# lachinov/brats2019

Hardware: AMD Instinct MI355X
Metric: volumes_per_sec_fwd_bwd_128cubed_x4ch (higher is better)
Workload: dtype bf16

## Files before the change

brats2019_amd/_lib.py:

```python
from __future__ import annotations

import ctypes as C
import os

import torch

_PKG = os.path.dirname(os.path.abspath(__file__))
LIB_PATH = os.environ.get("RU_LIB_PATH") or os.path.join(_PKG, "lib", "libresunet_hip.so")

_lib = None
PRECISIONS = {"f32": 0, "bf16x3": 1}
GRAD_PRECISIONS = {"bf16x3": 1, "bf16": 2}
FUSE_GN_BWD_STATS, FUSE_GN_BWD_APPLY, FUSE_SIDE_STREAM, FUSE_BATCH_WREDUCE, FUSE_TAIL_FINALIZE, FUSE_PW_DGRAD = 1, 2, 4, 8, 16, 32

_vp, _f, _d, _i, _sz = C.c_void_p, C.c_float, C.c_double, C.c_int, C.c_size_t

SIGNATURES = {
    "ru_last_error": (C.c_char_p, []),
    "ru_version": (_i, []),
    "ru_device_ok": (_i, []),
    "ru_conv3d_workspace_bytes": (_sz, [_i] * 7),
    "ru_conv3d_fwd": (_i, [_vp, _vp, _vp, _vp] + [_i] * 7 + [_vp, _sz, _vp]),
    "ru_conv3d_bwd_data": (_i, [_vp, _vp, _vp] + [_i] * 7 + [_vp, _sz, _vp]),
    "ru_conv3d_fwd_p": (_i, [_vp, _vp, _vp, _vp] + [_i] * 8 + [_vp, _sz, _vp]),
    "ru_conv3d_bwd_data_p": (_i, [_vp, _vp, _vp] + [_i] * 8 + [_vp, _sz, _vp]),
    "ru_conv3d_bwd_weight": (_i, [_vp, _vp, _vp, _vp] + [_i] * 7 + [_vp, _sz, _vp]),
    "ru_conv3d_bwd_weight_p": (_i, [_vp, _vp, _vp, _vp] + [_i] * 8 + [_vp, _sz, _vp]),
    "ru_groupnorm_workspace_bytes": (_sz, [_i, _i, _sz]),
    "ru_groupnorm_fwd": (_i, [_vp] * 7 + [_i, _i, _sz, _i, _f, _f, _vp, _sz, _vp]),
    "ru_groupnorm_bwd": (_i, [_vp] * 9 + [_i, _i, _sz, _i, _f, _vp, _sz, _vp]),
    "ru_leaky_relu_fwd": (_i, [_vp, _vp, _sz, _f, _vp]),
    "ru_leaky_relu_bwd": (_i, [_vp, _vp, _vp, _sz, _f, _vp]),
    "ru_upsample2x_trilinear_fwd": (_i, [_vp, _vp] + [_i] * 5 + [_vp]),
    "ru_upsample2x_trilinear_bwd": (_i, [_vp, _vp] + [_i] * 5 + [_vp]),
    "ru_sigmoid_fwd": (_i, [_vp, _vp, _sz, _vp]),
    "ru_criterion_workspace_bytes": (_sz, [_i, _i, _sz]),
    "ru_criterion_sums": (_i, [_vp, _vp, _vp, _i, _i, _sz, _f, _vp, _sz, _vp]),
    "ru_criterion_grad": (_i, [_vp, _vp, _vp, _d, _f, _f, _f, _f, _vp, _i, _i, _sz, _vp]),
    "ru_criterion_value": (_i, [C.POINTER(_d), _i, _d, _d, C.POINTER(_d), C.POINTER(_d)]),
    "ru_criterion_value_device": (_i, [_vp, _i, _d, _d, _d, _d, _vp, _vp]),
    "ru_crit_moments_workspace_bytes": (_sz, [_i, _i, _sz]),
    "ru_crit_moments": (_i, [_vp, _vp, _i, _i, _sz, C.c_uint, _vp, _vp, _sz, _vp]),
    "ru_crit_reduce": (_i, [_vp, _i, _i, _vp, _vp]),
    "ru_crit_eval": (_i, [_vp, _vp, _i, _i, _d, _d, _vp, _i, _vp, _vp, _vp]),
    "ru_crit_grad": (_i, [_vp, _vp, _vp, _vp, _i, _i, _sz, _i, _vp, _vp]),
    "ru_adam_amsgrad_step": (_i, [_vp] * 5 + [_sz] + [_f] * 5 + [_i, _vp]),
    "ru_adam_step": (_i, [_vp] * 5 + [_sz] + [_f] * 5 + [_i, _vp]),
    "ru_unet_create": (_vp, [_i, C.POINTER(_i), C.POINTER(_i), C.POINTER(_i), _i]),
    "ru_unet_destroy": (None, [_vp]),
    "ru_unet_set_precision": (_i, [_vp, _i]),
    "ru_unet_freeze_params": (_i, [_vp, _i]),
    "ru_unet_get_precision": (_i, [_vp]),
    "ru_unet_set_grad_precision": (_i, [_vp, _i]),
    "ru_unet_get_grad_precision": (_i, [_vp]),
    "ru_unet_set_fusion": (_i, [_vp, C.c_uint]),
    "ru_unet_probe": (_i, [_vp, _i]),
    "ru_unet_probe_read": (_i, [_vp, C.POINTER(C.c_double), C.POINTER(_i)]),
    "ru_unet_probe_read_families": (_i, [_vp, C.POINTER(C.c_double), C.POINTER(_i), _i]),
    "ru_unet_param_count": (_i, [_vp]),
    "ru_unet_param_name": (C.c_char_p, [_vp, _i]),
    "ru_unet_param_ndim": (_i, [_vp, _i]),
    "ru_unet_param_dim": (_i, [_vp, _i, _i]),
    "ru_unet_param_offset": (_sz, [_vp, _i]),
    "ru_unet_param_total": (_sz, [_vp]),
    "ru_unet_param_is_dead": (_i, [_vp, _i]),
    "ru_unet_workspace_bytes": (_sz, [_vp] + [_i] * 5),
    "ru_unet_forward": (_i, [_vp, _vp, _vp, _vp] + [_i] * 5 + [_vp, _sz, _vp]),
    "ru_unet_backward": (_i, [_vp] * 6),
    "ru_unet_backward_criterion": (_i, [_vp, _vp, _vp, _vp, _d, _f, _f, _f, _f, _vp, _vp, _vp]),
    "ru_unet_gn_stats": (_i, [_vp, _i, _vp, _vp, _vp]),
    "ru_comm_unique_id": (_i, [_vp]),
    "ru_comm_init": (_i, [C.POINTER(_vp), _vp, _i, _i]),
    "ru_comm_destroy": (_i, [_vp]),
    "ru_comm_rank": (_i, [_vp]),
    "ru_comm_world": (_i, [_vp]),
    "ru_allreduce": (_i, [_vp, _vp, _sz, _i, _vp]),
    "ru_comm_group_begin": (_i, []),
    "ru_comm_group_end": (_i, []),
    "ru_tta_merge": (_i, [_vp, _i, C.c_uint, _vp, _vp, _vp, _i, _i, _i, _i, _vp]),
    "ru_compose_labels": (_i, [_vp, _vp, C.c_ulonglong, _vp, _sz, _vp]),
    "ru_dice_counts": (_i, [_vp, _vp, _vp, _i, _i, _sz, _vp]),
    "ru_dice_accumulate": (_i, [_vp, _vp, _i, _i, _i, _vp]),
    "ru_hausdorff_workspace_bytes": (_sz, [_i] * 6),
    "ru_hausdorff_sq": (_i, [_vp, _vp] + [_i] * 6 + [_vp, _vp, _sz, _vp]),
    "ru_hausdorff_accumulate": (_i, [_vp, _vp] + [_i] * 4 + [_vp]),
    "ru_label_confusion": (_i, [_vp, _vp, _i, _i, _i, _sz, _vp, _vp, _vp]),
    "ru_overlap_accumulate": (_i, [_vp, _i, _i, _i, _i, _vp, _vp, _vp]),
    "ru_dice1d_accumulate": (_i, [_vp, _vp, _i, _i, _i, _vp]),
    "ru_rmse_accumulate": (_i, [_vp, _vp, _vp]),
    "ru_surface_workspace_bytes": (_sz, [_i] * 6),
    "ru_surface_metrics": (_i, [_vp, _vp] + [_i] * 6 + [_d, _vp, _vp, _vp, _sz, _vp]),
    "ru_surface_accumulate": (_i, [_vp, _vp] + [_i] * 4 + [_vp]),
    "ru_lesion_workspace_bytes": (_sz, [_i] * 7),
    "ru_lesion_metrics": (_i, [_vp, _vp] + [_i] * 7 + [C.c_longlong, _d, _vp, _vp, _vp, _i, _vp, _sz, _vp]),
    "ru_lesion_accumulate": (_i, [_vp, _vp] + [_i] * 4 + [_vp]),
    "ru_tile_gather": (_i, [_vp, _vp] + [_i] * 6 + [C.POINTER(_i), _i, _i, _i, _vp]),
    "ru_tile_scatter": (_i, [_vp, _vp] + [_i] * 6 + [C.POINTER(_i), _i, _i, _i, C.POINTER(_i), C.POINTER(_i), _vp]),
    "ru_blend_accumulate": (_i, [_vp, _vp, _vp] + [_i] * 8 + [C.POINTER(_i), _i, C.POINTER(_i), _i, C.POINTER(_i), _i, _i, _i, _vp]),
    "ru_blend_finalize": (_i, [_vp, _vp, _vp] + [_i] * 8 + [C.POINTER(_i), _i, C.POINTER(_i), _i, C.POINTER(_i), _i, _vp]),
    "ru_case_bbox": (_i, [_vp, _vp, _i, _i, _i, _i, _vp]),
# ... 8 lines not shown
    "ru_postprocess_regions": (_i, [_vp, _vp, _i, _i, _i, _i, C.POINTER(C.c_longlong), C.POINTER(C.c_ulonglong), C.c_uint, C.c_uint, _i, _vp, _vp, _vp, _vp, _sz, _vp]),
    "ru_ens_accumulate": (_i, [_vp, _i, C.c_uint, _vp, _i, _i, _i, _i, _i, C.POINTER(_i), C.POINTER(_i), _vp]),
    "ru_ens_finalize": (_i, [_vp, _i, _vp, _vp, _vp, _i, _sz, _vp]),
    "ru_ens_accumulate_finalize": (_i, [_vp, _i, C.c_uint, _vp, _i, _i, _vp, _vp, _vp, _i, _i, _i, _i, C.POINTER(_i), C.POINTER(_i), _vp]),
    "ru_ens_argmax": (_i, [_vp, _i, _vp, _i, _sz, _vp]),
    "ru_paste_probs": (_i, [_vp, _vp, _i, _i, _i, _i, C.POINTER(_i), C.POINTER(_i), _vp]),
    "ru_unc_accumulate": (_i, [_vp, _i, C.c_uint, _vp, _vp, _i, _i, _i, _i, _i, C.POINTER(_i), C.POINTER(_i), _vp]),
    "ru_unc_accumulate_finalize": (_i, [_vp, _i, C.c_uint, _vp, _vp, _i, _i, _i, _vp, _vp, _vp, _vp, _i, _i, _i, _i, C.POINTER(_i), C.POINTER(_i), _vp]),
    "ru_unc_finalize": (_i, [_vp, _vp, _i, _i, _i, _vp, _vp, _vp, _vp, _i, _sz, _vp]),
    "ru_unc_histogram": (_i, [_vp, _vp, _vp, _i, _i, _i, _vp, _vp, _vp]),
    "ru_unc_score": (_i, [_vp, C.POINTER(_i), _i, _vp, _vp, _vp]),
    "ru_paste_u8c": (_i, [_vp, _vp, _i, _i, _i, _i, C.POINTER(_i), C.POINTER(_i), _vp]),
    "ru_zscore_workspace_bytes": (_sz, [_i, _sz]),
    "ru_zscore_stats": (_i, [_vp, _vp, _i, _sz, _vp, _sz, _vp]),
    "ru_augment_patch": (_i, [_vp, _vp, _vp, _vp, _i, _i, _i, _i, _vp, _vp, _vp, _i, _vp, _vp, _vp, _vp, _vp]),
    "ru_augment_patch_soft": (_i, [_vp, _vp, _vp, _vp, _vp, _i, _i, _i, _i, _vp, _vp, _vp, _i, _vp, _vp, _vp, _vp, _vp]),
    "ru_elastic_workspace_bytes": (_sz, [_i, _i, _i]),
    "ru_elastic_noise": (_i, [C.c_ulonglong, _i, _i, _i, _vp, _vp]),
    "ru_elastic_field": (_i, [_vp, _d, _d, _i, _i, _i, _vp, _vp, _sz, _vp]),
    "ru_elastic_warp": (_i, [_vp, _i, _vp, _i, _vp, _i, _i, _i, _i, _vp, _vp, _vp, _vp, _vp]),
    "ru_layout_convert": (_i, [_vp, _vp, _i, _i, _sz, _i, _vp]),
    "ru_upsample2x_trilinear_fwd_l": (_i, [_vp, _vp] + [_i] * 5 + [_f, _vp]),
    "ru_upsample2x_trilinear_bwd_l": (_i, [_vp, _vp] + [_i] * 5 + [_vp]),
    "ru_conv3d_fwd_l": (_i, [_vp, _vp, _vp, _vp] + [_i] * 7 + [_vp, _sz, _vp]),
    "ru_conv3d_bwd_weight_l": (_i, [_vp, _vp, _vp] + [_i] * 7 + [_vp, _sz, _vp]),
}


CRIT_KINDS = {"Dice_loss_joint": 0, "BCE_Loss": 1, "MSE_Loss": 2, "CE_Loss": 3, "Dice1D": 4, "GDL_joint": 5, "sens_loss_joint": 6,
              "Dice_loss_separate": 7}
CRIT_MOMENTS, CRIT_MAX_TERMS = 7, 8
CRIT_MASK_LOGS, CRIT_MASK_ALL = (1 << 4) | (1 << 5), 0x7F
CRIT_M_D2 = 6

CONF_PROB, CONF_LABEL, OVERLAP_MAX_LABELS = 0, 1, 8
OVERLAP_MODES = {"itk": 0, "wt": 1, "validate": 2}

UNC_MEASURES = {"std": 0, "entropy": 1}
UNC_REGIONS, UNC_LEVELS, UNC_CLASSES = 3, 101, 4

SURFACE_PROB, SURFACE_LABEL, SURFACE_REGIONS, SURFACE_COUNTS = 0, 1, 3, 6
SURFACE_COLUMNS = {"dice": 0, "sensitivity": 1, "specificity": 2, "hd95": 3}

LESION_COUNTS, LESION_TABLE_COLUMNS, LESION_CHUNK = 6, 5, 8
LESION_COLUMNS = {"dice": 0, "hd95": 1}

POSTPROCESS_MASKS, POSTPROCESS_LABELS, POSTPROCESS_REGIONS, POSTPROCESS_STATS = 0, 1, 3, 6


class CritTerm(C.Structure):
    _fields_ = [("kind", _i), ("weight", _d), ("priority", _d), ("bg_weight", _d)]


def load():
    global _lib
    if _lib is not None:
        return _lib
    if not os.path.exists(LIB_PATH):
        raise RuntimeError(
            "libresunet_hip.so not found at %s -- build it with `python -m brats2019_amd.build` "
            "(hipcc, gfx950).  There is no CPU fallback for this path." % LIB_PATH)
    lib = C.CDLL(LIB_PATH)
    for name, (res, args) in SIGNATURES.items():
        if os.environ.get("RU_LIB_PATH") and not hasattr(lib, name):
            continue
        fn = getattr(lib, name)
        fn.restype = res
        fn.argtypes = args
    _lib = lib
    return lib


def last_error():
    return load().ru_last_error().decode("utf-8", "replace")


def check(rc, what=""):
    if rc != 0:
        raise RuntimeError("libresunet_hip: %s failed (%d): %s" % (what, rc, last_error()))


def require_gpu():
    if not torch.cuda.is_available():
        raise RuntimeError("brats2019_amd: no ROCm GPU visible -- the ResUNet hot path is HIP-only (no CPU fallback)")
    load()


def ptr(t, allow_none=False):
    if t is None:
        if allow_none:
            return None
        raise ValueError("null tensor")
    if not t.is_cuda:
        raise RuntimeError("brats2019_amd: expected a ROCm device tensor, got a %s tensor (HIP-only path)" % t.device)
    if not t.is_contiguous():
        raise ValueError("tensor must be contiguous (NCDHW)")
    return C.c_void_p(t.data_ptr())


def f32(t):
    if t.dtype != torch.float32:
        raise TypeError("expected float32, got %s" % t.dtype)
    return ptr(t)


def stream():
# ... 6 lines not shown
```

brats2019_amd/csrc/conv3_sb.hip:

```cpp
#include "conv3_sb_common.hpp"
#include "conv3_wz_pack.hpp"
#include "conv3_mx_pack.hpp"

namespace ru {

constexpr int SB1_W_BYTES = SB_KSTEPS * 2 * 64 * 16;
template <int TZ, int TY, bool IN16, bool OUT16>
__global__ __launch_bounds__(256, 2) void conv3_sb_kernel(const Conv3Args a, const u32x4* __restrict__ wfrag, int ntz, int nty, int ntx, int nchunk) {
    using P = SB<TZ, TY>;
    constexpr int MT = P::MT, HY = P::HY, HX = P::HX, HVOLP = P::HVOLP, NSV = P::NSV, NROW = P::NROW;
    extern __shared__ __attribute__((aligned(16))) float smem[];
    u32x4* lds = reinterpret_cast<u32x4*>(smem);

    const int tid = threadIdx.x, lane = tid & 63, wave = tid >> 6;
    int b = xcd_swizzle(blockIdx.x, gridDim.x);
    const int tiles_per_sample = ntz * nty * ntx;
    const int n = b / tiles_per_sample;
    const int tis = b - n * tiles_per_sample;
    b = tis;
    const int tx = b % ntx; b /= ntx;
    const int ty = b % nty;
    const int tz = b / nty;
    const int z0 = tz * TZ, y0 = ty * TY, x0 = tx * 16;
    const int cog = blockIdx.y;
// ... 526 lines not shown
    float t[8];
#pragma unroll
    for (int e = 0; e < 8; ++e) {
        const int ci = (g & 1) * 8 + e;
        float v = 0.f;
        if (tap >= 0 && ci < cin_conv && co < cout_conv)
            v = mode == 0 ? w[((size_t)co * Cin_f + ci) * 27 + tap] : w[((size_t)ci * Cin_f + co) * 27 + (26 - tap)];
        t[e] = v;
    }
    u32x4 hi, lo;
    split8(t, hi, lo);
    hfrag[((size_t)f * 2 + 0) * 64 + lane] = hi;
    hfrag[((size_t)f * 2 + 1) * 64 + lane] = lo;
}
constexpr int SB_FORMS_ALL = 15;
__device__ __forceinline__ void sb_pack_both(const float* __restrict__ w, u32x4* __restrict__ wfrag, int Cin_f, int Cout_f, int mode, int nchunk, int ncog, int forms, int i) {
    const int direct = ncog * nchunk * SB_KSTEPS * 64;
    if (i < direct) { if (!(forms & 16)) sb_pack_one(w, wfrag, Cin_f, Cout_f, mode, nchunk, ncog, i); return; }
    const int cin_conv = mode == 0 ? Cin_f : Cout_f, cout_conv = mode == 0 ? Cout_f : Cin_f;
    if (sb_head_shape(cin_conv, cout_conv)) { sb_pack_head_one(w, wfrag + (size_t)direct * 2, Cin_f, Cout_f, mode, i - direct); return; }
    if (mx_channels_ok(cin_conv, cout_conv)) { if (forms & 4) mx_pack_one(w, wfrag + (size_t)direct * 2, Cin_f, Cout_f, mode, ncog, i - direct, (forms & 32) != 0); return; }
    if (!wz_channels_ok(cin_conv, cout_conv)) return;
    const int wz = WZ16_FORM ? (cout_conv / 32) * nchunk * 4 * 2 * WZ_KSTEPS * 64 : 0;
    int r = i - direct;
    if (WZ16_FORM && (forms & 1)) {
        if (r < wz) { wz_pack_one(w, reinterpret_cast<wz_u32x4*>(wfrag + (size_t)direct * 2), Cin_f, Cout_f, mode, nchunk, cout_conv / 32, r); return; }
        r -= wz;
    }
    const int wz32 = (cout_conv / 32) * nchunk * 4 * 9 * 64;
    if (forms & 2) {
        if (r < wz32) { wz32_pack_one(w, reinterpret_cast<wz_u32x4*>(wfrag + ((size_t)direct + wz) * 2), Cin_f, Cout_f, mode, nchunk, cout_conv / 32, r); return; }
        r -= wz32;
    }
    if (forms & 8) wz32mx_pack_one(w, reinterpret_cast<wz_u32x4*>(wfrag + ((size_t)direct + wz + wz32) * 2), Cin_f, Cout_f, mode, nchunk, cout_conv / 32, r);
}
static inline int sb_pack_threads(int cin_conv, int cout_conv, int forms) {
    const int nchunk = cdiv(cin_conv, 16), ncog = cdiv(cout_conv, 16);
    return ncog * nchunk * SB_KSTEPS * 64 + (wz_channels_ok(cin_conv, cout_conv) ? (cout_conv / 32) * nchunk * (((WZ16_FORM && (forms & 1)) ? 4 * 2 * WZ_KSTEPS : 0) + ((forms & 2) ? 4 * 9 : 0) + ((forms & 8) ? WZ32MX_UNITS_XI : 0)) * 64 : 0)
         + (sb_head_shape(cin_conv, cout_conv) ? SB_HEAD_KSTEPS * 64 : 0) + (((forms & 4) && mx_channels_ok(cin_conv, cout_conv)) ? ncog * MX_UNITS * 64 : 0);
}
static int sb_pack_forms(int mode) {
    if (mode == 1) return conv3_mxg_enabled() ? (4 | 32) : 0;
    const bool mxon = conv3_mx_enabled();
    const char* e = getenv("RU_WZ");
    if (e && *e == '0') return mxon ? 4 : 0;
    if (mxon && conv3_mx_wz_enabled()) return 4 | 8;
    return (mxon ? 4 : 0) | (conv3_wz32_enabled() ? 2 : 1);
}
__global__ void conv3_sb_pack_kernel(const float* __restrict__ w, u32x4* __restrict__ wfrag, int Cin_f, int Cout_f, int mode, int nchunk, int ncog, int forms) {
    sb_pack_both(w, wfrag, Cin_f, Cout_f, mode, nchunk, ncog, forms, blockIdx.x * blockDim.x + threadIdx.x);
}
__global__ void conv3_sb_pack_batch_kernel(const SbPackBatch b) {
    const SbPackEntry& e = b.e[blockIdx.y];
    sb_pack_both(e.w, reinterpret_cast<u32x4*>(e.wfrag), e.Cin_f, e.Cout_f, e.mode, e.nchunk, e.ncog, e.forms, blockIdx.x * blockDim.x + threadIdx.x);
}
int conv3_sb_pack_batch(SbPackBatch& b, hipStream_t s) {
    if (b.n == 0) return RU_OK;
    int maxtotal = 0;
    for (int i = 0; i < b.n; ++i) {
        const SbPackEntry& e = b.e[i];
        const int t = sb_pack_threads(e.mode == 0 ? e.Cin_f : e.Cout_f, e.mode == 0 ? e.Cout_f : e.Cin_f, e.forms);
        if (t > maxtotal) maxtotal = t;
    }
    hipLaunchKernelGGL(conv3_sb_pack_batch_kernel, dim3(cdiv(maxtotal, 256), b.n), dim3(256), 0, s, b);
    RU_CHECK_LAUNCH("conv3_sb_pack_batch_kernel");
    b.n = 0;
    return RU_OK;
}
int conv3_sb_switch_signature() {
    const char* e = getenv("RU_WZ");
    return ((e && *e == '0') ? 0 : 1) | (conv3_wz32_enabled() ? 2 : 0) | (conv3_mx_enabled() ? 4 : 0) | (conv3_mx_wz_enabled() ? 8 : 0) | (conv3_mxg_enabled() ? 16 : 0);
}
bool conv3_sb_forward_skips_direct(int N, int Cin, int Cout, int D, int H, int W) {
    if (conv3_sb_uses_wz(N, Cin, Cout, D, H, W, 2)) return true;
    return conv3_mx_enabled() && conv3_mx_shape_ok(N, Cin, Cout, D, H, W);
}
int conv3_sb_pack_add(SbPackBatch& b, const float* w, void* wfrag, int Cin_f, int Cout_f, int mode, bool all_forms, hipStream_t s, bool skip_direct) {
    if (b.n == RU_PACK_BATCH) { const int rc = conv3_sb_pack_batch(b, s); if (rc) return rc; }
    const int cin_conv = mode == 0 ? Cin_f : Cout_f, cout_conv = mode == 0 ? Cout_f : Cin_f;
    SbPackEntry& e = b.e[b.n++];
    e.w = w; e.wfrag = wfrag; e.Cin_f = Cin_f; e.Cout_f = Cout_f; e.mode = mode; e.nchunk = cdiv(cin_conv, 16); e.ncog = cdiv(cout_conv, 16);
    e.forms = all_forms ? SB_FORMS_ALL : (sb_pack_forms(mode) | ((skip_direct && mode == 0) ? 16 : 0));
    return RU_OK;
}

size_t conv3_sb_frag_bytes_direct(int Cin_conv, int Cout_conv) {
    return (size_t)cdiv(Cout_conv, 16) * cdiv(Cin_conv, 16) * SB_KSTEPS * 2 * 64 * 16;
}
size_t conv3_sb_frag_bytes(int Cin_conv, int Cout_conv) {
    return conv3_sb_frag_bytes_direct(Cin_conv, Cout_conv) + wz_frag_bytes(Cin_conv, Cout_conv) + wz32_frag_bytes(Cin_conv, Cout_conv) + wz32mx_frag_bytes(Cin_conv, Cout_conv)
         + (sb_head_shape(Cin_conv, Cout_conv) ? (size_t)SB_HEAD_KSTEPS * 2 * 64 * 16 : 0) + mx_frag_bytes(Cin_conv, Cout_conv);
}
bool conv3_sb_head_takes_residual(int N, int Cin, int Cout, int D, int H, int W) {
    const char* e = getenv("RU_HEAD_RES");
    if (e && *e == '0') return false;
    if (!conv3_sb_head_form_enabled() || !sb_head_shape(Cin, Cout) || Cin % 16 != 0 || (W & 3) != 0) return false;
    if ((size_t)D * H * W * 64 >= ((size_t)1 << 31)) return false;
    return sb_use_v2(sb_choose(N, Cout, D, H, W));
}
bool conv3_sb_head_form_enabled() {
    const char* e = getenv("RU_HEAD_FORM");
    return !(e && e[0] == '0');
}

int conv3_sb_pack_weights(const float* w, void* wfrag, int Cin_f, int Cout_f, int mode, hipStream_t s, bool grad_operand) {
    const int cin_conv = mode == 0 ? Cin_f : Cout_f, cout_conv = mode == 0 ? Cout_f : Cin_f;
    const int nchunk = cdiv(cin_conv, 16), ncog = cdiv(cout_conv, 16);
    const int forms = SB_FORMS_ALL | (grad_operand ? 32 : 0);
    const int total = sb_pack_threads(cin_conv, cout_conv, forms);
    hipLaunchKernelGGL(conv3_sb_pack_kernel, dim3(cdiv(total, 256)), dim3(256), 0, s, w, (u32x4*)wfrag, Cin_f, Cout_f, mode, nchunk, ncog, forms);
    RU_CHECK_LAUNCH("conv3_sb_pack_kernel");
    return RU_OK;
}

bool conv3_sb_uses_wz(int N, int Cin, int Cout, int D, int H, int W, int products) {
    const char* e = getenv("RU_WZ");
    const bool off = e && *e == '0';
    return !off && products != 1 && conv3_wz_shape_ok(N, Cin, Cout, D, H, W);
}
int conv3_sb_tiles_per_sample(int N, int Cin, int Cout, int D, int H, int W, int products) {
    if (conv3_sb_uses_wz(N, Cin, Cout, D, H, W, products)) return (int)wz_grid_x(N, Cout, D, H, W);
    const SBChoice c = sb_choose(N, Cout, D, H, W);
    if (sb_use_v2(c)) return (int)sb2_grid_x(N, Cout, D, H, W);
    return cdiv(D, c.tz) * cdiv(H, c.ty) * cdiv(W, 16);
}

bool conv3_sb_bst_usable(int N, int Cout, int D, int H, int W) { return sb_use_v2(sb_choose(N, Cout, D, H, W)); }

template <int TZ, int TY, bool IN16, bool OUT16>
static int sb_cfg(const Conv3Args& a, hipStream_t s) {
    using P = SB<TZ, TY>;
    static PerDevice attr_done;
    if (!attr_done.get()) {
        hipError_t e = hipFuncSetAttribute(reinterpret_cast<const void*>(conv3_sb_kernel<TZ, TY, IN16, OUT16>), hipFuncAttributeMaxDynamicSharedMemorySize, P::LDS_BYTES + SB1_W_BYTES);
        if (e != hipSuccess) return hip_fail(e, "hipFuncSetAttribute(conv3_sb)");
        attr_done.set();
    }
// ... 86 lines not shown
```

brats2019_amd/csrc/engine.hip:

```cpp
#include "ru_common.h"

#include <vector>
#include <math.h>
#include <stdlib.h>
#include <string.h>

#include <string>
#include <vector>

namespace ru {

static thread_local char g_err[512] = "";
void set_error(const char* fmt, ...) {
    va_list ap;
    va_start(ap, fmt);
    vsnprintf(g_err, sizeof(g_err), fmt, ap);
    va_end(ap);
}
int hip_fail(hipError_t e, const char* what) {
    set_error("%s: %s", what, hipGetErrorString(e));
    return RU_EHIP;
}

constexpr float kSlope = 1e-2f;
// ... 30 lines not shown
    return on;
}
static int trace_sync(const char* what, hipStream_t s) {
    fprintf(stderr, "[ru] %s\n", what);
    const hipError_t e = hipStreamSynchronize(s);
    if (e != hipSuccess) { fprintf(stderr, "[ru]   -> %s\n", hipGetErrorString(e)); return hip_fail(e, what); }
    return RU_OK;
}

enum { FAM_CONV_L0 = 0, FAM_CONV_DEEP, FAM_WGRAD_L0, FAM_WGRAD_DEEP, FAM_GN, FAM_PW, FAM_OTHER, FAM_COUNT };
enum { INST_CONV16_FWD = 0, INST_CONV16_DGRAD, INST_CONV_DEEP_FWD, INST_CONV_DEEP_DGRAD, INST_WGRAD16_FUSED, INST_WGRAD16_PLAIN, INST_WGRAD_DEEP, INST_COUNT };
struct FamilySink {
    std::vector<hipEvent_t> ev;
    std::vector<int> fam;
    std::vector<int> inst;
    size_t used = 0;
    ~FamilySink() { for (hipEvent_t e : ev) (void)hipEventDestroy(e); }
};
static thread_local FamilySink* t_sink = nullptr;
static thread_local int t_hint_c = 16;
static thread_local int t_hint_inst = -1;
struct RedQueues { WgradRedList main, side; hipStream_t side_stream = nullptr; };
static thread_local RedQueues* t_red = nullptr;
static WgradRedList* red_for(hipStream_t s) { return t_red ? ((t_red->side_stream && s == t_red->side_stream) ? &t_red->side : &t_red->main) : nullptr; }
static int family_of(const char* call) {
    auto has = [&](const char* k) { return strstr(call, k) != nullptr; };
    if (has("wgrad3_launch")) return t_hint_c <= 16 ? FAM_WGRAD_L0 : FAM_WGRAD_DEEP;
    if (has("wgrad_reduce_flush")) return FAM_WGRAD_DEEP;
    if (has("conv3_launch") || has("conv3_sb_launch")) return t_hint_c <= 16 ? FAM_CONV_L0 : FAM_CONV_DEEP;
    if (has("gn_")) return FAM_GN;
    if (has("conv1_") || has("wgrad1_launch") || has("up2_") || has("s2d_launch") || has("d2s_launch") || has("lrelu_bwd_launch")) return FAM_PW;
    return FAM_OTHER;
}
static void sink_begin(const char* call, hipStream_t s) {
    FamilySink& k = *t_sink;
    while (k.ev.size() < k.used + 2) {
        hipEvent_t e;
        if (hipEventCreate(&e) != hipSuccess) return;
        k.ev.push_back(e);
    }
    if (k.fam.size() < k.ev.size() / 2) { k.fam.resize(k.ev.size() / 2); k.inst.resize(k.ev.size() / 2); }
    k.fam[k.used / 2] = family_of(call);
    k.inst[k.used / 2] = t_hint_inst;
    t_hint_inst = -1;
    (void)hipEventRecord(k.ev[k.used], s);
}
static void sink_end(hipStream_t s) {
    FamilySink& k = *t_sink;
    if (k.ev.size() < k.used + 2) return;
    (void)hipEventRecord(k.ev[k.used + 1], s);
    k.used += 2;
}

#define RU_RUN(call)                      \
    do {                                  \
        if (!A.dry) {                     \
            if (A.failed) { set_error("workspace too small"); return RU_ENOMEM; } \
            if (t_sink) sink_begin(#call, s); \
            const int rc__ = (call);      \
            if (t_sink) sink_end(s);      \
            if (rc__ != RU_OK) return rc__; \
            if (trace_on()) { const int rt__ = trace_sync(#call, s); if (rt__ != RU_OK) return rt__; } \
        }                                 \
    } while (0)

__global__ void gn_scale_shift_kernel(const float* __restrict__ gamma, const float* __restrict__ beta, const float* __restrict__ mean,
                                      const float* __restrict__ rstd, float* __restrict__ scale, float* __restrict__ shift, int N, int C, int G) {
    const int i = blockIdx.x * blockDim.x + threadIdx.x;
    if (i >= N * C) return;
    const int n = i / C, c = i % C, g = c / (C / G);
    const float a = gamma[c] * rstd[n * G + g];
    scale[i] = a;
    shift[i] = beta[c] - mean[n * G + g] * a;
}

}

using namespace ru;

struct ParamInfo {
    std::string name;
    int ndim;
    int dims[5];
    size_t offset, numel;
    bool dead;
};

struct BlockP {
    int down = -1, conv1 = -1, conv2 = -1, n1w = -1, n1b = -1, n2w = -1, n2b = -1;
    int cin_down = 0, c = 0;
    size_t pk_f1 = 0, pk_f2 = 0, pk_d1 = 0, pk_d2 = 0, pk_downT = 0, pk_down16 = 0;
    size_t fk_f1 = 0, fk_f2 = 0, fk_d1 = 0, fk_d2 = 0;
};

struct GNSave {
    float *mean = nullptr, *rstd = nullptr, *scale = nullptr, *shift = nullptr;
    float act_slope = 0.01f;
    float* k = nullptr;
};

struct BlockSave {
    const BlockP* bp = nullptr;
    const float* xprev = nullptr;
    float* xs2d = nullptr;
    const float* x = nullptr;
    const GNSave* xg = nullptr;
    float *y1 = nullptr, *y2 = nullptr, *out = nullptr;
    GNSave g1, g2;
    int N = 0, C = 0, D = 0, H = 0, W = 0;
};

struct DecSave {
    const float* z = nullptr;
    float *u = nullptr, *v = nullptr, *c = nullptr;
    const float* skip = nullptr;
    int level = 0;
};

constexpr int kOneProduct = 0x100;
struct ru_unet {
    int depth = 0, nout = 0;
    std::vector<int> enc, dec, ch;
    std::vector<ParamInfo> params;
    size_t total = 0;
    std::vector<std::vector<BlockP>> enc_blocks, dec_blocks;
    std::vector<BlockP> first_blocks;
    std::vector<int> up_w, dec1_w;
    std::vector<size_t> pk_upT, pk_decT;
    int conv_in = -1, nin_w = -1, nin_b = -1, conv_out_w = -1, conv_out_b = -1;
    size_t pk_in = 0, pk_out = 0, pk_out_d = 0, pk_total = 0;
    size_t fk_in = 0, fk_out = 0, fk_out_d = 0, fk_total = 0;
    int precision = RU_PREC_F32;
    unsigned fusion = RU_FUSE_GN_BWD_STATS | RU_FUSE_GN_BWD_APPLY | RU_FUSE_SIDE_STREAM | RU_FUSE_BATCH_WREDUCE | RU_FUSE_PW_DGRAD;
    int grad_precision = RU_PREC_BF16X3;
    int grad_products() const { return (precision == RU_PREC_BF16X3 && grad_precision == RU_PREC_BF16) ? 1 : 3; }
    int wgrad_mode() const { return precision | (grad_products() == 1 ? kOneProduct : 0); }
    bool c16 = false;
    char* fpack = nullptr;

    bool have_fwd = false, training = false;
    int N = 0, D = 0, H = 0, W = 0;
    char* ws = nullptr;
    size_t ws_bytes = 0, fwd_end = 0, fwd_keep = 0;
    float* pack = nullptr;
    const float* x_in = nullptr;
    const float* x_in4 = nullptr;
    bool x_in4_planned = false;
    bool params_frozen = false;
    const float* packed_params = nullptr;
    const void* packed_base = nullptr;
    int packed_prec = -1;
    bool packed_c16 = false;
    int pack_sig = -1;
    float *y0 = nullptr, *t0 = nullptr, *probs = nullptr;
    GNSave g0;
    const float* head_in = nullptr;
    std::vector<BlockSave> first_s;
    std::vector<std::vector<BlockSave>> enc_s, dec_s;
    std::vector<DecSave> dstage;
    std::vector<const float*> skips;
    std::vector<GNSave> gn_order;
    bool probe_on = false;
    bool probe_families = false;
    ru::FamilySink* sink = nullptr;
    std::vector<hipEvent_t> probe_ev;
    size_t probe_used = 0;
    hipStream_t side = nullptr;
    std::vector<hipEvent_t> fork_ev;
    ru::RedQueues red;
    unsigned* tickets = nullptr;
    int ticket_next = 0;
    unsigned* next_ticket() { return tickets ? tickets + (ticket_next++ & 255) : nullptr; }
    bool tails() const { return c16 && (fusion & RU_FUSE_TAIL_FINALIZE) && tickets != nullptr; }
    size_t fork_used = 0;
    ~ru_unet() {
        for (hipEvent_t e : probe_ev) (void)hipEventDestroy(e);
        for (hipEvent_t e : fork_ev) (void)hipEventDestroy(e);
        if (side) (void)hipStreamDestroy(side);
        if (tickets) (void)hipFree(tickets);
        delete sink;
    }
};

static int add_param(ru_unet* h, const std::string& name, std::initializer_list<int> dims, bool dead = false) {
    ParamInfo p;
    p.name = name;
    p.ndim = (int)dims.size();
    size_t n = 1;
    int i = 0;
    for (int d : dims) { p.dims[i++] = d; n *= (size_t)d; }
    for (; i < 5; ++i) p.dims[i] = 1;
    p.offset = h->total;
    p.numel = n;
    p.dead = dead;
    h->total += n;
    h->params.push_back(p);
    return (int)h->params.size() - 1;
}

static BlockP add_block(ru_unet* h, const std::string& prefix, int cin_down, int c, bool dead = false) {
    BlockP b;
    b.c = c;
    b.cin_down = cin_down;
    if (cin_down > 0) b.down = add_param(h, prefix + "downsample.0.weight", {c, cin_down, 2, 2, 2}, dead);
    b.conv1 = add_param(h, prefix + "conv1.conv1.weight", {c, c, 3, 3, 3}, dead);
    b.conv2 = add_param(h, prefix + "conv2.conv1.weight", {c, c, 3, 3, 3}, dead);
    b.n1w = add_param(h, prefix + "norm1.weight", {c}, dead);
    b.n1b = add_param(h, prefix + "norm1.bias", {c}, dead);
    b.n2w = add_param(h, prefix + "norm2.weight", {c}, dead);
    b.n2b = add_param(h, prefix + "norm2.bias", {c}, dead);
    return b;
}

static std::string fmt(const char* f, int a, int b = 0) {
    char buf[128];
    snprintf(buf, sizeof(buf), f, a, b);
    return buf;
}

static void assign_block_packs(ru_unet* h, BlockP& b) {
    const size_t n = conv3_packed_floats(b.c, b.c);
    b.pk_f1 = h->pk_total; h->pk_total += n;
    b.pk_f2 = h->pk_total; h->pk_total += n;
    b.pk_d1 = h->pk_total; h->pk_total += n;
    b.pk_d2 = h->pk_total; h->pk_total += n;
    if (b.down >= 0) {
        b.pk_downT = h->pk_total; h->pk_total += (size_t)8 * b.cin_down * b.c;
        b.pk_down16 = h->pk_total; h->pk_total += (size_t)2 * 8 * b.cin_down * b.c;
    }
    const size_t f = conv3_sb_frag_bytes(b.c, b.c);
    b.fk_f1 = h->fk_total; h->fk_total += f;
    b.fk_f2 = h->fk_total; h->fk_total += f;
    b.fk_d1 = h->fk_total; h->fk_total += f;
    b.fk_d2 = h->fk_total; h->fk_total += f;
}

extern "C" ru_unet_t ru_unet_create(int depth, const int* encoder_layers, const int* decoder_layers,
                                    const int* number_of_channels, int number_of_outputs) {
    if (depth < 2 || depth > 8 || !encoder_layers || !decoder_layers || !number_of_channels || number_of_outputs < 1) {
        set_error("ru_unet_create: bad configuration");
        return nullptr;
    }
    for (int i = 0; i < depth; ++i) {
        if (number_of_channels[i] % kGroups != 0 || number_of_channels[i] <= 0 || encoder_layers[i] < 1 || decoder_layers[i] < 1) {
            set_error("ru_unet_create: channels must be positive multiples of 8 (GroupNorm(8, C)) and layer counts >= 1");
            return nullptr;
        }
    }
    ru_unet* h = new ru_unet();
    if (const char* e = getenv("RU_SIDE_STREAM")) { if (*e == '0') h->fusion &= ~(unsigned)RU_FUSE_SIDE_STREAM; }
    if (const char* e = getenv("RU_FUSION_OFF")) h->fusion &= ~(unsigned)strtoul(e, nullptr, 0);
    if (const char* e = getenv("RU_FUSION_ON")) h->fusion |= (unsigned)strtoul(e, nullptr, 0) & 63u;
    h->depth = depth;
    h->nout = number_of_outputs;
    h->enc.assign(encoder_layers, encoder_layers + depth);
    h->dec.assign(decoder_layers, decoder_layers + depth);
    h->ch.assign(number_of_channels, number_of_channels + depth);
    const std::vector<int>& ch = h->ch;
    h->enc_blocks.resize(depth - 1);
    for (int i = 0; i < depth - 1; ++i)
        for (int j = 0; j < h->enc[i + 1]; ++j)
            h->enc_blocks[i].push_back(add_block(h, fmt("encoder_convs.%d.%d.", i, j), j == 0 ? ch[i] : 0, ch[i + 1]));
    for (int i = 0; i < depth - 1; ++i) h->up_w.push_back(add_param(h, fmt("upsampling.%d.1.weight", i), {ch[i], ch[i + 1], 1, 1, 1}));
    h->dec_blocks.resize(depth);
    for (int i = 0; i < depth; ++i)
        for (int j = 0; j < h->dec[i]; ++j)
            h->dec_blocks[i].push_back(add_block(h, fmt("decoder_convs.%d.%d.", i, j), 0, ch[i], i == depth - 1));
    for (int i = 0; i < depth; ++i)
        h->dec1_w.push_back(add_param(h, fmt("decoder_convs1x1.%d.weight", i), {ch[i], 2 * ch[i], 1, 1, 1}, i == depth - 1));
    h->conv_in = add_param(h, "conv_input.weight", {ch[0], kInCh, 3, 3, 3});
    h->nin_w = add_param(h, "norm_input.weight", {ch[0]});
    h->nin_b = add_param(h, "norm_input.bias", {ch[0]});
    for (int j = 0; j < h->enc[0]; ++j) h->first_blocks.push_back(add_block(h, fmt("conv_first.%d.", j), 0, ch[0]));
    h->conv_out_w = add_param(h, "conv_output.weight", {number_of_outputs, ch[0], 3, 3, 3});
    h->conv_out_b = add_param(h, "conv_output.bias", {number_of_outputs});
    h->pk_total = 0;
    h->pk_in = h->pk_total; h->pk_total += conv3_packed_floats(kInCh, ch[0]);
    h->pk_out = h->pk_total; h->pk_total += conv3_packed_floats(ch[0], number_of_outputs);
    h->pk_out_d = h->pk_total; h->pk_total += conv3_packed_floats(number_of_outputs, ch[0]);
    h->fk_total = 0;
    h->fk_in = h->fk_total; h->fk_total += conv3_sb_frag_bytes(kInCh, ch[0]);
    h->fk_out = h->fk_total; h->fk_total += conv3_sb_frag_bytes(ch[0], number_of_outputs);
    h->fk_out_d = h->fk_total; h->fk_total += conv3_sb_frag_bytes(number_of_outputs, ch[0]);
    for (auto& b : h->first_blocks) assign_block_packs(h, b);
    for (auto& lv : h->enc_blocks) for (auto& b : lv) assign_block_packs(h, b);
    for (int i = 0; i < depth - 1; ++i) for (auto& b : h->dec_blocks[i]) assign_block_packs(h, b);
    for (int i = 0; i < depth - 1; ++i) {
        h->pk_upT.push_back(h->pk_total); h->pk_total += (size_t)ch[i + 1] * ch[i];
        h->pk_decT.push_back(h->pk_total); h->pk_total += (size_t)2 * ch[i] * ch[i];
    }
    return h;
}

extern "C" void ru_unet_destroy(ru_unet_t h) { delete h; }
extern "C" int ru_unet_set_precision(ru_unet_t h, int precision) {
    RU_REQUIRE(h && (precision == RU_PREC_F32 || precision == RU_PREC_BF16X3), "ru_unet_set_precision: bad argument");
    h->precision = precision;
    h->have_fwd = false;
    return RU_OK;
}
extern "C" int ru_unet_get_precision(ru_unet_t h) { return h ? h->precision : -1; }
extern "C" int ru_unet_set_fusion(ru_unet_t h, unsigned mask) {
    RU_REQUIRE(h && (mask & ~(unsigned)(RU_FUSE_GN_BWD_STATS | RU_FUSE_GN_BWD_APPLY | RU_FUSE_SIDE_STREAM | RU_FUSE_BATCH_WREDUCE | RU_FUSE_TAIL_FINALIZE | RU_FUSE_PW_DGRAD)) == 0, "ru_unet_set_fusion: bad argument");
// ... 23 lines not shown
    for (size_t i = 0; i + 1 < k.used; i += 2) {
        hipError_t e = hipEventSynchronize(k.ev[i + 1]);
        if (e != hipSuccess) return hip_fail(e, "hipEventSynchronize(family probe)");
        float t = 0.f;
        e = hipEventElapsedTime(&t, k.ev[i], k.ev[i + 1]);
        if (e != hipSuccess) return hip_fail(e, "hipEventElapsedTime(family probe)");
        ms[k.fam[i / 2]] += t;
        launches[k.fam[i / 2]] += 1;
        const int in = k.inst[i / 2];
        if (in >= 0 && ru::FAM_COUNT + in < nfam) { ms[ru::FAM_COUNT + in] += t; launches[ru::FAM_COUNT + in] += 1; }
    }
    k.used = 0;
    return RU_OK;
}
extern "C" int ru_unet_probe_read(ru_unet_t h, double* total_ms, int* launches) {
    RU_REQUIRE(h && total_ms && launches, "ru_unet_probe_read: null argument");
    double sum = 0.0;
    for (size_t i = 0; i + 1 < h->probe_used; i += 2) {
        hipError_t e = hipEventSynchronize(h->probe_ev[i + 1]);
        if (e != hipSuccess) return hip_fail(e, "hipEventSynchronize(probe)");
        float ms = 0.f;
        e = hipEventElapsedTime(&ms, h->probe_ev[i], h->probe_ev[i + 1]);
        if (e != hipSuccess) return hip_fail(e, "hipEventElapsedTime(probe)");
        sum += ms;
    }
    *total_ms = sum;
    *launches = (int)(h->probe_used / 2);
    h->probe_used = 0;
    return RU_OK;
}
extern "C" int ru_unet_set_grad_precision(ru_unet_t h, int precision) {
    RU_REQUIRE(h && (precision == RU_PREC_BF16X3 || precision == RU_PREC_BF16), "ru_unet_set_grad_precision: RU_PREC_BF16X3 or RU_PREC_BF16");
    h->grad_precision = precision;
    return RU_OK;
}
extern "C" int ru_unet_get_grad_precision(ru_unet_t h) { return h ? h->grad_precision : -1; }
extern "C" int ru_unet_freeze_params(ru_unet_t h, int frozen) {
    RU_REQUIRE(h, "ru_unet_freeze_params: null handle");
    h->params_frozen = frozen != 0;
    h->packed_params = nullptr;
    return RU_OK;
}
extern "C" int ru_unet_param_count(ru_unet_t h) { return h ? (int)h->params.size() : 0; }
extern "C" const char* ru_unet_param_name(ru_unet_t h, int i) { return (h && i >= 0 && i < (int)h->params.size()) ? h->params[i].name.c_str() : nullptr; }
extern "C" int ru_unet_param_ndim(ru_unet_t h, int i) { return (h && i >= 0 && i < (int)h->params.size()) ? h->params[i].ndim : 0; }
extern "C" int ru_unet_param_dim(ru_unet_t h, int i, int d) { return (h && i >= 0 && i < (int)h->params.size() && d >= 0 && d < 5) ? h->params[i].dims[d] : 0; }
extern "C" size_t ru_unet_param_offset(ru_unet_t h, int i) { return (h && i >= 0 && i < (int)h->params.size()) ? h->params[i].offset : 0; }
extern "C" size_t ru_unet_param_total(ru_unet_t h) { return h ? h->total : 0; }
extern "C" int ru_unet_param_is_dead(ru_unet_t h, int i) { return (h && i >= 0 && i < (int)h->params.size()) ? (int)h->params[i].dead : 0; }

static inline const float* P(const ru_unet* h, const float* params, int idx) { return params ? params + h->params[idx].offset : nullptr; }
static inline float* G(const ru_unet* h, float* grads, int idx) { return grads ? grads + h->params[idx].offset : nullptr; }

static int pack_all(ru_unet* h, const float* params, Arena& A, hipStream_t s) {
    float* pk = h->pack;
    SbPackBatch batch;
    batch.n = 0;
    auto pack3 = [&](int pidx, size_t pk_off, size_t fk_off, int cin_f, int cout_f, int mode, int lvl = -1) -> int {
        const bool skipd = h->training && h->c16 && mode == 0 && lvl >= 0 &&
                           conv3_sb_forward_skips_direct(h->N, cin_f, cout_f, h->D >> lvl, h->H >> lvl, h->W >> lvl);
        if (h->precision == RU_PREC_BF16X3) RU_RUN(conv3_sb_pack_add(batch, P(h, params, pidx), h->fpack + fk_off, cin_f, cout_f, mode, !h->training, s, skipd));
        if (h->precision == RU_PREC_F32 && h->c16) RU_RUN(conv3_f32c_pack_weights(P(h, params, pidx), h->fpack + fk_off, cin_f, cout_f, mode, s));
        if (!h->c16) RU_RUN(conv3_pack_weights(P(h, params, pidx), pk + pk_off, cin_f, cout_f, mode, s));
        return RU_OK;
    };
    auto blk = [&](const BlockP& b, int lvl) -> int {
        int rc = pack3(b.conv1, b.pk_f1, b.fk_f1, b.c, b.c, 0, lvl); if (rc) return rc;
        rc = pack3(b.conv2, b.pk_f2, b.fk_f2, b.c, b.c, 0, lvl); if (rc) return rc;
        if (h->training) {
            rc = pack3(b.conv1, b.pk_d1, b.fk_d1, b.c, b.c, 1); if (rc) return rc;
            rc = pack3(b.conv2, b.pk_d2, b.fk_d2, b.c, b.c, 1); if (rc) return rc;
        }
        if (b.down >= 0) {
            if (h->c16) RU_RUN(pack_down16_launch(P(h, params, b.down), pk + b.pk_down16, pk + b.pk_down16 + (size_t)8 * b.cin_down * b.c, b.c, b.cin_down, s));
            else RU_RUN(transpose_launch(P(h, params, b.down), pk + b.pk_downT, b.c, 8 * b.cin_down, s));
        }
        return RU_OK;
    };
    { int rc = pack3(h->conv_in, h->pk_in, h->fk_in, kInCh, h->ch[0], 0); if (rc) return rc; }
    { int rc = pack3(h->conv_out_w, h->pk_out, h->fk_out, h->ch[0], h->nout, 0); if (rc) return rc; }
    if (h->training) { int rc = pack3(h->conv_out_w, h->pk_out_d, h->fk_out_d, h->ch[0], h->nout, 1); if (rc) return rc; }
    for (auto& b : h->first_blocks) { int rc = blk(b, 0); if (rc) return rc; }
    for (size_t lv = 0; lv < h->enc_blocks.size(); ++lv) for (auto& b : h->enc_blocks[lv]) { int rc = blk(b, (int)lv + 1); if (rc) return rc; }
    for (int i = 0; i < h->depth - 1; ++i) for (auto& b : h->dec_blocks[i]) { int rc = blk(b, i); if (rc) return rc; }
    for (int i = 0; i < h->depth - 1; ++i) {
        if (h->c16 && !h->training) continue;
        RU_RUN(transpose_launch(P(h, params, h->up_w[i]), pk + h->pk_upT[i], h->ch[i], h->ch[i + 1], s));
        RU_RUN(transpose_launch(P(h, params, h->dec1_w[i]), pk + h->pk_decT[i], h->ch[i], 2 * h->ch[i], s));
    }
    RU_RUN(conv3_sb_pack_batch(batch, s));
    return RU_OK;
}

static int conv3_gn(ru_unet* h, Arena& A, hipStream_t s, const float* x, const float* wp, const char* wf, float* y, const GNSave* in_gn,
                    const float* gamma, const float* beta, GNSave& out_gn, int N, int Cin, int Cout, int D, int H, int W, bool x_c16 = true,
                    bool x_c4 = false) {
    const int nblk = !h->c16 ? conv3_tiles_per_sample(N, Cin, Cout, D, H, W, h->precision)
                     : (h->precision == RU_PREC_F32 ? conv3_f32c_tiles_per_sample(N, Cin, Cout, D, H, W) : conv3_sb_tiles_per_sample(N, Cin, Cout, D, H, W));
    t_hint_c = Cout;
    float* partials = A.alloc((size_t)N * Cout * nblk * 2);
    out_gn.mean = A.alloc_keep((size_t)N * kGroups);
    out_gn.rstd = A.alloc_keep((size_t)N * kGroups);
    out_gn.scale = A.alloc_keep((size_t)N * Cout);
    out_gn.shift = A.alloc_keep((size_t)N * Cout);
    Conv3Args a{};
    a.x = x; a.wp = wp; a.y = y; a.mode = h->precision; a.wfrag = wf;
    a.in_scale = in_gn ? in_gn->scale : nullptr;
    a.in_shift = in_gn ? in_gn->shift : nullptr;
    a.in_slope = in_gn ? in_gn->act_slope : kSlope;
    a.stat_partials = partials;
    a.N = N; a.Cin = Cin; a.Cout = Cout; a.D = D; a.H = H; a.W = W;
    a.in_c16 = h->c16 && x_c16; a.out_c16 = h->c16; a.in_c4 = x_c4;
    a.products = 2;
    const bool probed = h->probe_on && !A.dry && h->c16 && x_c16 && !x_c4 && Cin == 16 && Cout == 16 && D == h->D && H == h->H && W == h->W;
    if (probed) {
        while (h->probe_ev.size() < h->probe_used + 2) {
            hipEvent_t e;
            const hipError_t er = hipEventCreate(&e);
            if (er != hipSuccess) return hip_fail(er, "hipEventCreate(probe)");
            h->probe_ev.push_back(e);
        }
        (void)hipEventRecord(h->probe_ev[h->probe_used], s);
    }
    const int ksplit = (!h->c16 && conv3_effective_mode(h->precision, W) == RU_PREC_F32) ? conv3_f32_ksplit(N, Cin, Cout, D, H, W) : 1;
    out_gn.k = (h->training && h->c16) ? A.alloc_keep((size_t)N * 3 * Cout) : nullptr;
    const bool tail = !A.dry && h->tails() && ksplit == 1 && h->precision == RU_PREC_BF16X3;
    if (tail) {
        FinTail& f = a.fin;
        f.ticket = h->next_ticket(); f.kind = 1; f.nblk = nblk; f.N = N; f.C = Cout; f.G = kGroups; f.V = (size_t)D * H * W; f.eps = kEps;
        f.gamma = gamma; f.beta = beta; f.mean = out_gn.mean; f.rstd = out_gn.rstd; f.scale = out_gn.scale; f.shift = out_gn.shift; f.bst_k = out_gn.k;
    }
    if (ksplit > 1) {
        const size_t nel = (size_t)N * Cout * D * H * W;
        float* part = A.alloc((size_t)ksplit * nel);
        a.y = part; a.stat_partials = nullptr; a.ksplit = ksplit;
        RU_RUN(conv3_launch(a, s));
        RU_RUN(sum_partials_launch(part, ksplit, nel, y, s));
        RU_RUN(gn_stats_launch(y, partials, N, Cout, (size_t)D * H * W, s));
    } else {
        t_hint_inst = (a.in_c16 && a.out_c16) ? (Cin == 16 && Cout == 16 ? INST_CONV16_FWD : (Cin >= 32 ? INST_CONV_DEEP_FWD : -1)) : -1;
        RU_RUN(conv3_launch(a, s));
// ... 31 lines not shown
        Conv1Args c1{};
        c1.x0 = sv.xs2d; c1.C0 = 8 * bp.cin_down; c1.y = xd; c1.out_slope = 1.f;
        c1.N = N; c1.Cout = C; c1.V = Vo;
        if (h->c16) {
            c1.x0 = xprev; c1.s2d = 1; c1.Dc = Do; c1.Hc = Ho; c1.Wc = Wo;
            c1.wT = h->pack + bp.pk_down16; c1.ldw = 8 * bp.cin_down;
            RU_RUN(conv1_16_launch(c1, s));
        } else {
            RU_RUN(s2d_launch(xprev, sv.xs2d, N, bp.cin_down, D, H, W, s));
            c1.wT = h->pack + bp.pk_downT; c1.ldw = C;
            RU_RUN(conv1_launch(c1, s));
        }
        x = xd; D = Do; H = Ho; W = Wo;
    }
    const size_t V = (size_t)D * H * W;
    sv.x = x; sv.N = N; sv.C = C; sv.D = D; sv.H = H; sv.W = W;
    sv.y1 = A.alloc((size_t)N * C * V);
    int rc = conv3_gn(h, A, s, x, h->pack + bp.pk_f1, h->fpack + bp.fk_f1, sv.y1, xin_gn, P(h, params, bp.n1w), P(h, params, bp.n1b), sv.g1, N, C, C, D, H, W);
    if (rc) return rc;
    sv.y2 = A.alloc((size_t)N * C * V);
    rc = conv3_gn(h, A, s, sv.y1, h->pack + bp.pk_f2, h->fpack + bp.fk_f2, sv.y2, &sv.g1, P(h, params, bp.n2w), P(h, params, bp.n2b), sv.g2, N, C, C, D, H, W);
    if (rc) return rc;
    if (defer_out) {
        RU_REQUIRE(h->c16 && !xin_gn, "block_fwd: the deferred residual pass exists in the voxel-major flow only");
        sv.out = h->training ? A.alloc((size_t)N * C * V) : nullptr;
        *out = sv.out;
        return RU_OK;
    }
    sv.out = recycle ? out_early : A.alloc((size_t)N * C * V);
    if (h->c16) RU_RUN(gn_apply16_launch(sv.y2, sv.g2.scale, sv.g2.shift, x, sv.out, N, C, V, kSlope, s,
                                         xin_gn ? xin_gn->scale : nullptr, xin_gn ? xin_gn->shift : nullptr, xin_gn ? xin_gn->act_slope : 1.f));
    else RU_RUN(gn_apply_launch(sv.y2, sv.g2.scale, sv.g2.shift, x, sv.out, N, C, V, kSlope, s));
    *out = sv.out;
    if (recycle) A.rewind(mark);
    return RU_OK;
}

static int unet_forward_impl(ru_unet* h, const float* params, const float* x, float* probs_out, Arena& A, hipStream_t s) {
    const int N = h->N, depth = h->depth;
    std::vector<int> Dl(depth), Hl(depth), Wl(depth);
    for (int i = 0; i < depth; ++i) { Dl[i] = h->D >> i; Hl[i] = h->H >> i; Wl[i] = h->W >> i; }
    auto Vl = [&](int i) { return (size_t)Dl[i] * Hl[i] * Wl[i]; };
    h->gn_order.clear();
    static const bool f32c_off = [] { const char* e = getenv("RU_F32C"); return e && *e == '0'; }();
    const bool f32c_fits = (size_t)h->D * h->H * h->W * 64 < ((size_t)1 << 31);
    h->c16 = (h->precision == RU_PREC_BF16X3 || (h->precision == RU_PREC_F32 && !h->training && !f32c_off && f32c_fits)) && (h->W & 3) == 0;
    for (int c : h->ch) h->c16 = h->c16 && (c % 16 == 0);
    h->pack = A.alloc(h->pk_total);
    h->fpack = reinterpret_cast<char*>(A.alloc(h->fk_total / sizeof(float) + 64));
    float* wf4_in = A.alloc(conv3_sb4_frag_bytes(h->ch[0]) / sizeof(float) + 64);
    const bool reuse_packs = h->params_frozen && !h->training && !A.dry && h->packed_params == params && h->packed_base == (const void*)h->pack &&
                             h->packed_prec == h->precision && h->packed_c16 == h->c16;
    int rc = RU_OK;
    if (!reuse_packs) {
        rc = pack_all(h, params, A, s);
        if (rc) return rc;
    }

    const int C0 = h->ch[0];
    const BlockSave* head_block = nullptr;
    h->x_in = x;
    h->x_in4 = nullptr;
    h->x_in4_planned = false;
    h->y0 = A.alloc((size_t)N * C0 * Vl(0));
    const size_t stem_mark = A.off;
    if (h->c16 && h->precision == RU_PREC_BF16X3 && conv3_sb4_usable(N, kInCh, C0, Dl[0], Hl[0], Wl[0])) {
        float* x4 = A.alloc((size_t)N * 4 * Vl(0));
        float* wf4 = wf4_in;
        h->x_in4 = x4;
        h->x_in4_planned = true;
        RU_RUN(pad_to_c4_launch(x, x4, N, kInCh, Vl(0), s));
        if (!reuse_packs) RU_RUN(conv3_sb4_pack_weights(P(h, params, h->conv_in), wf4, kInCh, C0, 0, s));
        rc = conv3_gn(h, A, s, x4, nullptr, reinterpret_cast<const char*>(wf4), h->y0, nullptr, P(h, params, h->nin_w), P(h, params, h->nin_b), h->g0,
                      N, kInCh, C0, Dl[0], Hl[0], Wl[0], false, true);
    } else {
        rc = conv3_gn(h, A, s, x, h->pack + h->pk_in, h->fpack + h->fk_in, h->y0, nullptr, P(h, params, h->nin_w), P(h, params, h->nin_b), h->g0, N, kInCh, C0, Dl[0], Hl[0], Wl[0], false);
    }
    if (rc) return rc;
    if (!h->training) A.rewind(stem_mark);
    h->g0.act_slope = 1.0f;
    const bool stem_fused = h->c16 && !h->first_blocks.empty() && h->first_blocks[0].down < 0;
    h->t0 = nullptr;
    if (!stem_fused) {
        h->t0 = A.alloc((size_t)N * C0 * Vl(0));
        if (h->c16) RU_RUN(gn_apply16_launch(h->y0, h->g0.scale, h->g0.shift, nullptr, h->t0, N, C0, Vl(0), 1.0f, s));
        else RU_RUN(gn_apply_launch(h->y0, h->g0.scale, h->g0.shift, nullptr, h->t0, N, C0, Vl(0), 1.0f, s));
    }
    const float* cur = stem_fused ? h->y0 : h->t0;
    h->first_s.assign(h->first_blocks.size(), BlockSave());
    for (size_t j = 0; j < h->first_blocks.size(); ++j) {
        rc = block_fwd(h, params, A, s, h->first_blocks[j], cur, N, Dl[0], Hl[0], Wl[0], h->first_s[j], &cur, (stem_fused && j == 0) ? &h->g0 : nullptr);
        if (rc) return rc;
    }
    h->skips.assign(depth - 1, nullptr);
    h->enc_s.assign(depth - 1, {});
    for (int i = 0; i < depth - 1; ++i) {
        h->skips[i] = cur;
        h->enc_s[i].assign(h->enc_blocks[i].size(), BlockSave());
        for (size_t j = 0; j < h->enc_blocks[i].size(); ++j) {
            const int lv = j == 0 ? i : i + 1;
            rc = block_fwd(h, params, A, s, h->enc_blocks[i][j], cur, N, Dl[lv], Hl[lv], Wl[lv], h->enc_s[i][j], &cur);
            if (rc) return rc;
        }
    }
    h->dstage.assign(depth - 1, DecSave());
    h->dec_s.assign(depth - 1, {});
    for (int i = depth - 2; i >= 0; --i) {
        DecSave& ds = h->dstage[i];
        ds.level = i;
        ds.z = cur;
        ds.skip = h->skips[i];
        const int Ci = h->ch[i], Cc = h->ch[i + 1];
        const bool recycle = !h->training;
        float* c_early = recycle ? A.alloc((size_t)N * Ci * Vl(i)) : nullptr;
        const size_t dmark = A.off;
        if (!h->c16) {
            ds.u = A.alloc((size_t)N * Cc * Vl(i));
            RU_RUN(up2_fwd_launch(cur, ds.u, N, Cc, Dl[i + 1], Hl[i + 1], Wl[i + 1], s));
        }
        ds.v = A.alloc((size_t)N * Ci * Vl(i));
        Conv1Args c1{};
        c1.x0 = ds.u; c1.C0 = Cc; c1.y = ds.v; c1.out_slope = kSlope;
        c1.N = N; c1.Cout = Ci; c1.V = Vl(i);
        ds.c = recycle ? c_early : A.alloc((size_t)N * Ci * Vl(i));
        Conv1Args c2{};
        c2.x0 = ds.skip; c2.C0 = Ci; c2.x1 = ds.v; c2.C1 = Ci;
        c2.y = ds.c; c2.out_slope = 1.f; c2.N = N; c2.Cout = Ci; c2.V = Vl(i);
        if (h->c16) {
            float* zc = A.alloc((size_t)N * Ci * Vl(i + 1));
            c1.x0 = cur; c1.y = zc; c1.out_slope = 1.f; c1.V = Vl(i + 1);
            c1.wT = P(h, params, h->up_w[i]); c1.ldw = Cc;
// ... 104 lines not shown
    }
    Wgrad3Args w{};
    w.x = x; w.dy = dy; w.dw = dw; w.mode = mode; w.x_c16 = x_c16; w.dy_c16 = dy_c16; w.dy_s16 = dy_s16 ? 1 : 0;
    w.products = products; w.defer = red_for(s);
    w.in_scale = xg ? xg->scale : nullptr; w.in_shift = xg ? xg->shift : nullptr; w.in_slope = xg ? xg->act_slope : kSlope;
    w.ws_bytes = wgrad3_workspace_bytes(N, Cin, Cout, D, H, W);
    w.ws = A.alloc(w.ws_bytes / sizeof(float));
    w.N = N; w.Cin = Cin; w.Cout = Cout; w.D = D; w.H = H; w.W = W;
    if (gb) {
        w.gb_y = gb->y; w.gb_d = gb->d; w.gb_scale = gb->g->scale; w.gb_shift = gb->g->shift; w.gb_coef = gb->coef; w.gb_slope = kSlope;
        w.gb_out = const_cast<float*>(dy); w.dy_s16 = 0; w.gb_g16 = gb->g16 ? 1 : 0;
    }
    t_hint_inst = (x_c16 && dy_c16) ? (Cin == 16 && Cout == 16 ? (gb ? INST_WGRAD16_FUSED : INST_WGRAD16_PLAIN) : (Cin >= 32 ? INST_WGRAD_DEEP : -1)) : -1;
    RU_RUN(wgrad3_launch(w, s));
    return RU_OK;
}

static int wgrad1_run(Arena& A, hipStream_t s, const float* x, const float* dy, float* dw, int ldw, int N, int Cin, int Cout, size_t V,
                      bool c16 = false, int tap_split = 0) {
    Wgrad1Args w{};
    w.x = x; w.dy = dy; w.dw = dw; w.ldw = ldw; w.c16 = c16; w.tap_split = tap_split; w.defer = red_for(s);
    w.ws_bytes = wgrad1_workspace_bytes(N, Cin, Cout, V);
    w.ws = A.alloc(w.ws_bytes / sizeof(float));
    w.N = N; w.Cin = Cin; w.Cout = Cout; w.V = V;
    RU_RUN(wgrad1_launch(w, s));
    return RU_OK;
}

static int side_event(ru_unet* h, hipEvent_t* out) {
    if (h->fork_used == h->fork_ev.size()) {
        hipEvent_t e;
        const hipError_t er = hipEventCreateWithFlags(&e, hipEventDisableTiming);
        if (er != hipSuccess) return hip_fail(er, "hipEventCreateWithFlags(side)");
        h->fork_ev.push_back(e);
    }
    *out = h->fork_ev[h->fork_used++];
    return RU_OK;
}
static int side_fork(ru_unet* h, hipStream_t main) {
    if (!h->side) {
        int lo = 0, hi = 0;
        (void)hipDeviceGetStreamPriorityRange(&lo, &hi);
        const hipError_t er = hipStreamCreateWithPriority(&h->side, hipStreamNonBlocking, lo);
        if (er != hipSuccess) return hip_fail(er, "hipStreamCreateWithPriority(side)");
    }
    h->red.side_stream = h->side;
    hipEvent_t e;
    int rc = side_event(h, &e);
    if (rc) return rc;
    hipError_t er = hipEventRecord(e, main);
    if (er == hipSuccess) er = hipStreamWaitEvent(h->side, e, 0);
    return er == hipSuccess ? RU_OK : hip_fail(er, "side_fork");
}
static int side_join(ru_unet* h, hipStream_t main) {
    if (!h->side || h->fork_used == 0) return RU_OK;
    hipEvent_t e;
    int rc = side_event(h, &e);
    if (rc) return rc;
    hipError_t er = hipEventRecord(e, h->side);
    if (er == hipSuccess) er = hipStreamWaitEvent(main, e, 0);
    h->fork_used = 0;
    return er == hipSuccess ? RU_OK : hip_fail(er, "side_join");
}

struct GNNext {
    const float* y; const float* k; float slope;
    const GNSave* g; const float* gamma; float* dgamma; float* dbeta;
    FusedSums out;
};
static int block_bwd(ru_unet* h, const float* params, float* grads, Arena& A, hipStream_t s, const BlockSave& sv, const float* dout,
                     const float** dxprev_out, const float* join = nullptr, bool* joined = nullptr, const FusedSums* sums2 = nullptr,
                     GNNext* nx = nullptr) {
    if (joined) *joined = false;
    const BlockP& bp = *sv.bp;
    const int N = sv.N, C = sv.C, D = sv.D, H = sv.H, W = sv.W;
    t_hint_c = C;
    const size_t V = (size_t)D * H * W;
    float* dy2 = A.alloc((size_t)N * C * V);
    const bool c16 = h->c16;
    const bool fa = c16 && h->precision == RU_PREC_BF16X3 && C == 16 && (h->fusion & RU_FUSE_GN_BWD_APPLY);
    const bool ds16 = c16;
    const int dgrad_products = c16 ? 1 : h->grad_products();
    float *coef2 = nullptr, *coef1 = nullptr;
    int rc = gn_bwd(h, A, s, sv.y2, dout, sv.g2, P(h, params, bp.n2w), kSlope, dy2, G(h, grads, bp.n2w), G(h, grads, bp.n2b), N, C, V, sums2,
                    fa ? &coef2 : nullptr, ds16);
    if (rc) return rc;
    const bool g16 = fa && h->grad_products() == 3 && conv3_mxg_usable(N, C, C, D, H, W);
    const GbApply gb2{sv.y2, dout, &sv.g2, coef2, g16};
    const bool aside = !A.dry && (h->fusion & RU_FUSE_SIDE_STREAM) && c16 && h->precision == RU_PREC_BF16X3 && !fa && !trace_on();
    hipStream_t sw = s;
    if (aside) { rc = side_fork(h, s); if (rc) return rc; sw = h->side; }
    rc = wgrad3_run(A, sw, h->wgrad_mode(), sv.y1, &sv.g1, dy2, G(h, grads, bp.conv2), N, C, C, D, H, W, c16, c16, nullptr, ds16, fa ? &gb2 : nullptr);
    if (rc) return rc;
    float* da1 = A.alloc((size_t)N * C * V);
    Conv3Args d2{};
    d2.x = dy2; d2.wp = h->pack + bp.pk_d2; d2.y = da1; d2.mode = h->precision; d2.products = h->grad_products(); d2.wfrag = h->fpack + bp.fk_d2; d2.in_c16 = c16; d2.out_c16 = c16; d2.in_s16 = ds16; d2.in_g16 = g16; d2.N = N; d2.Cin = C; d2.Cout = C; d2.D = D; d2.H = H; d2.W = W;
    const bool fuse1 = c16 && h->precision == RU_PREC_BF16X3 && conv3_sb_bst_usable(N, C, D, H, W) && (h->fusion & RU_FUSE_GN_BWD_STATS);
    FusedSums sums1;
    if (fuse1) {
        sums1.nblk = conv3_sb_tiles_per_sample(N, C, C, D, H, W, dgrad_products);
        sums1.part = A.alloc((size_t)N * C * sums1.nblk * 2);
        sums1.coef = A.alloc((size_t)N * C * 3);
        d2.bst_y = sv.y1; d2.bst_k = sv.g1.k; d2.bst_slope = kSlope; d2.stat_partials = sums1.part;
        if (!A.dry && h->tails()) {
            fill_bwd_tail(h, d2.fin, sums1, sv.g1, P(h, params, bp.n1w), G(h, grads, bp.n1w), G(h, grads, bp.n1b), N, C, V, 1);
            sums1.done = true;
        }
    }
    t_hint_inst = c16 ? (C == 16 ? INST_CONV16_DGRAD : INST_CONV_DEEP_DGRAD) : -1;
    RU_RUN(conv3_launch(d2, s));
    float* dy1 = A.alloc((size_t)N * C * V);
    rc = gn_bwd(h, A, s, sv.y1, da1, sv.g1, P(h, params, bp.n1w), kSlope, dy1, G(h, grads, bp.n1w), G(h, grads, bp.n1b), N, C, V, fuse1 ? &sums1 : nullptr,
                fa ? &coef1 : nullptr, ds16);
    if (rc) return rc;
// ... 13 lines not shown
        nx->out.coef = A.alloc((size_t)N * C * 3);
        d1.bst_y = nx->y; d1.bst_k = nx->k; d1.bst_slope = nx->slope; d1.stat_partials = nx->out.part;
        if (!A.dry && h->tails() && nx->g) {
            fill_bwd_tail(h, d1.fin, nx->out, *nx->g, nx->gamma, nx->dgamma, nx->dbeta, N, C, V, 1);
            nx->out.done = true;
        }
    }
    t_hint_inst = c16 ? (C == 16 ? INST_CONV16_DGRAD : INST_CONV_DEEP_DGRAD) : -1;
    RU_RUN(conv3_launch(d1, s));
    if (bp.down < 0) { *dxprev_out = dx; return RU_OK; }
    const int Cp = bp.cin_down;
    {
        Wgrad1Args w{};
        w.x = c16 ? sv.xprev : sv.xs2d; w.dy = dx; w.dw = G(h, grads, bp.down); w.ldw = 8 * Cp; w.c16 = c16; w.tap_split = c16 ? Cp : 0; w.defer = red_for(s);
        if (c16) { w.s2d = 1; w.Dc = D; w.Hc = H; w.Wc = W; }
        w.ws_bytes = wgrad1_workspace_bytes(N, 8 * Cp, C, V);
        w.ws = A.alloc(w.ws_bytes / sizeof(float));
        w.N = N; w.Cin = 8 * Cp; w.Cout = C; w.V = V;
        RU_RUN(wgrad1_launch(w, s));
    }
    float* t = c16 ? nullptr : A.alloc((size_t)N * 8 * Cp * V);
    Conv1Args c1{};
    c1.x0 = dx; c1.C0 = C; c1.y = t; c1.out_slope = 1.f; c1.N = N; c1.Cout = 8 * Cp; c1.V = V;
    float* dxp = A.alloc((size_t)N * Cp * V * 8);
    if (c16) {
        c1.wT = h->pack + bp.pk_down16 + (size_t)8 * Cp * C; c1.ldw = C;
        c1.y = dxp; c1.s2d = 2; c1.Dc = D; c1.Hc = H; c1.Wc = W;
        c1.add = join;
        if (joined) *joined = true;
        if (nx && (h->fusion & RU_FUSE_GN_BWD_STATS) && conv1_16_bst_nblk(c1) > 0) {
            nx->out.nblk = conv1_16_bst_nblk(c1);
            nx->out.part = A.alloc((size_t)N * Cp * nx->out.nblk * 2);
            nx->out.coef = A.alloc((size_t)N * Cp * 3);
            c1.bst_y = nx->y; c1.bst_k = nx->k; c1.bst_slope = nx->slope; c1.stat_partials = nx->out.part;
        }
        RU_RUN(conv1_16_launch(c1, s));
    } else {
        c1.wT = P(h, params, bp.down); c1.ldw = 8 * Cp;
        RU_RUN(conv1_launch(c1, s));
        RU_RUN(d2s_launch(t, dxp, N, Cp, 2 * D, 2 * H, 2 * W, s));
    }
    *dxprev_out = dxp;
    return RU_OK;
}

static int unet_backward_impl(ru_unet* h, const float* params, const float* dprobs, float* grads, float* dx_in, Arena& A, hipStream_t s,
                              const CritGradArgs* crit = nullptr) {
    const int N = h->N, depth = h->depth;
    std::vector<int> Dl(depth), Hl(depth), Wl(depth);
    for (int i = 0; i < depth; ++i) { Dl[i] = h->D >> i; Hl[i] = h->H >> i; Wl[i] = h->W >> i; }
    auto Vl = [&](int i) { return (size_t)Dl[i] * Hl[i] * Wl[i]; };
    const int C0 = h->ch[0];
    t_hint_c = C0;
    RU_RUN(fill_launch(grads, 0.f, h->total, s));
    const bool c16 = h->c16;
    const bool head4 = c16 && conv3_sb4_usable(N, h->nout, C0, Dl[0], Hl[0], Wl[0]);
    float* d4 = head4 ? A.alloc((size_t)N * 4 * Vl(0)) : nullptr;
    const bool need_dlog = !head4 || C0 > 16;
    float* dlog = need_dlog ? A.alloc((size_t)N * h->nout * Vl(0)) : nullptr;
    const size_t wsb = bias_grad_workspace_bytes(N, h->nout, Vl(0));
    float* wsp = A.alloc(wsb / sizeof(float) + 1);
    const bool crit_fused = crit && head4 && !need_dlog;
    float* dpb = (!(head4 && !need_dlog) && (crit || A.dry)) ? A.alloc((size_t)N * h->nout * Vl(0)) : nullptr;
    if (crit && !crit_fused) {
        RU_RUN(crit_grad_launch(h->probs, crit->target, crit->sums, crit->count, crit->w_dice, crit->w_bce, crit->bgw, crit->priority, dpb, N, h->nout, Vl(0), s));
        dprobs = dpb;
    }
    if (crit_fused) {
        RU_RUN(head_grad_c4_crit_launch(h->probs, *crit, d4, G(h, grads, h->conv_out_b), N, h->nout, Vl(0), wsp, wsb, s));
    } else if (head4) {
        RU_RUN(head_grad_c4_launch(h->probs, dprobs, d4, G(h, grads, h->conv_out_b), N, h->nout, Vl(0), wsp, wsb, s));
        if (need_dlog) RU_RUN(sigmoid_bwd_launch(h->probs, dprobs, dlog, (size_t)N * h->nout * Vl(0), s));
    } else {
        RU_RUN(sigmoid_bwd_launch(h->probs, dprobs, dlog, (size_t)N * h->nout * Vl(0), s));
        RU_RUN(bias_grad_launch(dlog, G(h, grads, h->conv_out_b), N, h->nout, Vl(0), wsp, wsb, s));
    }
    int rc = wgrad3_run(A, s, h->wgrad_mode(), h->head_in, nullptr, dlog, G(h, grads, h->conv_out_w), N, C0, h->nout, Dl[0], Hl[0], Wl[0], c16, false,
                        C0 <= 16 ? d4 : nullptr);
    if (rc) return rc;
    float* dcur_buf = A.alloc((size_t)N * C0 * Vl(0));
    Conv3Args dh{};
    dh.x = dlog; dh.wp = h->pack + h->pk_out_d; dh.y = dcur_buf; dh.mode = h->precision; dh.wfrag = h->fpack + h->fk_out_d; dh.out_c16 = c16; dh.N = N; dh.Cin = h->nout; dh.Cout = C0; dh.D = Dl[0]; dh.H = Hl[0]; dh.W = Wl[0];
    if (head4) {
        float* wf4 = A.alloc(conv3_sb4_frag_bytes(C0) / sizeof(float) + 64);
        RU_RUN(conv3_sb4_pack_weights(P(h, params, h->conv_out_w), wf4, C0, h->nout, 1, s));
        dh.x = d4; dh.wfrag = wf4; dh.in_c4 = 1;
    }
    const bool no_bst = !(h->fusion & RU_FUSE_GN_BWD_STATS);
    const BlockSave* hb = (depth >= 2 && !h->dec_s[0].empty()) ? &h->dec_s[0].back() : nullptr;
    FusedSums hsums;
    if (head4 && hb && !no_bst && conv3_sb_bst_usable(N, C0, Dl[0], Hl[0], Wl[0])) {
        hsums.nblk = conv3_sb_tiles_per_sample(N, h->nout, C0, Dl[0], Hl[0], Wl[0]);
        hsums.part = A.alloc((size_t)N * C0 * hsums.nblk * 2);
        hsums.coef = A.alloc((size_t)N * C0 * 3);
        dh.bst_y = hb->y2; dh.bst_k = hb->g2.k; dh.bst_slope = kSlope; dh.stat_partials = hsums.part;
        if (!A.dry && h->tails()) {
            const BlockP& lb = *hb->bp;
            fill_bwd_tail(h, dh.fin, hsums, hb->g2, P(h, params, lb.n2w), G(h, grads, lb.n2w), G(h, grads, lb.n2b), N, C0, Vl(0), 1);
            hsums.done = true;
        }
    }
    RU_RUN(conv3_launch(dh, s));
    const float* dcur = dcur_buf;
    std::vector<const float*> dskip(depth - 1, nullptr);
    FusedSums carry = hsums;
    for (int i = 0; i <= depth - 2; ++i) {
        for (int j = (int)h->dec_s[i].size() - 1; j >= 0; --j) {
            const bool fused2 = carry.nblk > 0 && j == (int)h->dec_s[i].size() - 1;
            const FusedSums sin = carry;
            rc = block_bwd(h, params, grads, A, s, h->dec_s[i][j], dcur, &dcur, nullptr, nullptr, fused2 ? &sin : nullptr);
            if (rc) return rc;
        }
        carry = FusedSums();
        const DecSave& ds = h->dstage[i];
        const int Ci = h->ch[i], Cc = h->ch[i + 1];
        const size_t V = Vl(i);
        const float* wdec = P(h, params, h->dec1_w[i]);
        float* gdec = G(h, grads, h->dec1_w[i]);
        float* dsk = A.alloc((size_t)N * Ci * V);
        float* dv = A.alloc((size_t)N * Ci * V);
        float* dpre = A.alloc((size_t)N * Ci * V);
        const bool dg_fused = c16 && Ci <= 32 && (h->fusion & RU_FUSE_PW_DGRAD);
        if (c16) {
            Wgrad1Args w{};
            w.x = ds.skip; w.x1 = ds.v; w.C0 = Ci; w.dy = dcur; w.dw = gdec; w.ldw = 2 * Ci; w.c16 = 1; w.defer = red_for(s);
            w.ws_bytes = wgrad1_workspace_bytes(N, 2 * Ci, Ci, V);
            w.ws = A.alloc(w.ws_bytes / sizeof(float));
            w.N = N; w.Cin = 2 * Ci; w.Cout = Ci; w.V = V;
            if (dg_fused) { w.dg_w = wdec; w.dg_ldw = 2 * Ci; w.dg_y0 = dsk; w.dg_y1 = dpre; w.dg_mask_slope = kSlope; }
            RU_RUN(wgrad1_launch(w, s));
        } else {
            rc = wgrad1_run(A, s, ds.skip, dcur, gdec, 2 * Ci, N, Ci, Ci, V, c16);
            if (rc) return rc;
            rc = wgrad1_run(A, s, ds.v, dcur, A.dry ? nullptr : gdec + Ci, 2 * Ci, N, Ci, Ci, V, c16);
            if (rc) return rc;
        }
        Conv1Args a1{};
        a1.x0 = dcur; a1.C0 = Ci; a1.y = dsk; a1.out_slope = 1.f; a1.N = N; a1.Cout = Ci; a1.V = V;
// ... 117 lines not shown
        RU_RUN(conv3_launch(di, s));
    }
    if (t_red && !t_red->side.e.empty()) RU_RUN(wgrad_reduce_flush(t_red->side, h->side));
    if (!A.dry) { rc = side_join(h, s); if (rc) return rc; }
    if (t_red && !t_red->main.e.empty()) RU_RUN(wgrad_reduce_flush(t_red->main, s));
    return RU_OK;
}

static int check_dims(ru_unet* h, int N, int D, int H, int W) {
    const int m = 1 << (h->depth - 1);
    RU_REQUIRE(N > 0 && D > 0 && H > 0 && W > 0, "ru_unet: bad extents");
    RU_REQUIRE(D % m == 0 && H % m == 0 && W % m == 0, "ru_unet: D,H,W must be divisible by %d (model.py:361 stride-2 convs)", m);
    return RU_OK;
}

extern "C" size_t ru_unet_workspace_bytes(ru_unet_t h, int N, int D, int H, int W, int training) {
    if (!h || check_dims(h, N, D, H, W) != RU_OK) return 0;
    ru_unet tmp = *h;
    tmp.probe_ev.clear();
    tmp.probe_on = false;
    tmp.sink = nullptr;
    tmp.side = nullptr;
    tmp.tickets = nullptr;
    tmp.fork_ev.clear();
    tmp.N = N; tmp.D = D; tmp.H = H; tmp.W = W; tmp.training = training != 0;
    Arena A;
    A.dry = true;
    if (unet_forward_impl(&tmp, nullptr, nullptr, nullptr, A, nullptr) != RU_OK) return 0;
    if (training) {
        if (unet_backward_impl(&tmp, nullptr, nullptr, nullptr, (float*)1, A, nullptr) != RU_OK) return 0;
    }
    return A.need() + 4096;
}

extern "C" int ru_unet_forward(ru_unet_t h, const float* params, const float* x, float* probs, int N, int D, int H, int W, int training,
                               void* ws, size_t ws_bytes, ru_stream_t stream) {
    RU_REQUIRE(h && params && x && probs && ws, "ru_unet_forward: null argument");
    int rc = check_dims(h, N, D, H, W);
    if (rc) return rc;
    h->have_fwd = false;
    h->N = N; h->D = D; h->H = H; h->W = W; h->training = training != 0;
    h->ws = (char*)ws; h->ws_bytes = ws_bytes;
    Arena A;
    A.dry = false; A.base = (char*)ws; A.cap = ws_bytes;
    if (!h->tickets && (h->fusion & RU_FUSE_TAIL_FINALIZE)) {
        hipError_t e = hipMalloc((void**)&h->tickets, 256 * sizeof(unsigned));
        if (e != hipSuccess) { h->tickets = nullptr; return hip_fail(e, "ru_unet_forward: ticket words"); }
    }
    if (h->tickets && (h->fusion & RU_FUSE_TAIL_FINALIZE)) {
        hipError_t e = hipMemsetAsync(h->tickets, 0, 256 * sizeof(unsigned), (hipStream_t)stream);
        if (e != hipSuccess) return hip_fail(e, "ru_unet_forward: ticket words");
    }
    h->ticket_next = 0;
    ru::t_sink = h->probe_families ? h->sink : nullptr;
    rc = unet_forward_impl(h, params, x, probs, A, (hipStream_t)stream);
    ru::t_sink = nullptr;
    if (rc) return rc;
    if (A.failed) { set_error("ru_unet_forward: workspace too small (%zu bytes given)", ws_bytes); return RU_ENOMEM; }
    h->fwd_end = A.off;
    h->fwd_keep = A.keep;
    h->have_fwd = true;
    return RU_OK;
}

static int backward_entry(ru_unet_t h, const float* params, const float* dprobs, const CritGradArgs* crit, float* grads, float* dx, ru_stream_t stream) {
    if (!h->have_fwd || !h->training) { set_error("ru_unet_backward: needs a preceding training-mode ru_unet_forward"); return RU_ESTATE; }
    Arena A;
    A.dry = false; A.base = h->ws; A.cap = h->ws_bytes; A.off = h->fwd_end; A.keep = h->fwd_keep;
    ru::t_sink = h->probe_families ? h->sink : nullptr;
    h->red.main.e.clear();
    h->red.side.e.clear();
    ru::t_red = (h->fusion & RU_FUSE_BATCH_WREDUCE) && !trace_on() ? &h->red : nullptr;
    RU_REQUIRE(h->precision != RU_PREC_BF16X3 || h->pack_sig == conv3_sb_switch_signature(),
               "ru_unet_backward: RU_WZ / RU_MX / RU_MXG changed since the forward whose packs this backward reads (signature %d then, %d now)", h->pack_sig, conv3_sb_switch_signature());
    int rc = unet_backward_impl(h, params, dprobs, grads, dx, A, (hipStream_t)stream, crit);
    ru::t_red = nullptr;
    ru::t_sink = nullptr;
    if (rc && h->side) {
        (void)side_join(h, (hipStream_t)stream);
        h->fork_used = 0;
    }
    if (rc) return rc;
    if (A.failed) { set_error("ru_unet_backward: workspace too small"); return RU_ENOMEM; }
    return RU_OK;
}
extern "C" int ru_unet_backward_criterion(ru_unet_t h, const float* params, const float* target, const double* sums, double count,
                                          float w_dice, float w_bce, float bg_weight, float priority, float* grads, float* dx, ru_stream_t stream) {
    RU_REQUIRE(h && params && target && sums && grads && count > 0.0, "ru_unet_backward_criterion: null argument");
    const CritGradArgs cg{target, sums, count, w_dice, w_bce, bg_weight, priority};
    return backward_entry(h, params, nullptr, &cg, grads, dx, stream);
}

extern "C" int ru_unet_backward(ru_unet_t h, const float* params, const float* dprobs, float* grads, float* dx, ru_stream_t stream) {
    RU_REQUIRE(h && params && dprobs && grads, "ru_unet_backward: null argument");
    return backward_entry(h, params, dprobs, nullptr, grads, dx, stream);
}

extern "C" int ru_unet_gn_stats(ru_unet_t h, int idx, float* mean, float* rstd, ru_stream_t stream) {
    RU_REQUIRE(h && h->have_fwd, "ru_unet_gn_stats: no forward state");
    if (idx < 0) return (int)h->gn_order.size();
    RU_REQUIRE(idx < (int)h->gn_order.size() && mean && rstd, "ru_unet_gn_stats: bad index");
    const size_t bytes = (size_t)h->N * kGroups * sizeof(float);
    hipError_t e = hipMemcpyAsync(mean, h->gn_order[idx].mean, bytes, hipMemcpyDeviceToDevice, (hipStream_t)stream);
    if (e == hipSuccess) e = hipMemcpyAsync(rstd, h->gn_order[idx].rstd, bytes, hipMemcpyDeviceToDevice, (hipStream_t)stream);
    if (e != hipSuccess) return hip_fail(e, "ru_unet_gn_stats");
    return RU_OK;
}

extern "C" const char* ru_last_error(void) { return g_err; }
// ... 206 lines not shown
}

extern "C" int ru_groupnorm_bwd(const float* x, const float* gamma, const float* beta, const float* mean, const float* rstd, const float* dy,
                                float* dx, float* dgamma, float* dbeta, int N, int C, size_t V, int G, float slope,
                                void* ws, size_t ws_bytes, ru_stream_t stream) {
    RU_REQUIRE(x && gamma && beta && mean && rstd && dy && dx, "ru_groupnorm_bwd: null argument");
    RU_REQUIRE(C % G == 0, "ru_groupnorm_bwd: C %% G != 0");
    hipStream_t s = (hipStream_t)stream;
    WsCarver Cw(ws, ws_bytes);
    const int nblk = gn_bwd_tiles(V);
    float* part = Cw.take((size_t)N * C * nblk * 2);
    float* scale = Cw.take((size_t)N * C);
    float* shift = Cw.take((size_t)N * C);
    float* coef = Cw.take((size_t)N * C * 3);
    RU_WS_OK(Cw);
    hipLaunchKernelGGL(gn_scale_shift_kernel, dim3(cdiv(N * C, 256)), dim3(256), 0, s, gamma, beta, mean, rstd, scale, shift, N, C, G);
    RU_CHECK_LAUNCH("gn_scale_shift_kernel");
    int rc = gn_bwd_reduce_launch(x, dy, scale, shift, mean, rstd, slope, part, N, C, V, G, s);
    if (rc) return rc;
    rc = gn_bwd_finalize_launch(part, nblk, gamma, mean, rstd, coef, dgamma, dbeta, N, C, V, G, s);
    if (rc) return rc;
    return gn_bwd_apply_launch(x, dy, scale, shift, coef, slope, dx, N, C, V, s);
}

extern "C" int ru_leaky_relu_fwd(const float* x, float* y, size_t n, float slope, ru_stream_t stream) { return lrelu_fwd_launch(x, y, n, slope, (hipStream_t)stream); }
extern "C" int ru_leaky_relu_bwd(const float* y, const float* dy, float* dx, size_t n, float slope, ru_stream_t stream) { return lrelu_bwd_launch(y, dy, dx, n, slope, (hipStream_t)stream); }
extern "C" int ru_upsample2x_trilinear_fwd(const float* x, float* y, int N, int C, int D, int H, int W, ru_stream_t stream) { return up2_fwd_launch(x, y, N, C, D, H, W, (hipStream_t)stream); }
extern "C" int ru_upsample2x_trilinear_bwd(const float* dy, float* dx, int N, int C, int D, int H, int W, ru_stream_t stream) { return up2_bwd_launch(dy, dx, N, C, D, H, W, (hipStream_t)stream); }
extern "C" int ru_sigmoid_fwd(const float* x, float* y, size_t n, ru_stream_t stream) { return sigmoid_launch(x, y, n, (hipStream_t)stream); }

extern "C" size_t ru_criterion_workspace_bytes(int N, int C, size_t V) { return 4096 + (size_t)N * C * crit_tiles(V) * 3 * sizeof(float); }
extern "C" int ru_criterion_sums(const float* p, const float* g, double* sums, int N, int C, size_t V, float bg_weight, void* ws, size_t ws_bytes, ru_stream_t stream) {
    RU_REQUIRE(p && g && sums, "ru_criterion_sums: null argument");
    return crit_sums_launch(p, g, sums, N, C, V, bg_weight, ws, ws_bytes, (hipStream_t)stream);
}
extern "C" int ru_criterion_grad(const float* p, const float* g, const double* sums, double count, float w_dice, float w_bce, float bg_weight,
                                 float priority, float* dp, int N, int C, size_t V, ru_stream_t stream) {
    RU_REQUIRE(p && g && sums && dp && count > 0, "ru_criterion_grad: bad argument");
    return crit_grad_launch(p, g, sums, count, w_dice, w_bce, bg_weight, priority, dp, N, C, V, (hipStream_t)stream);
}
extern "C" int ru_criterion_value(const double* sums_host, int C, double count, double priority, double* dice, double* bce) {
    RU_REQUIRE(sums_host && C > 0 && count > 0, "ru_criterion_value: bad argument");
    double acc = 0.0;
    for (int c = 0; c < C; ++c) acc += 2.0 * (sums_host[c] + 1e-6) / (sums_host[C + c] + 2e-6);
    if (dice) *dice = priority * (1.0 - acc / C);
    if (bce) *bce = -sums_host[2 * C] / count;
    return RU_OK;
}
extern "C" int ru_criterion_value_device(const double* sums, int C, double count, double priority, double w_dice, double w_bce, double* out3,
                                         ru_stream_t stream) {
    RU_REQUIRE(sums && out3 && C > 0 && C <= 64 && count > 0, "ru_criterion_value_device: bad argument");
    return crit_value_launch(sums, C, count, priority, w_dice, w_bce, out3, (hipStream_t)stream);
}
extern "C" int ru_adam_amsgrad_step(float* w, const float* g, float* m, float* v, float* vmax, size_t n, float lr, float beta1, float beta2,
                                    float eps, float weight_decay, int step, ru_stream_t stream) {
    RU_REQUIRE(w && g && m && v && vmax, "ru_adam_amsgrad_step: null argument");
    return adam_launch(w, g, m, v, vmax, n, lr, beta1, beta2, eps, weight_decay, step, (hipStream_t)stream);
}

extern "C" int ru_adam_step(float* w, const float* g, float* m, float* v, float* vmax_or_null, size_t n, float lr, float beta1, float beta2,
                            float eps, float weight_decay, int step, ru_stream_t stream) {
    RU_REQUIRE(w && g && m && v, "ru_adam_step: null argument");
    return adam_launch(w, g, m, v, vmax_or_null, n, lr, beta1, beta2, eps, weight_decay, step, (hipStream_t)stream);
}

extern "C" int ru_tta_merge(const float* probs, int K, unsigned flips, float* mean_out, unsigned char* mask, unsigned long long* counts,
                            int C, int D, int H, int W, ru_stream_t stream) {
    RU_REQUIRE(probs && mask && counts, "ru_tta_merge: null argument");
    return tta_merge_launch(probs, K, flips, mean_out, mask, counts, C, D, H, W, (hipStream_t)stream);
}
extern "C" int ru_compose_labels(const unsigned char* mask, const unsigned long long* counts, unsigned long long et_min, unsigned char* labels,
                                 size_t V, ru_stream_t stream) {
    RU_REQUIRE(mask && counts && labels, "ru_compose_labels: null argument");
    return compose_labels_launch(mask, counts, et_min, labels, V, (hipStream_t)stream);
}

extern "C" int ru_dice_accumulate(const unsigned long long* counts, double* acc, int N, int C, int nacc, ru_stream_t stream) {
    return dice_accumulate_launch(counts, acc, N, C, nacc, (hipStream_t)stream);
}
extern "C" int ru_dice_counts(const float* p, const float* g, unsigned long long* counts, int N, int C, size_t V, ru_stream_t stream) {
    RU_REQUIRE(p && g && counts && N > 0 && C > 0, "ru_dice_counts: bad argument");
    return dice_counts_launch(p, g, counts, N * C, V, (hipStream_t)stream);
}

extern "C" int ru_layout_convert(const float* src, float* dst, int N, int C, size_t V, int to_c16, ru_stream_t stream) {
    RU_REQUIRE(src && dst && N > 0, "ru_layout_convert: bad argument");
    return layout_convert_launch(src, dst, N, C, V, to_c16, (hipStream_t)stream);
}

extern "C" int ru_upsample2x_trilinear_fwd_l(const float* x, float* y, int N, int C, int D, int H, int W, float out_slope, ru_stream_t stream) {
    RU_REQUIRE(x && y && N > 0 && C > 0 && D > 0 && H > 0 && W > 0, "ru_upsample2x_trilinear_fwd_l: bad argument");
    return up2_fwd16_launch(x, y, N, C, D, H, W, out_slope, (hipStream_t)stream);
}
extern "C" int ru_upsample2x_trilinear_bwd_l(const float* dy, float* dx, int N, int C, int D, int H, int W, ru_stream_t stream) {
    RU_REQUIRE(dy && dx && N > 0 && C > 0 && D > 0 && H > 0 && W > 0, "ru_upsample2x_trilinear_bwd_l: bad argument");
    return up2_bwd16_launch(dy, dx, N, C, D, H, W, (hipStream_t)stream);
}
extern "C" int ru_conv3d_fwd_l(const float* x, const float* w, const float* bias, float* y, int N, int Cin, int Cout, int D, int H, int W,
                               int flags, void* ws, size_t ws_bytes, ru_stream_t stream) {
    RU_REQUIRE(x && w && y, "ru_conv3d_fwd_l: null argument");
    hipStream_t s = (hipStream_t)stream;
    WsCarver C(ws, ws_bytes);
    Conv3Args a{};
    void* wf = C.take(conv3_sb_frag_bytes(Cin, Cout) / 4 + 64);
    RU_WS_OK(C);
    const bool f32 = (flags & 16) != 0;
// ... 79 lines not shown
```

brats2019_amd/csrc/pointwise.hip:

```cpp
#include "pw_helpers.hpp"

namespace ru {

template <int VEC, int COT>
__global__ __launch_bounds__(256) void conv1_kernel(const Conv1Args a) {
    const int n = blockIdx.z;
    const int co0 = blockIdx.y * COT;
    const size_t V = a.V;
    const size_t v = ((size_t)blockIdx.x * 256 + threadIdx.x) * VEC;
    if (v >= V) return;
    float acc[COT][VEC];
#pragma unroll
    for (int o = 0; o < COT; ++o)
#pragma unroll
        for (int k = 0; k < VEC; ++k) acc[o][k] = 0.f;
    int widx[COT];
#pragma unroll
    for (int o = 0; o < COT; ++o) widx[o] = (co0 + o < a.Cout) ? co0 + o : a.Cout - 1;

    const float* xp = a.x0 + (size_t)n * a.C0 * V + v;
    const float* wr = a.wT;
#pragma unroll 4
    for (int c = 0; c < a.C0; ++c) {
        float xv[VEC];
// ... 67 lines not shown
    const float* x0 = a.x0 + (size_t)n * a.C0 * V;
    const float* x1 = a.x1 ? a.x1 + (size_t)n * a.C1 * V : a.x0;
    auto cstep = [&](int c0) __attribute__((always_inline)) {
        const int c = c0 + k;
        const bool cok = c < Ct;
        const int cc = cok ? c : Ct - 1;
        const float av = cok ? a.wT[(size_t)cc * a.ldw + oa] : 0.f;
        const float* xp = cc < a.C0 ? x0 + (size_t)cc * V : x1 + (size_t)(cc - a.C0) * V;
        float bv[4];
#pragma unroll
        for (int t = 0; t < 4; ++t) bv[t] = xp[vb[t]];
#pragma unroll
        for (int t = 0; t < 4; ++t) acc[t] = __builtin_amdgcn_mfma_f32_16x16x4f32(av, bv[t], acc[t], 0, 0, 0);
    };
    int c0 = 0;
    for (; c0 + 12 < Ct; c0 += 16) { cstep(c0); cstep(c0 + 4); cstep(c0 + 8); cstep(c0 + 12); }
    for (; c0 < Ct; c0 += 4) cstep(c0);
#pragma unroll
    for (int t = 0; t < 4; ++t) {
        const size_t v = v0 + 16 * t + r;
        if (v >= V) continue;
#pragma unroll
        for (int q = 0; q < 4; ++q) {
            const int o = o0 + k * 4 + q;
            if (o >= a.Cout) continue;
            const size_t idx = ((size_t)n * a.Cout + o) * V + v;
            float y = lrelu(acc[t][q], a.out_slope);
            if (a.add) y += a.add[idx];
            a.y[idx] = y;
        }
    }
}

int conv1_launch(const Conv1Args& a, hipStream_t s) {
    RU_REQUIRE(a.N > 0 && a.C0 > 0 && a.Cout > 0 && a.V > 0 && a.ldw >= a.Cout, "conv1: bad shape");
    const bool vec = (a.V % 4) == 0;
    const long wg_big = (long)((a.V / 4 + 255) / 256) * cdiv(a.Cout, 16) * a.N;
    if (wg_big < 256 && a.C0 + a.C1 >= 32) {
        const int nvt = (int)((a.V + 63) / 64);
        dim3 grid((unsigned)cdiv(nvt, 4), (unsigned)cdiv(a.Cout, 16), (unsigned)a.N);
        hipLaunchKernelGGL(conv1_mfma_kernel, grid, dim3(256), 0, s, a, nvt);
    } else if (!vec || wg_big < 256) {
        dim3 grid((unsigned)((a.V + 255) / 256), (unsigned)cdiv(a.Cout, 4), (unsigned)a.N);
        hipLaunchKernelGGL((conv1_kernel<1, 4>), grid, dim3(256), 0, s, a);
    } else {
        dim3 grid((unsigned)((a.V / 4 + 255) / 256), (unsigned)cdiv(a.Cout, 16), (unsigned)a.N);
        hipLaunchKernelGGL((conv1_kernel<4, 16>), grid, dim3(256), 0, s, a);
    }
    RU_CHECK_LAUNCH("conv1_kernel");
    return RU_OK;
}

__global__ void transpose_kernel(const float* __restrict__ src, float* __restrict__ dst, int rows, int cols) {
    const int i = blockIdx.x * blockDim.x + threadIdx.x;
    if (i >= rows * cols) return;
    const int c = i / rows, r = i % rows;
    dst[i] = src[(size_t)r * cols + c];
}
int transpose_launch(const float* src, float* dst, int rows, int cols, hipStream_t s) {
    hipLaunchKernelGGL(transpose_kernel, dim3(cdiv(rows * cols, 256)), dim3(256), 0, s, src, dst, rows, cols);
    RU_CHECK_LAUNCH("transpose_kernel");
    return RU_OK;
}

__global__ __launch_bounds__(256) void s2d_kernel(const float* __restrict__ x, float* __restrict__ y, int NC, int D, int H, int W) {
    const int Do = D / 2, Ho = H / 2, Wo = W / 2;
    const size_t total = (size_t)NC * Do * Ho * Wo;
    const size_t Vo = (size_t)Do * Ho * Wo;
    for (size_t i = (size_t)blockIdx.x * blockDim.x + threadIdx.x; i < total; i += (size_t)gridDim.x * blockDim.x) {
        const int xo = (int)(i % Wo);
        size_t r = i / Wo;
        const int yo = (int)(r % Ho); r /= Ho;
        const int zo = (int)(r % Do);
        const size_t nc = r / Do;
        const float* xp = x + ((nc * D + 2 * zo) * H + 2 * yo) * (size_t)W + 2 * xo;
        float* yp = y + nc * 8 * Vo + ((size_t)zo * Ho + yo) * Wo + xo;
#pragma unroll
        for (int ij = 0; ij < 4; ++ij) {
            const float2 t = *reinterpret_cast<const float2*>(xp + ((size_t)(ij >> 1) * H + (ij & 1)) * W);
            yp[(size_t)(ij * 2) * Vo] = t.x;
            yp[(size_t)(ij * 2 + 1) * Vo] = t.y;
        }
    }
}
__global__ __launch_bounds__(256) void d2s_kernel(const float* __restrict__ y, float* __restrict__ x, int NC, int D, int H, int W) {
    const int Do = D / 2, Ho = H / 2, Wo = W / 2;
    const size_t total = (size_t)NC * Do * Ho * Wo;
    const size_t Vo = (size_t)Do * Ho * Wo;
    for (size_t i = (size_t)blockIdx.x * blockDim.x + threadIdx.x; i < total; i += (size_t)gridDim.x * blockDim.x) {
        const int xo = (int)(i % Wo);
        size_t r = i / Wo;
        const int yo = (int)(r % Ho); r /= Ho;
        const int zo = (int)(r % Do);
        const size_t nc = r / Do;
        float* xp = x + ((nc * D + 2 * zo) * H + 2 * yo) * (size_t)W + 2 * xo;
        const float* yp = y + nc * 8 * Vo + ((size_t)zo * Ho + yo) * Wo + xo;
#pragma unroll
        for (int ij = 0; ij < 4; ++ij) {
            float2 t;
            t.x = yp[(size_t)(ij * 2) * Vo];
            t.y = yp[(size_t)(ij * 2 + 1) * Vo];
            *reinterpret_cast<float2*>(xp + ((size_t)(ij >> 1) * H + (ij & 1)) * W) = t;
        }
    }
}
int s2d_launch(const float* x, float* y, int N, int C, int D, int H, int W, hipStream_t s) {
    RU_REQUIRE(D % 2 == 0 && H % 2 == 0 && W % 2 == 0, "s2d: extents must be even");
    const size_t total = (size_t)N * C * (D / 2) * (H / 2) * (W / 2);
    hipLaunchKernelGGL(s2d_kernel, dim3(grid1d(total, 256)), dim3(256), 0, s, x, y, N * C, D, H, W);
    RU_CHECK_LAUNCH("s2d_kernel");
// ... 609 lines not shown
int head_grad_c4_crit_launch(const float* p, const CritGradArgs& cg, float* d4, float* db, int N, int C, size_t V, void* ws, size_t ws_bytes, hipStream_t s) {
    RU_REQUIRE(C > 0 && C <= 4 && V % 4 == 0 && cg.target && cg.sums, "head_grad_c4_crit: 1..4 channels, V % 4 == 0, target and sums");
    if (!ws || ws_bytes < bias_grad_workspace_bytes(N, C, V)) { set_error("head_grad_c4_crit: workspace too small"); return RU_ENOMEM; }
    const int nblk = (int)((V + BG_CHUNK - 1) / BG_CHUNK);
    hipLaunchKernelGGL(head_grad_c4_kernel<true>, dim3(nblk, N), dim3(256), 0, s, p, cg.target, d4, (float*)ws, C, V, nblk, cg);
    RU_CHECK_LAUNCH("head_grad_c4_kernel<crit>");
    hipLaunchKernelGGL(bias_final_kernel, dim3(C), dim3(256), 0, s, (const float*)ws, db, N, C, nblk);
    RU_CHECK_LAUNCH("bias_final_kernel");
    return RU_OK;
}

constexpr int CR_CHUNK = 8192;
int crit_tiles(size_t V) { return (int)((V + CR_CHUNK - 1) / CR_CHUNK); }
__global__ __launch_bounds__(256) void crit_partial_kernel(const float* __restrict__ p, const float* __restrict__ g, float* __restrict__ part,
                                                           size_t V, int nblk, float bgw) {
    __shared__ float buf[4];
    const size_t row = blockIdx.y;
    const size_t v0 = (size_t)blockIdx.x * CR_CHUNK;
    const size_t v1 = v0 + CR_CHUNK < V ? v0 + CR_CHUNK : V;
    const float one_eps = (float)(1.0 + 1e-6);
    float si = 0.f, su = 0.f, sb = 0.f;
    for (size_t v = v0 + threadIdx.x; v < v1; v += 256) {
        const float pv = p[row * V + v], gv = g[row * V + v];
        si += pv * gv;
        su += pv * pv + gv;
        sb += gv * logf(pv + 1e-6f) + bgw * (1.f - gv) * logf(one_eps - pv);
    }
    si = block_sum(si, buf);
    su = block_sum(su, buf);
    sb = block_sum(sb, buf);
    if (threadIdx.x == 0) {
        float* q = part + (row * nblk + blockIdx.x) * 3;
        q[0] = si; q[1] = su; q[2] = sb;
    }
}
__global__ __launch_bounds__(256) void crit_final_kernel(const float* __restrict__ part, double* __restrict__ sums, int N, int C, int nblk) {
    __shared__ double buf[4];
    double bce = 0.0;
    for (int c = 0; c < C; ++c) {
        double si = 0.0, su = 0.0, sb = 0.0;
        for (int i = threadIdx.x; i < N * nblk; i += 256) {
            const int n = i / nblk, b = i % nblk;
            const float* q = part + (((size_t)n * C + c) * nblk + b) * 3;
            si += (double)q[0]; su += (double)q[1]; sb += (double)q[2];
        }
        si = block_sum_d(si, buf);
        su = block_sum_d(su, buf);
        sb = block_sum_d(sb, buf);
        if (threadIdx.x == 0) { sums[c] = si; sums[C + c] = su; }
        bce += sb;
    }
    if (threadIdx.x == 0) sums[2 * C] = bce;
}
int crit_sums_launch(const float* p, const float* g, double* sums, int N, int C, size_t V, float bgw, void* ws, size_t ws_bytes, hipStream_t s) {
    const int nblk = crit_tiles(V);
    if (!ws || ws_bytes < (size_t)N * C * nblk * 3 * sizeof(float)) { set_error("criterion: workspace too small"); return RU_ENOMEM; }
    hipLaunchKernelGGL(crit_partial_kernel, dim3(nblk, N * C), dim3(256), 0, s, p, g, (float*)ws, V, nblk, bgw);
    RU_CHECK_LAUNCH("crit_partial_kernel");
    hipLaunchKernelGGL(crit_final_kernel, dim3(1), dim3(256), 0, s, (const float*)ws, sums, N, C, nblk);
    RU_CHECK_LAUNCH("crit_final_kernel");
    return RU_OK;
}
__global__ void crit_value_kernel(const double* __restrict__ sums, int C, double count, double priority, double w_dice, double w_bce,
                                  double* __restrict__ out) {
    double q = threadIdx.x < (unsigned)C ? 2.0 * (sums[threadIdx.x] + 1e-6) / (sums[C + threadIdx.x] + 2e-6) : 0.0;
    for (int o = 32; o > 0; o >>= 1) q += __shfl_xor(q, o);
    if (threadIdx.x == 0) {
        const double dice = priority * (1.0 - q / C), bce = -sums[2 * C] / count;
        out[0] = w_dice * dice + w_bce * bce; out[1] = dice; out[2] = bce;
    }
}
int crit_value_launch(const double* sums, int C, double count, double priority, double w_dice, double w_bce, double* out3, hipStream_t s) {
    hipLaunchKernelGGL(crit_value_kernel, dim3(1), dim3(64), 0, s, sums, C, count, priority, w_dice, w_bce, out3);
    RU_CHECK_LAUNCH("crit_value_kernel");
    return RU_OK;
}
__global__ __launch_bounds__(256) void crit_grad_kernel(const float* __restrict__ p, const float* __restrict__ g, const double* __restrict__ sums,
                                                        double count, float w_dice, float w_bce, float bgw, float priority,
                                                        float* __restrict__ dp, int C, size_t V) {
    const size_t row = blockIdx.y;
    const int c = (int)(row % C);
    const double I = sums[c] + 1e-6, U = sums[C + c] + 2e-6;
    const double k = (double)priority * (2.0 / (double)C) * (double)w_dice;
    const float cg = (float)(-k / U), cp = (float)(2.0 * k * I / (U * U));
    const float cb = (float)((double)w_bce / count);
    const float one_eps = (float)(1.0 + 1e-6);
    for (size_t v = (size_t)blockIdx.x * 256 + threadIdx.x; v < V; v += (size_t)gridDim.x * 256) {
        const float pv = p[row * V + v], gv = g[row * V + v];
        const float bce = -(gv / (pv + 1e-6f) - bgw * (1.f - gv) / (one_eps - pv));
        dp[row * V + v] = (cg * gv + cp * pv) + cb * bce;
    }
}
int crit_grad_launch(const float* p, const float* g, const double* sums, double count, float w_dice, float w_bce,
                     float bgw, float priority, float* dp, int N, int C, size_t V, hipStream_t s) {
    hipLaunchKernelGGL(crit_grad_kernel, rows_grid(V, 1, N * C), dim3(256), 0, s, p, g, sums, count, w_dice, w_bce, bgw, priority, dp, C, V);
    RU_CHECK_LAUNCH("crit_grad_kernel");
    return RU_OK;
}

__global__ __launch_bounds__(256) void tta_merge_kernel(const float* __restrict__ p, int K, unsigned flips, float* __restrict__ mean_out,
                                                        unsigned char* __restrict__ mask_out, unsigned long long* __restrict__ counts,
                                                        int C, int D, int H, int W) {
    __shared__ unsigned int cnt[4];
    const size_t V = (size_t)D * H * W;
    const int c = blockIdx.y;
    if (threadIdx.x < 4) cnt[threadIdx.x] = 0;
    __syncthreads();
    unsigned int local = 0;
    for (size_t v = (size_t)blockIdx.x * 256 + threadIdx.x; v < V; v += (size_t)gridDim.x * 256) {
        const int x = (int)(v % W);
        const int y = (int)((v / W) % H);
        const int z = (int)(v / ((size_t)W * H));
        float acc = 0.f;
        for (int k = 0; k < K; ++k) {
            const unsigned f = (flips >> (3 * k)) & 7u;
            const int zz = (f & 1u) ? D - 1 - z : z, yy = (f & 2u) ? H - 1 - y : y, xx = (f & 4u) ? W - 1 - x : x;
            const float t = p[(((size_t)k * C + c) * D + zz) * H * W + (size_t)yy * W + xx];
            acc = k == 0 ? t : acc + t;
        }
        const float m = acc / (float)K;
        if (mean_out) mean_out[(size_t)c * V + v] = m;
        const bool on = m > 0.5f;
        mask_out[(size_t)c * V + v] = on ? 1 : 0;
// ... 233 lines not shown
            const float t = (float)(x - f);
            const size_t stride = ax == 0 ? HW : (ax == 1 ? (size_t)a.W : 1);
            off[ax][0] = (size_t)(reflect_idx(i0, a.P[ax]) + a.lo[ax]) * stride;
            off[ax][1] = (size_t)(reflect_idx(i0 + 1, a.P[ax]) + a.lo[ax]) * stride;
            wgt[ax][0] = 1.f - t;
            wgt[ax][1] = t;
        }
        float acc[RU_AUG_MAXC];
#pragma unroll
        for (int c = 0; c < RU_AUG_MAXC; ++c) acc[c] = 0.f;
        float cw1 = 0.f, cw2 = 0.f, cw3 = 0.f;
#pragma unroll
        for (int q = 0; q < 8; ++q) {
            const int qa = q >> 2, qb = (q >> 1) & 1, qc = q & 1;
            const float w = wgt[0][qa] * wgt[1][qb] * wgt[2][qc];
            const size_t v = off[0][qa] + off[1][qb] + off[2][qc];
#pragma unroll
            for (int c = 0; c < RU_AUG_MAXC; ++c)
                if (c < a.C) acc[c] += w * a.image[(size_t)c * DHW + v];
            if (SOFT) {
                cw1 += w * a.soft[v];
                cw2 += w * a.soft[DHW + v];
                cw3 += w * a.soft[2 * DHW + v];
            } else {
                const int l = a.label[v];
                cw1 += l == 1 ? w : 0.f;
                cw2 += l == 2 ? w : 0.f;
                cw3 += l == 3 ? w : 0.f;
            }
        }
#pragma unroll
        for (int c = 0; c < RU_AUG_MAXC; ++c)
            if (c < a.C) a.data[(size_t)c * total + o] = ((acc[c] - a.mean[c]) * a.istd[c]) * a.gain[c] + a.bias[c];
        if (SOFT) {
            a.target[o] = cw1;
            a.target[total + o] = cw2;
            a.target[2 * total + o] = cw3;
        } else {
            a.target[o] = (cw1 + cw2) + cw3;
            a.target[total + o] = cw1 + cw3;
            a.target[2 * total + o] = cw3;
        }
    }
}
int augment_patch_launch(const AugmentArgs& a, hipStream_t s) {
    const size_t total = (size_t)a.P[0] * a.P[1] * a.P[2];
    if (a.soft) hipLaunchKernelGGL(augment_patch_kernel<true>, dim3(grid1d(total, 256, 4096)), dim3(256), 0, s, a);
    else hipLaunchKernelGGL(augment_patch_kernel<false>, dim3(grid1d(total, 256, 4096)), dim3(256), 0, s, a);
    RU_CHECK_LAUNCH("augment_patch_kernel");
    return RU_OK;
}

template <bool AMS>
__global__ __launch_bounds__(256) void adam_kernel(float* __restrict__ w, const float* __restrict__ g, float* __restrict__ m, float* __restrict__ v,
                                                   float* __restrict__ vmax, size_t n, float step_size, float b1, float b2, float eps, float wd,
                                                   float bc2_sqrt) {
    for (size_t i = (size_t)blockIdx.x * 256 + threadIdx.x; i < n; i += (size_t)gridDim.x * 256) {
        const float wi = w[i];
        const float gi = g[i] + wd * wi;
        const float mi = m[i] + (gi - m[i]) * (1.f - b1);
        const float vi = v[i] * b2 + (1.f - b2) * gi * gi;
        float vm = vi;
        if (AMS) { vm = fmaxf(vmax[i], vi); vmax[i] = vm; }
        const float denom = sqrtf(vm) / bc2_sqrt + eps;
        m[i] = mi; v[i] = vi;
        w[i] = wi - step_size * (mi / denom);
    }
}
int adam_launch(float* w, const float* g, float* m, float* v, float* vmax, size_t n, float lr, float b1, float b2,
                float eps, float wd, int step, hipStream_t s) {
    if (n == 0) return RU_OK;
    RU_REQUIRE(step >= 1, "adam: step is 1-based");
    const double bc1 = 1.0 - pow((double)b1, (double)step), bc2 = 1.0 - pow((double)b2, (double)step);
    if (vmax) hipLaunchKernelGGL(adam_kernel<true>, dim3(grid1d(n, 256 * 4, 4096)), dim3(256), 0, s, w, g, m, v, vmax, n, (float)((double)lr / bc1), b1, b2, eps, wd,
                                 (float)sqrt(bc2));
    else hipLaunchKernelGGL(adam_kernel<false>, dim3(grid1d(n, 256 * 4, 4096)), dim3(256), 0, s, w, g, m, v, vmax, n, (float)((double)lr / bc1), b1, b2, eps, wd,
                            (float)sqrt(bc2));
    RU_CHECK_LAUNCH("adam_kernel");
    return RU_OK;
}

}
```

brats2019_amd/csrc/pointwise_c16.hip:

```cpp
#include "pw_helpers.hpp"
#include "fin_tail.hpp"
#include <type_traits>
#include <stdlib.h>

namespace ru {

typedef float f32x4_c16 __attribute__((ext_vector_type(4)));
template <int I, int N, class F> __device__ __forceinline__ void static_for_c1_impl(F&& f) {
    if constexpr (I < N) { f(std::integral_constant<int, I>{}); static_for_c1_impl<I + 1, N>(f); }
}
template <int N, class F> __device__ __forceinline__ void static_for_c1(F&& f) { static_for_c1_impl<0, N>(f); }

static inline dim3 c16_grid(size_t V, int blocks_nc, unsigned cap = 2048) {
    size_t bx = (V * 4 + 255) / 256;
    if (bx > cap) bx = cap;
    if (bx < 1) bx = 1;
    return dim3((unsigned)bx, (unsigned)blocks_nc);
}

template <int RES, bool NT = false>
__global__ __launch_bounds__(256) void gn_apply16_kernel(const float* __restrict__ x, const float* __restrict__ scale, const float* __restrict__ shift,
                                                         const float* __restrict__ res, float* __restrict__ y, int C, size_t V, float slope,
                                                         const float* __restrict__ rscale, const float* __restrict__ rshift, float rslope) {
    const int nb = blockIdx.y, CB = C >> 4;
// ... 257 lines not shown
        const int kx = (int)(r % W); r /= W;
        const int ky = (int)(r % H);
        const int k0 = (int)(r / H) * UP2B_ZC;
        const int k1 = k0 + UP2B_ZC < D ? k0 + UP2B_ZC : D;
        float wy[4], wx[4];
        size_t oy[4], ox[4];
#pragma unroll
        for (int t = 0; t < 4; ++t) {
            const int y = 2 * ky - 1 + t, xx = 2 * kx - 1 + t;
            wy[t] = (y >= 0 && y < Ho) ? up2_coef(y, H, ky) : 0.f;
            wx[t] = (xx >= 0 && xx < Wo) ? up2_coef(xx, W, kx) : 0.f;
            oy[t] = (size_t)(y < 0 ? 0 : (y >= Ho ? Ho - 1 : y)) * Wo;
            ox[t] = (size_t)(xx < 0 ? 0 : (xx >= Wo ? Wo - 1 : xx)) * 4 + q;
        }
        float4 accP = make_float4(0.f, 0.f, 0.f, 0.f), accC = accP;
        for (int m = k0; m <= k1; ++m) {
#pragma unroll
            for (int h = 0; h < 2; ++h) {
                const int z = 2 * m - 1 + h;
                const bool in = z >= 0 && z < Do;
                const size_t zrow = (size_t)(z < 0 ? 0 : (z >= Do ? Do - 1 : z)) * Ho * Wo;
                float4 pz = make_float4(0.f, 0.f, 0.f, 0.f);
#pragma unroll
                for (int b = 0; b < 4; ++b) {
                    const float4* row = dp + (zrow + oy[b]) * 4;
                    const float4 p0 = row[ox[0]], p1 = row[ox[1]], p2 = row[ox[2]], p3 = row[ox[3]];
                    pz.x += wy[b] * (wx[0] * p0.x + wx[1] * p1.x + wx[2] * p2.x + wx[3] * p3.x);
                    pz.y += wy[b] * (wx[0] * p0.y + wx[1] * p1.y + wx[2] * p2.y + wx[3] * p3.y);
                    pz.z += wy[b] * (wx[0] * p0.z + wx[1] * p1.z + wx[2] * p2.z + wx[3] * p3.z);
                    pz.w += wy[b] * (wx[0] * p0.w + wx[1] * p1.w + wx[2] * p2.w + wx[3] * p3.w);
                }
                const float cP = (in && m - 1 >= k0) ? up2_coef(z, D, m - 1) : 0.f;
                const float cC = (in && m < k1) ? up2_coef(z, D, m) : 0.f;
                accP.x += cP * pz.x; accP.y += cP * pz.y; accP.z += cP * pz.z; accP.w += cP * pz.w;
                accC.x += cC * pz.x; accC.y += cC * pz.y; accC.z += cC * pz.z; accC.w += cC * pz.w;
            }
            if (m - 1 >= k0) op[(((size_t)(m - 1) * H + ky) * W + kx) * 4 + q] = accP;
            accP = accC;
            accC = make_float4(0.f, 0.f, 0.f, 0.f);
        }
    }
}
int up2_bwd16_launch(const float* dy, float* dx, int N, int C, int D, int H, int W, hipStream_t s) {
    RU_REQUIRE(C % 16 == 0, "up2_bwd16: C must be a multiple of 16");
    const size_t total = (size_t)((D + UP2B_ZC - 1) / UP2B_ZC) * H * W * 4;
    size_t bx = (total + 255) / 256;
    if (bx > 16384) bx = 16384;
    hipLaunchKernelGGL(up2_bwd16_kernel, dim3((unsigned)bx, (unsigned)(N * (C / 16))), dim3(256), 0, s, dy, dx, D, H, W);
    RU_CHECK_LAUNCH("up2_bwd16_kernel");
    return RU_OK;
}

__global__ void pack_down16_kernel(const float* __restrict__ w, float* __restrict__ wd, float* __restrict__ wdT, int Cout, int Cin) {
    const int i = blockIdx.x * blockDim.x + threadIdx.x;
    if (i >= Cout * Cin * 8) return;
    const int tap = i & 7, c = (i >> 3) % Cin, o = i / (8 * Cin);
    const float v = w[i];
    wd[(size_t)o * 8 * Cin + tap * Cin + c] = v;
    wdT[(size_t)(tap * Cin + c) * Cout + o] = v;
}
int pack_down16_launch(const float* w, float* wd, float* wdT, int Cout, int Cin, hipStream_t s) {
    const int total = Cout * Cin * 8;
    hipLaunchKernelGGL(pack_down16_kernel, dim3(cdiv(total, 256)), dim3(256), 0, s, w, wd, wdT, Cout, Cin);
    RU_CHECK_LAUNCH("pack_down16_kernel");
    return RU_OK;
}

template <int COB, int S2D, int NSLOT, bool PAIR = false>
__global__ __launch_bounds__(256, (PAIR || NSLOT > 0) ? 2 : 1) void conv1_16_kernel(const Conv1Args a, int nvt) {
    static_assert(!PAIR || (S2D == 2 && COB == 4 && (NSLOT == 1 || NSLOT == 2)), "paired stores: the scatter mode with statistics, four blocks per workgroup");
    constexpr bool BST = NSLOT > 0;
    constexpr int NSL = BST ? NSLOT : 1;
    __shared__ float red[BST ? 4 * NSL * 16 * 2 : 1];
    const int lane = threadIdx.x & 63, wave = threadIdx.x >> 6;
    const int n = blockIdx.z, cog = blockIdx.y;
    const size_t V = a.V;
    const int r = lane & 15, g = lane >> 4;
    const int nkb0 = a.C0 >> 4, nkb1 = a.C1 >> 4, nkb = nkb0 + nkb1, CBo = a.Cout >> 4;
    const int Hf = 2 * a.Hc, Wf = 2 * a.Wc;
    const size_t Vf = V * 8;
    const int CBf_out = CBo >> 3;
    const int Cstat = S2D == 2 ? (a.Cout >> 3) : a.Cout;
    f32x4_c16 bs1[NSL], bs2[NSL], bk[NSL][3];
    if constexpr (BST) {
#pragma unroll
        for (int sl = 0; sl < NSL; ++sl) {
            bs1[sl] = f32x4_c16{0.f, 0.f, 0.f, 0.f}; bs2[sl] = f32x4_c16{0.f, 0.f, 0.f, 0.f};
            const int cob = cog * COB + sl, chb = S2D == 2 ? cob % CBf_out : cob;
            const float* kp = a.bst_k + (size_t)n * 3 * Cstat + (cob < CBo ? chb : 0) * 16 + 4 * g;
#pragma unroll
            for (int t3 = 0; t3 < 3; ++t3) { const float4 q = *reinterpret_cast<const float4*>(kp + (size_t)t3 * Cstat); bk[sl][t3] = f32x4_c16{q.x, q.y, q.z, q.w}; }
        }
    }
    const bool nt_out = (size_t)a.N * a.Cout * V * sizeof(float) >= ((size_t)128 << 20);
    const int vt = blockIdx.x * 4 + wave;
    const bool live = vt < nvt;
    if (!live) { if constexpr (!BST) return; }
    if (live) {
    const size_t v0 = (size_t)vt * 64;
    size_t vb[4], fv[4];
#pragma unroll
    for (int t = 0; t < 4; ++t) {
        size_t v = v0 + 16 * t + r;
        if (v >= V) v = V - 1;
        vb[t] = v * 16 + 4 * g;
        fv[t] = 0;
        if constexpr (S2D != 0) {
            const int xc = (int)(v % a.Wc);
            const size_t rr = v / a.Wc;
            const int yc = (int)(rr % a.Hc), zc = (int)(rr / a.Hc);
            fv[t] = ((size_t)(2 * zc) * Hf + 2 * yc) * Wf + 2 * xc;
        }
// ... 329 lines not shown
```

brats2019_amd/csrc/ru_common.h:

```cpp
#pragma once
#include <hip/hip_runtime.h>
#include <stddef.h>
#include <stdint.h>
#include <stdio.h>
#include <stdarg.h>

#include <vector>

#include "../../include/resunet_hip.h"

namespace ru {

typedef __bf16 ru_bf16x2 __attribute__((ext_vector_type(2)));
__device__ __forceinline__ void split_pair(float a, float b, unsigned& hb, unsigned& lb) {
    ru_bf16x2 h;
    h[0] = (__bf16)a;
    h[1] = (__bf16)b;
    hb = __builtin_bit_cast(unsigned, h);
    const float h0 = __builtin_bit_cast(float, __builtin_amdgcn_perm(hb, hb, 0x01000c0cu));
    const float h1 = __builtin_bit_cast(float, hb & 0xffff0000u);
    ru_bf16x2 l;
    l[0] = (__bf16)(a - h0);
    l[1] = (__bf16)(b - h1);
    lb = __builtin_bit_cast(unsigned, l);
}
__device__ __forceinline__ unsigned mxg_exponent_byte(unsigned biased_exponent_of_amax) {
    const int b = (int)biased_exponent_of_amax - 7;
    return (unsigned)(b < 9 ? 9 : b);
}
typedef short ru_s16x2 __attribute__((ext_vector_type(2)));
template <class V>
__device__ __forceinline__ float mxg_hi8(const float (&t)[8], V& hi, float (&lo)[8]) {
    float m = 0.f;
#pragma unroll
    for (int c = 0; c < 4; ++c) {
        ru_bf16x2 h;
        h[0] = (__bf16)t[2 * c];
        h[1] = (__bf16)t[2 * c + 1];
        const unsigned hb = __builtin_bit_cast(unsigned, h);
        hi[c] = hb;
        const float h0 = __builtin_bit_cast(float, __builtin_amdgcn_perm(hb, hb, 0x01000c0cu)), h1 = __builtin_bit_cast(float, hb & 0xffff0000u);
        lo[2 * c] = t[2 * c] - h0;
        lo[2 * c + 1] = t[2 * c + 1] - h1;
        m = fmaxf(m, fmaxf(fabsf(h0), fabsf(h1)));
    }
    return m;
}
__device__ __forceinline__ void mxg_cvt8(const float (&t)[8], const float (&lo)[8], float amax16, unsigned (&l8)[2], unsigned (&x8)[2]) {
    const unsigned b = mxg_exponent_byte((__builtin_bit_cast(unsigned, amax16) >> 23) & 0xffu);
    const float sc = __builtin_bit_cast(float, b << 23), sc8 = __builtin_bit_cast(float, (b - 8u) << 23);
#pragma unroll
    for (int d = 0; d < 2; ++d) {
        ru_s16x2 w = __builtin_amdgcn_cvt_scalef32_pk_fp8_f32(__builtin_bit_cast(ru_s16x2, lo[4 * d]), lo[4 * d], lo[4 * d + 1], sc8, false);
        w = __builtin_amdgcn_cvt_scalef32_pk_fp8_f32(w, lo[4 * d + 2], lo[4 * d + 3], sc8, true);
        l8[d] = __builtin_bit_cast(unsigned, w);
        ru_s16x2 v = __builtin_amdgcn_cvt_scalef32_pk_fp8_f32(__builtin_bit_cast(ru_s16x2, t[4 * d]), t[4 * d], t[4 * d + 1], sc, false);
        v = __builtin_amdgcn_cvt_scalef32_pk_fp8_f32(v, t[4 * d + 2], t[4 * d + 3], sc, true);
        x8[d] = __builtin_bit_cast(unsigned, v);
    }
}
template <int NP, class V>
__device__ __forceinline__ void split_n(const float (&t)[2 * NP], V& hi, V& lo) {
#pragma unroll
    for (int i = 0; i < NP; ++i) {
        unsigned hb, lb;
        split_pair(t[2 * i], t[2 * i + 1], hb, lb);
        hi[i] = hb;
        lo[i] = lb;
    }
}

void set_error(const char* fmt, ...);
int hip_fail(hipError_t e, const char* what);

#define RU_CHECK_LAUNCH(what)                                  \
    do {                                                       \
        hipError_t e__ = hipGetLastError();                    \
        if (e__ != hipSuccess) return ru::hip_fail(e__, what); \
    } while (0)

#define RU_REQUIRE(cond, ...)            \
    do {                                 \
        if (!(cond)) {                   \
            ru::set_error(__VA_ARGS__);  \
            return RU_EINVAL;            \
        }                                \
    } while (0)

struct PerDevice {
    bool done[64] = {};
    static int cur() { int d = 0; return (hipGetDevice(&d) == hipSuccess && d >= 0 && d < 64) ? d : -1; }
    bool get() const { const int d = cur(); return d >= 0 && done[d]; }
    void set() { const int d = cur(); if (d >= 0) done[d] = true; }
};

static inline size_t align_up(size_t v, size_t a) { return (v + a - 1) / a * a; }
static inline int cdiv(int a, int b) { return (a + b - 1) / b; }
static inline int round_up(int a, int b) { return cdiv(a, b) * b; }

struct Box3 { int lo[3], size[3]; };
static inline int make_box(Box3& b, const int* lo, const int* size, int D, int H, int W, const char* who) {
    const int dims[3] = {D, H, W};
    for (int a = 0; a < 3; ++a) {
        if (!(lo[a] >= 0 && size[a] > 0 && lo[a] + size[a] <= dims[a])) { set_error("%s: the box must lie inside the volume", who); return RU_EINVAL; }
        b.lo[a] = lo[a]; b.size[a] = size[a];
    }
    return RU_OK;
}

struct FinTail {
    unsigned* ticket;
    int kind;
    int nblk, N, C, G;
    size_t V;
    float eps;
    int s2_sign;
    const float* gamma;
    const float* beta;
    float* mean;
    float* rstd;
    float* scale;
    float* shift;
// ... 15 lines not shown
    float in_slope;
    const float* in_res;
    float* in_sum_out;
    float* stat_partials;
    int sigmoid;
    int N, Cin, Cout, D, H, W;
    int CinP, CoutP;
    int mode;
    const void* wfrag;
    int in_c16, out_c16;
    int in_s16;
    int in_g16;
    int in_c4;
    const float* bst_y;
    const float* bst_k;
    float bst_slope;
    int products;
    int ksplit;
    FinTail fin;
};
int conv3_f32_ksplit(int N, int Cin, int Cout, int D, int H, int W);
int sum_partials_launch(const float* part, int ksplit, size_t n, float* y, hipStream_t s);
int conv3_cin_pad(int Cin);
static inline int conv3_cout_pad(int Cout) { return round_up(Cout, 16); }
static inline int conv3_effective_mode(int mode, int W) { return (mode == RU_PREC_BF16X3 && (W & 3) == 0) ? RU_PREC_BF16X3 : RU_PREC_F32; }
int conv3_tiles_per_sample(int N, int Cin, int Cout, int D, int H, int W, int mode);
int conv3_launch(const Conv3Args& a, hipStream_t s);
size_t conv3_f32c_frag_bytes(int Cin_conv, int Cout_conv);
int conv3_f32c_pack_weights(const float* w, void* wfr, int Cin_f, int Cout_f, int mode, hipStream_t s);
int conv3_f32c_tiles_per_sample(int N, int Cin, int Cout, int D, int H, int W);
int conv3_f32c_launch(const Conv3Args& a, const void* wfr, hipStream_t s);
bool conv3_f32c_head_takes_residual(int Cin, int Cout, int W);
int conv3_sb_tiles_per_sample(int N, int Cin, int Cout, int D, int H, int W, int products = 3);
bool conv3_sb_head_form_enabled();
bool conv3_sb_uses_wz(int N, int Cin, int Cout, int D, int H, int W, int products);
bool conv3_sb_head_takes_residual(int N, int Cin, int Cout, int D, int H, int W);
int conv3_sb_launch(const Conv3Args& a, hipStream_t s);
size_t conv3_sb_frag_bytes(int Cin_conv, int Cout_conv);
size_t conv3_sb_frag_bytes_direct(int Cin_conv, int Cout_conv);
size_t conv3_sb4_frag_bytes(int Cout_conv);
int conv3_sb4_pack_weights(const float* w, void* wfrag, int Cin_f, int Cout_f, int mode, hipStream_t s);
bool conv3_sb4_usable(int N, int Cin, int Cout, int D, int H, int W);
int conv3_sb_pack_weights(const float* w, void* wfrag, int Cin_f, int Cout_f, int mode, hipStream_t s, bool grad_operand = false);
constexpr int RU_PACK_BATCH = 64;
struct SbPackEntry { const float* w; void* wfrag; int Cin_f, Cout_f, mode, nchunk, ncog, forms; };
struct SbPackBatch { SbPackEntry e[RU_PACK_BATCH]; int n; };
int conv3_sb_pack_add(SbPackBatch& b, const float* w, void* wfrag, int Cin_f, int Cout_f, int mode, bool all_forms, hipStream_t s, bool skip_direct = false);
int conv3_sb_switch_signature();
bool conv3_mxg_enabled();
bool conv3_mxg_usable(int N, int Cin, int Cout, int D, int H, int W);
int conv3_mxg_split_launch(const float* x, void* g16, size_t nvox, hipStream_t s);
bool conv3_sb_forward_skips_direct(int N, int Cin, int Cout, int D, int H, int W);
int conv3_sb_pack_batch(SbPackBatch& b, hipStream_t s);
int conv3_pack_weights(const float* w, float* wp, int Cin_f, int Cout_f, int mode, hipStream_t s);
size_t conv3_packed_floats(int Cin_conv, int Cout_conv);

struct Wgrad3Args {
    const float* x;
    const float* dy;
    const float* in_scale;
    const float* in_shift;
    float in_slope;
    float* dw;
    float* db;
    void* ws;
    size_t ws_bytes;
    int N, Cin, Cout, D, H, W;
    int mode;
    int x_c16, dy_c16;
    int dw_cin, dw_cout;
    int dy_s16;
    int x_c4, dy_c4;
    const float* gb_y;
    const float* gb_d;
    const float* gb_scale;
    const float* gb_shift;
    const float* gb_coef;
    float gb_slope;
    float* gb_out;
    int gb_g16;
    int products;
    int swapped;
    struct WgradRedList* defer;
};
size_t wgrad3_workspace_bytes(int N, int Cin, int Cout, int D, int H, int W);
int wgrad3_launch(const Wgrad3Args& a, hipStream_t s);
struct WgradRedEntry { const float* partials; float* dw; int nparts, taps, CoP, CiP, Cout, Cin, so, sc, split, flip, lo, blk0; };
struct WgradRedList { std::vector<WgradRedEntry> e; };
int wgrad_reduce_launch(const float* partials, int nparts, int taps, int CoP, int CiP, int Cout, int Cin, float* dw, int so, int sc, int split, hipStream_t s,
                        int flip_taps = 0, WgradRedList* defer = nullptr);
int wgrad_reduce_flush(WgradRedList& l, hipStream_t s);
size_t wgrad3_sb_workspace_bytes(int N, int Cin, int Cout, int D, int H, int W);
int wgrad3_sb_launch(const Wgrad3Args& a, hipStream_t s);
size_t wgrad3_tr_workspace_bytes(int N, int Cin, int Cout, int D, int H, int W);
int wgrad3_tr_launch(const Wgrad3Args& a, hipStream_t s);

struct Wgrad1Args {
    const float* x;
    const float* dy;
    float* dw;
    int ldw;
    void* ws;
    size_t ws_bytes;
    int N, Cin, Cout;
    size_t V;
    int c16;
// ... 37 lines not shown
int layout_convert_launch(const float* src, float* dst, int N, int C, size_t V, int to_c16, hipStream_t s);
int pad_to_c16_launch(const float* src, float* dst, int N, int C, size_t V, hipStream_t s);
int pad_to_c4_launch(const float* src, float* dst, int N, int C, size_t V, hipStream_t s);

int s2d_launch(const float* x, float* y, int N, int C, int D, int H, int W, hipStream_t s);
int d2s_launch(const float* y, float* x, int N, int C, int D, int H, int W, hipStream_t s);

int gn_stats_tiles(size_t V);
int gn_stats_launch(const float* x, float* partials, int N, int C, size_t V, hipStream_t s);
int gn_finalize_launch(const float* partials, int nblk, const float* gamma, const float* beta, float* mean, float* rstd,
                       float* scale, float* shift, int N, int C, size_t V, int G, float eps, hipStream_t s, float* bst_k = nullptr);
int gn_apply_launch(const float* x, const float* scale, const float* shift, const float* res, float* y,
                    int N, int C, size_t V, float slope, hipStream_t s);
int gn_bwd_tiles(size_t V);
int gn_bwd_reduce_launch(const float* x, const float* dy, const float* scale, const float* shift, const float* mean,
                         const float* rstd, float slope, float* partials, int N, int C, size_t V, int G, hipStream_t s);
int gn_bwd_finalize_launch(const float* partials, int nblk, const float* gamma, const float* mean, const float* rstd,
                           float* coef, float* dgamma, float* dbeta, int N, int C, size_t V, int G, hipStream_t s, int s2_sign = 0);
bool conv3_sb_bst_usable(int N, int Cout, int D, int H, int W);
int gn_bwd_apply_launch(const float* x, const float* dy, const float* scale, const float* shift, const float* coef,
                        float slope, float* dx, int N, int C, size_t V, hipStream_t s);

int lrelu_fwd_launch(const float* x, float* y, size_t n, float slope, hipStream_t s);
int lrelu_bwd_launch(const float* y, const float* dy, float* dx, size_t n, float slope, hipStream_t s);
int sigmoid_launch(const float* x, float* y, size_t n, hipStream_t s);
int sigmoid_bwd_launch(const float* p, const float* dp, float* dz, size_t n, hipStream_t s);
int add_launch(const float* a, const float* b, float* y, size_t n, hipStream_t s);
int fill_launch(float* p, float v, size_t n, hipStream_t s);
int up2_fwd_launch(const float* x, float* y, int N, int C, int D, int H, int W, hipStream_t s);
int up2_bwd_launch(const float* dy, float* dx, int N, int C, int D, int H, int W, hipStream_t s);
int bias_grad_launch(const float* dy, float* db, int N, int C, size_t V, void* ws, size_t ws_bytes, hipStream_t s);
size_t bias_grad_workspace_bytes(int N, int C, size_t V);
int head_grad_c4_launch(const float* p, const float* dp, float* d4, float* db, int N, int C, size_t V, void* ws, size_t ws_bytes, hipStream_t s);
struct CritGradArgs { const float* target; const double* sums; double count; float w_dice, w_bce, bgw, priority; };
int head_grad_c4_crit_launch(const float* p, const CritGradArgs& cg, float* d4, float* db, int N, int C, size_t V, void* ws, size_t ws_bytes, hipStream_t s);

int gn_apply16_launch(const float* x, const float* scale, const float* shift, const float* res, float* y, int N, int C, size_t V, float slope, hipStream_t s,
                      const float* rscale = nullptr, const float* rshift = nullptr, float rslope = 1.f);
int gn_bwd_tiles16(size_t V);
int gn_bwd_reduce16_launch(const float* x, const float* dy, const float* scale, const float* shift, const float* mean, const float* rstd,
                           float slope, float* partials, int N, int C, size_t V, int G, hipStream_t s, const FinTail* fin = nullptr);
int gn_bwd_apply16_launch(const float* x, const float* dy, const float* scale, const float* shift, const float* coef, float slope, float* dx,
                          int N, int C, size_t V, int split, hipStream_t s);
int up2_fwd16_launch(const float* x, float* y, int N, int C, int D, int H, int W, float slope, hipStream_t s);
int up2_bwd16_launch(const float* dy, float* dx, int N, int C, int D, int H, int W, hipStream_t s);
int pack_down16_launch(const float* w, float* wd, float* wdT, int Cout, int Cin, hipStream_t s);
int conv1_16_launch(const Conv1Args& a, hipStream_t s);

int crit_tiles(size_t total);
int crit_sums_launch(const float* p, const float* g, double* sums, int N, int C, size_t V, float bgw, void* ws, size_t ws_bytes, hipStream_t s);
int crit_grad_launch(const float* p, const float* g, const double* sums, double count, float w_dice, float w_bce,
                     float bgw, float priority, float* dp, int N, int C, size_t V, hipStream_t s);
int crit_value_launch(const double* sums, int C, double count, double priority, double w_dice, double w_bce, double* out3, hipStream_t s);
int tta_merge_launch(const float* p, int K, unsigned flips, float* mean_out, unsigned char* mask, unsigned long long* counts, int C, int D, int H, int W, hipStream_t s);
int compose_labels_launch(const unsigned char* mask, const unsigned long long* counts, unsigned long long et_min, unsigned char* labels, size_t V, hipStream_t s);
int dice_counts_launch(const float* p, const float* g, unsigned long long* counts, int rows, size_t V, hipStream_t s);
int dice_accumulate_launch(const unsigned long long* counts, double* acc, int N, int C, int nacc, hipStream_t s);
constexpr int RU_AUG_MAXC = 8;
struct AugmentArgs {
    const float* image;
    const unsigned char* label;
    const float* soft;
    float* data;
    float* target;
    int C, D, H, W;
    int lo[3], P[3];
    double scale[3];
    int flags;
    float mean[RU_AUG_MAXC], istd[RU_AUG_MAXC], gain[RU_AUG_MAXC], bias[RU_AUG_MAXC];
};
size_t zscore_workspace_bytes(int C, size_t V);
int zscore_stats_launch(const float* x, double* stats, int C, size_t V, void* ws, size_t ws_bytes, hipStream_t s);
int augment_patch_launch(const AugmentArgs& a, hipStream_t s);
int adam_launch(float* w, const float* g, float* m, float* v, float* vmax, size_t n, float lr, float b1, float b2,
                float eps, float wd, int step, hipStream_t s);

}
```

brats2019_amd/loss.py:

```python
from __future__ import annotations

import torch
import torch.nn as nn

from . import _lib, ops


def _all_reduce_sums(sums, group):
    import torch.distributed as dist
    if group is not False and dist.is_available() and dist.is_initialized():
        dist.all_reduce(sums, op=dist.ReduceOp.SUM, group=None if group in (None, True) else group)
        return dist.get_world_size(None if group in (None, True) else group)
    return 1


_HAND_OVER_DEPTH = 0


class hand_over_to_network:

    def __enter__(self):
        global _HAND_OVER_DEPTH
        _HAND_OVER_DEPTH += 1
        return self

    def __exit__(self, *exc):
        global _HAND_OVER_DEPTH
        _HAND_OVER_DEPTH -= 1
        return False


def _observed(pred):
    return bool(getattr(pred, "retains_grad", False)) or bool(getattr(pred, "_backward_hooks", None))


def _hand_over(pred, gt, sums, count, w_dice, w_bce, bg_weight, priority, gout):
    node = pred.grad_fn
    if node is None or not getattr(node, "accepts_criterion", False) or type(node).__name__ != "_UNetFnBackward":
        return None
    if getattr(node, "pending_criterion", None) is not None:
        pc, node.pending_criterion = node.pending_criterion, None
        first = ops.criterion_grad(pred, pc["target"], pc["sums"], pc["count"], pc["w_dice"], pc["w_bce"], pc["bg_weight"], pc["priority"]).mul_(pc["gout"].to(torch.float32))
        return first.add_(ops.criterion_grad(pred, gt, sums, count, w_dice, w_bce, bg_weight, priority).mul_(gout.to(torch.float32)))
    if _HAND_OVER_DEPTH <= 0 or _observed(pred):
        return None
    dummy = torch.zeros((), dtype=pred.dtype, device=pred.device).expand(pred.shape)
    node.pending_criterion = dict(target=gt, sums=sums, count=count, w_dice=w_dice, w_bce=w_bce, bg_weight=bg_weight, priority=priority, gout=gout, dummy=dummy)

    def _clear():
        node.pending_criterion = None
    torch.autograd.Variable._execution_engine.queue_callback(_clear)
    return dummy


class _CriterionFn(torch.autograd.Function):
    @staticmethod
    def forward(ctx, pred, gt, w_dice, w_bce, bg_weight, priority, group):
        sums = ops.criterion_sums(pred, gt, bg_weight)
        world = _all_reduce_sums(sums, group)
        count = float(pred.numel()) * world
        out = ops.criterion_losses(sums, count, priority, w_dice, w_bce)
        ctx.save_for_backward(pred, gt, sums)
        ctx.cfg = (count, w_dice, w_bce, bg_weight, priority)
        return out[0].to(torch.float32)

    @staticmethod
    def backward(ctx, gout):
        pred, gt, sums = ctx.saved_tensors
        count, w_dice, w_bce, bg_weight, priority = ctx.cfg
        dp = _hand_over(pred, gt, sums, count, w_dice, w_bce, bg_weight, priority, gout)
        if dp is None:
            dp = ops.criterion_grad(pred, gt, sums, count, w_dice, w_bce, bg_weight, priority)
            dp.mul_(gout.to(dp.dtype))
        return dp, None, None, None, None, None, None


class _PairFn(torch.autograd.Function):

    @staticmethod
    def forward(ctx, pred, gt, bg_weight, priority, group):
        sums = ops.criterion_sums(pred, gt, bg_weight)
        world = _all_reduce_sums(sums, group)
        count = float(pred.numel()) * world
        out = ops.criterion_losses(sums, count, priority, 0.5, 0.5).to(torch.float32)
        ctx.save_for_backward(pred, gt, sums)
        ctx.cfg = (count, bg_weight, priority)
        loss, dice, bce = out[0], out[1], out[2]
        ctx.mark_non_differentiable(dice, bce)
        return loss, dice, bce

    @staticmethod
    def backward(ctx, gout, _gd, _gb):
        pred, gt, sums = ctx.saved_tensors
        count, bg_weight, priority = ctx.cfg
        dp = _hand_over(pred, gt, sums, count, 0.5, 0.5, bg_weight, priority, gout)
        if dp is None:
            dp = ops.criterion_grad(pred, gt, sums, count, 0.5, 0.5, bg_weight, priority)
            dp.mul_(gout.to(dp.dtype))
        return dp, None, None, None, None


def fuse_criterion_list(criterion):
    if not isinstance(criterion, (tuple, list)) or len(criterion) != 2:
        return _fuse_terms(criterion)
    kinds = [type(c) for c in criterion]
    if sorted(k.__name__ for k in kinds) != ["BCE_Loss", "Dice_loss_joint"] or not all(k in (Dice_loss_joint, BCE_Loss) for k in kinds):
        return _fuse_terms(criterion)
    dice = criterion[0] if kinds[0] is Dice_loss_joint else criterion[1]
    bce = criterion[0] if kinds[0] is BCE_Loss else criterion[1]
    if dice.index != bce.label_index or dice.data_parallel != bce.data_parallel:
        return None
    dice_first = kinds[0] is Dice_loss_joint

    def run(x, y):
        assert x[dice.index].shape == y[dice.index].shape
        loss, d, b = _PairFn.apply(x[dice.index], y[dice.index], float(bce.bg_weight), float(dice.priority), dice.data_parallel)
        return loss, ([d, b] if dice_first else [b, d])
    return run


class _LossBase(nn.Module):

    def __init__(self):
        super().__init__()
        self.data_parallel = False

    def _run(self, x, y, index, w_dice, w_bce, bg_weight, priority):
        assert x[index].shape == y[index].shape
        return _CriterionFn.apply(x[index], y[index], w_dice, w_bce, bg_weight, priority, self.data_parallel)


class Dice_loss_joint(_LossBase):

    def __init__(self, index=0, priority=1):
        super().__init__()
        self.index = index
        self.priority = priority
# ... 135 lines not shown
```

brats2019_amd/ops.py:

```python
from __future__ import annotations

import ctypes as C

import torch

from . import _lib as L

LEAKY_SLOPE = 1e-2


def _dims5(x):
    if x.dim() != 5:
        raise ValueError("expected an NCDHW tensor, got shape %s" % (tuple(x.shape),))
    return [int(v) for v in x.shape]


def _prep(t):
    L.require_gpu()
    if t is None:
        return None
    return t.contiguous().float() if (not t.is_contiguous() or t.dtype != torch.float32) else t


def conv3d(x, w, bias=None, precision="f32"):
# ... 83 lines not shown
    x = _prep(x)
    n, c, d, h, w = _dims5(x)
    y = torch.empty((n, c, 2 * d, 2 * h, 2 * w), dtype=torch.float32, device=x.device)
    L.check(L.load().ru_upsample2x_trilinear_fwd(L.f32(x), L.f32(y), n, c, d, h, w, L.stream()), "ru_upsample2x_trilinear_fwd")
    return y


def upsample2x_bwd(dy):
    dy = _prep(dy)
    n, c, d2, h2, w2 = _dims5(dy)
    dx = torch.empty((n, c, d2 // 2, h2 // 2, w2 // 2), dtype=torch.float32, device=dy.device)
    L.check(L.load().ru_upsample2x_trilinear_bwd(L.f32(dy), L.f32(dx), n, c, d2 // 2, h2 // 2, w2 // 2, L.stream()),
            "ru_upsample2x_trilinear_bwd")
    return dx


def sigmoid(x):
    x = _prep(x)
    y = torch.empty_like(x)
    L.check(L.load().ru_sigmoid_fwd(L.f32(x), L.f32(y), x.numel(), L.stream()), "ru_sigmoid_fwd")
    return y


def criterion_sums(p, g, bg_weight=1e-2):
    p, g = _prep(p), _prep(g)
    if p.shape != g.shape:
        raise AssertionError("prediction/target shape mismatch")
    lib = L.load()
    n, c = int(p.shape[0]), int(p.shape[1])
    v = p.numel() // (n * c)
    sums = torch.empty(2 * c + 1, dtype=torch.float64, device=p.device)
    ws = L.workspace(lib.ru_criterion_workspace_bytes(n, c, v), p.device)
    L.check(lib.ru_criterion_sums(L.f32(p), L.f32(g), L.ptr(sums), n, c, v, bg_weight, L.ptr(ws), ws.numel(), L.stream()),
            "ru_criterion_sums")
    return sums


def criterion_grad(p, g, sums, count, w_dice=0.5, w_bce=0.5, bg_weight=1e-2, priority=1.0):
    p, g = _prep(p), _prep(g)
    n, c = int(p.shape[0]), int(p.shape[1])
    v = p.numel() // (n * c)
    dp = torch.empty_like(p)
    L.check(L.load().ru_criterion_grad(L.f32(p), L.f32(g), L.ptr(sums), float(count), w_dice, w_bce, bg_weight, priority,
                                       L.f32(dp), n, c, v, L.stream()), "ru_criterion_grad")
    return dp


def criterion_losses(sums, count, priority=1.0, w_dice=0.5, w_bce=0.5):
    c = (sums.numel() - 1) // 2
    out = torch.empty(3, dtype=torch.float64, device=sums.device)
    L.check(L.load().ru_criterion_value_device(L.ptr(sums), c, float(count), float(priority), float(w_dice), float(w_bce), L.ptr(out), L.stream()),
            "ru_criterion_value_device")
    return out


def criterion_value(sums, count, priority=1.0):
    out = criterion_losses(sums, count, priority)
    return out[1], out[2]


def _rows(p):
    n, c = int(p.shape[0]), int(p.shape[1])
    return n, c, p.numel() // max(n * c, 1)


def crit_moments(p, g, mask=L.CRIT_MASK_ALL):
    p, g = _prep(p), _prep(g)
    if p.shape != g.shape:
        raise AssertionError("prediction/target shape mismatch")
    lib = L.load()
    n, c, v = _rows(p)
    m = torch.empty((n, c, L.CRIT_MOMENTS), dtype=torch.float64, device=p.device)
    ws = L.workspace(lib.ru_crit_moments_workspace_bytes(n, c, v), p.device)
    L.check(lib.ru_crit_moments(L.f32(p), L.f32(g), n, c, v, int(mask), L.ptr(m), L.ptr(ws), ws.numel(), L.stream()), "ru_crit_moments")
    return m


def crit_reduce(moments):
    n, c = int(moments.shape[0]), int(moments.shape[1])
    out = torch.empty(c * L.CRIT_MOMENTS + 1, dtype=torch.float64, device=moments.device)
    L.check(L.load().ru_crit_reduce(L.ptr(moments), n, c, L.ptr(out), L.stream()), "ru_crit_reduce")
    return out


def crit_eval(totals, moments, terms, count, n_global):
    n, c = int(moments.shape[0]), int(moments.shape[1])
    arr = (L.CritTerm * max(len(terms), 1))(*[L.CritTerm(L.CRIT_KINDS[k], float(w), float(pr), float(bg)) for k, w, pr, bg in terms])
    values = torch.empty(1 + len(terms), dtype=torch.float64, device=moments.device)
    coef = torch.empty((n, c, 5), dtype=torch.float32, device=moments.device)
    L.check(L.load().ru_crit_eval(L.ptr(totals), L.ptr(moments), n, c, float(count), float(n_global), C.cast(arr, C.c_void_p), len(terms),
                                  L.ptr(values), L.ptr(coef), L.stream()), "ru_crit_eval")
    return values, coef


def crit_grad(p, g, coef, scale=None, with_logs=True):
    p, g = _prep(p), _prep(g)
    n, c, v = _rows(p)
    dp = torch.empty_like(p)
    sc = None if scale is None else scale.detach().to(torch.float32).contiguous()
    L.check(L.load().ru_crit_grad(L.f32(p), L.f32(g), L.ptr(coef), L.ptr(sc, True), n, c, v, int(bool(with_logs)), L.f32(dp), L.stream()),
            "ru_crit_grad")
    return dp


def adam_amsgrad_step(w, g, m, v, vmax, step, lr, betas=(0.9, 0.999), eps=1e-8, weight_decay=0.0):
    L.check(L.load().ru_adam_amsgrad_step(L.f32(w), L.f32(g), L.f32(m), L.f32(v), L.f32(vmax), w.numel(), lr, betas[0], betas[1],
# ... 629 lines not shown
```

brats2019_amd/optim.py:

```python
from __future__ import annotations

import torch

from . import _lib as L


class Adam(torch.optim.Optimizer):
    def __init__(self, params, lr=1e-3, betas=(0.9, 0.999), eps=1e-8, weight_decay=0, amsgrad=False, **unsupported):
        for k, v in unsupported.items():
            if k in ("foreach", "fused", "capturable", "differentiable", "maximize", "decoupled_weight_decay") and not v:
                continue
            raise NotImplementedError("brats2019_amd.optim.Adam: option %s=%r is not implemented by the HIP kernel" % (k, v))
        if not 0.0 <= lr:
            raise ValueError("Invalid learning rate: %r" % (lr,))
        if not 0.0 <= eps:
            raise ValueError("Invalid epsilon value: %r" % (eps,))
        if not (0.0 <= betas[0] < 1.0 and 0.0 <= betas[1] < 1.0):
            raise ValueError("Invalid beta parameters: %r" % (betas,))
        if not 0.0 <= weight_decay:
            raise ValueError("Invalid weight_decay value: %r" % (weight_decay,))
        super().__init__(params, dict(lr=lr, betas=betas, eps=eps, weight_decay=weight_decay, amsgrad=amsgrad))
        self._flat = {}

    def __setstate__(self, state):
        super().__setstate__(state)
        for group in self.param_groups:
            group.setdefault("amsgrad", False)
        self._flat = {}

    def load_state_dict(self, state_dict):
        super().load_state_dict(state_dict)
        self._flat = {}

    _KEYS = ("exp_avg", "exp_avg_sq", "max_exp_avg_sq")

    def _plan(self, gi, group):
        plan = self._flat.get(gi)
        params = [p for p in group["params"]]
        sig = (bool(group["amsgrad"]),) + tuple((p.data_ptr(), p.dtype, p.device) for p in params)
        if plan is not None and plan["sig"] == sig:
            return plan
        for p in params:
            if not p.is_cuda:
                raise RuntimeError("brats2019_amd.optim.Adam: parameters must live on a ROCm GPU (HIP-only path; no CPU fallback)")
            if p.dtype != torch.float32 or not p.is_contiguous():
                raise TypeError("brats2019_amd.optim.Adam: contiguous float32 parameters only")
        keys = self._KEYS if group["amsgrad"] else self._KEYS[:2]
        lo = min(p.data_ptr() for p in params)
        hi = max(p.data_ptr() + 4 * p.numel() for p in params)
        span = (hi - lo) // 4
        dev = params[0].device
        total = sum(p.numel() for p in params)
        flat_ok = span <= 2 * total + 1024 and all(p.device == dev for p in params)
        bufs = {k: torch.zeros(span if flat_ok else 0, dtype=torch.float32, device=dev) for k in keys}
        order = sorted(range(len(params)), key=lambda i: params[i].data_ptr())
        plan = dict(sig=sig, lo=lo, span=span, flat=flat_ok, bufs=bufs, order=order, keys=keys)
        for p in params:
            if p in self.state and self.state[p]:
                self._init_state(plan, p)
        self._flat[gi] = plan
        return plan

    def _init_state(self, plan, p):
        st = self.state[p]
        off = (p.data_ptr() - plan["lo"]) // 4
        for k in plan["keys"]:
            old = st.get(k)
            if plan["flat"]:
                view = plan["bufs"][k][off:off + p.numel()].view_as(p)
                if old is not None and old.data_ptr() != view.data_ptr():
                    view.copy_(old.to(device=p.device, dtype=torch.float32))
                st[k] = view
            elif old is None or not (old.is_cuda and old.dtype == torch.float32 and old.is_contiguous()):
                st[k] = torch.zeros_like(p, memory_format=torch.contiguous_format) if old is None else old.to(device=p.device, dtype=torch.float32).contiguous()
        if "step" not in st:
            st["step"] = torch.tensor(0.0, dtype=torch.float32)
        return st

    @torch.no_grad()
    def step(self, closure=None):
        loss = None
        if closure is not None:
            with torch.enable_grad():
                loss = closure()
        lib = L.load()
        stream = L.stream()
        for gi, group in enumerate(self.param_groups):
            params = group["params"]
            if not params:
                continue
            plan = self._plan(gi, group)
            ams = bool(group["amsgrad"])
            b1, b2 = group["betas"]
            lr = group["lr"]
            lr = float(lr.item()) if isinstance(lr, torch.Tensor) else float(lr)
            runs = []
            for i in plan["order"]:
                p = params[i]
                g = p.grad
                if g is None:
                    continue
                if g.is_sparse:
                    raise RuntimeError("Adam does not support sparse gradients")
                if not g.is_cuda or g.dtype != torch.float32 or not g.is_contiguous():
                    g = g.to(device=p.device, dtype=torch.float32).contiguous()
                    p.grad = g
                st = self.state[p]
                if "step" not in st or any(k not in st for k in plan["keys"]):
                    st = self._init_state(plan, p)
                stp = st["step"]
                k = int(stp.item() if isinstance(stp, torch.Tensor) else stp) + 1
                if isinstance(stp, torch.Tensor):
                    stp += 1
                else:
                    st["step"] = k
                n = p.numel()
                ptrs = (p.data_ptr(), g.data_ptr(), st["exp_avg"].data_ptr(), st["exp_avg_sq"].data_ptr(),
                        st["max_exp_avg_sq"].data_ptr() if ams else 0)
                if runs:
                    r = runs[-1]
                    if r[6] == k and all(r[j] + 4 * r[5] == ptrs[j] for j in range(4 + int(ams))):
                        r[5] += n
                        continue
                runs.append([ptrs[0], ptrs[1], ptrs[2], ptrs[3], ptrs[4], n, k])
            for w, g, m, v, vm, n, k in runs:
                L.check(lib.ru_adam_step(w, g, m, v, vm if ams else None, n, lr, float(b1), float(b2), float(group["eps"]),
                                         float(group["weight_decay"]), k, stream), "ru_adam_step")
            self.__dict__["last_launches"] = len(runs)
        return loss
```

brats2019_amd/parallel.py:

```python
from __future__ import annotations

import math

import torch
import torch.distributed as dist


class HipBackend:

    def __init__(self, cfg=None, device=None, precision=None, grad_precision=None):
        from . import _lib as L
        from .engine import UNetEngine, DEFAULT_CFG
        from .model import default_precision
        L.require_gpu()
        self.cfg = dict(cfg or DEFAULT_CFG)
        self.engine = UNetEngine(precision=precision or default_precision(self.cfg["number_of_channels"]), **self.cfg)
        if grad_precision:
            self.engine.set_grad_precision(grad_precision)
        self.device = torch.device(device if device is not None else "cuda:%d" % torch.cuda.current_device())
        self.total = self.engine.layout.total
        self.live_segments = []
        for _name, (shape, off, dead) in self.engine.layout.entries.items():
            n = 1
            for d in shape:
                n *= d
            if dead:
                continue
            if self.live_segments and self.live_segments[-1][1] == off:
                self.live_segments[-1][1] = off + n
            else:
                self.live_segments.append([off, off + n])

        self.reduce_runs = merge_runs(self.live_segments)

    def new_flat(self, fill=0.0):
        return torch.full((self.total,), float(fill), dtype=torch.float32, device=self.device)

    def forward(self, flat, x, training=True):
        return self.engine.forward(flat, x, training=training)

    def criterion_sums(self, probs, target, bg_weight):
        from . import ops
        return ops.criterion_sums(probs, target, bg_weight)

    def criterion_losses(self, sums, count, priority):
        from . import ops
        out = ops.criterion_losses(sums, count, priority, 0.5, 0.5)
        return out[0], out[1], out[2]

    def criterion_grad(self, probs, target, sums, count, bg_weight, priority):
        from . import ops
        return ops.criterion_grad(probs, target, sums, count, 0.5, 0.5, bg_weight, priority)

    def backward(self, flat, dprobs, grads):
        return self.engine.backward(flat, dprobs, flat_grads=grads)

    def backward_criterion(self, flat, target, sums, count, bg_weight, priority, grads):
        return self.engine.backward_criterion(flat, target, sums, count, 0.5, 0.5, bg_weight, priority, flat_grads=grads)

    def adam(self, flat, grads, m, v, vmax, step, lr, betas, eps, weight_decay):
        from . import ops
        for a, b in self.live_segments:
            ops.adam_amsgrad_step(flat[a:b], grads[a:b], m[a:b], v[a:b], vmax[a:b], step, lr, betas, eps, weight_decay)


def merge_runs(runs, max_gap=1 << 16):
    out = []
    for a, e in runs:
        if out and a - out[-1][1] <= max_gap:
            out[-1][1] = e
        else:
            out.append([a, e])
    return out


class RcclComm:

    def __init__(self, rank, world, unique_id=None, group=None):
        import ctypes as C
        from . import _lib as L
        L.require_gpu()
        lib = L.load()
        self.rank, self.world = int(rank), int(world)
        if unique_id is None:
            buf = (C.c_char * 128)()
            if self.rank == 0:
                L.check(lib.ru_comm_unique_id(C.cast(buf, C.c_void_p)), "ru_comm_unique_id")
            box = [bytes(buf)]
            if self.world > 1:
                if not (dist.is_available() and dist.is_initialized()):
                    raise RuntimeError("RcclComm: pass unique_id, or initialise torch.distributed so that rank 0 can broadcast it")
                dist.broadcast_object_list(box, src=0, group=group)
            unique_id = box[0]
        self.unique_id = bytes(unique_id)
        h = C.c_void_p()
        idbuf = C.create_string_buffer(self.unique_id, 128)
        L.check(lib.ru_comm_init(C.byref(h), C.cast(idbuf, C.c_void_p), self.rank, self.world), "ru_comm_init")
        self.h = h

    def all_reduce(self, t):
        from . import _lib as L
        if t.dtype not in (torch.float32, torch.float64):
            raise TypeError("RcclComm.all_reduce: float32 or float64, got %s" % t.dtype)
        L.check(L.load().ru_allreduce(self.h, L.ptr(t), t.numel(), 0 if t.dtype == torch.float32 else 1, L.stream()), "ru_allreduce")
        return t

    def all_reduce_many(self, tensors):
        from . import _lib as L
        if len(tensors) <= 1:
            for t in tensors:
                self.all_reduce(t)
            return
        lib = L.load()
        L.check(lib.ru_comm_group_begin(), "ru_comm_group_begin")
        try:
            for t in tensors:
# ... 4 lines not shown
        L.check(lib.ru_comm_group_end(), "ru_comm_group_end")

    def close(self):
        from . import _lib as L
        if getattr(self, "h", None):
            L.load().ru_comm_destroy(self.h)
            self.h = None

    def __del__(self):
        try:
            self.close()
        except Exception:
            pass


class DataParallelStep:

    def __init__(self, backend, flat_params, lr=2e-5, betas=(0.9, 0.999), eps=1e-8, weight_decay=1e-6,
                 step_size=16000, gamma=0.5, bg_weight=1e-2, priority=1.0, process_group=None, comm=None):
        self.backend = backend
        self.flat = flat_params
        self.grads = torch.zeros_like(flat_params)
        self.m = torch.zeros_like(flat_params)
        self.v = torch.zeros_like(flat_params)
        self.vmax = torch.zeros_like(flat_params)
        self.base_lr, self.betas, self.eps, self.weight_decay = lr, betas, eps, weight_decay
        self.step_size, self.gamma = step_size, gamma
        self.bg_weight, self.priority = bg_weight, priority
        self.group = process_group
        self.global_step = 0
        self.comm = comm
        self.fuse_criterion_grad = True
        self.comm_probe = None
        if comm is not None:
            self.distributed, self.world, self.rank = True, comm.world, comm.rank
        else:
            self.distributed = dist.is_available() and dist.is_initialized()
            self.world = dist.get_world_size(self.group) if self.distributed else 1
            self.rank = dist.get_rank(self.group) if self.distributed else 0

    @staticmethod
    def shard(batch_size, rank, world):
        if batch_size % world != 0:
            raise ValueError("global batch %d is not divisible by world size %d" % (batch_size, world))
        per = batch_size // world
        return slice(rank * per, (rank + 1) * per)

    def lr(self):
        return self.base_lr * self.gamma ** (self.global_step // self.step_size)

    def loss_and_grads(self, x_shard, target_shard):
        b = self.backend
        probs = b.forward(self.flat, x_shard, training=True)
        sums = b.criterion_sums(probs, target_shard, self.bg_weight)
        if self.distributed:
            self._all_reduce(sums)
        count = float(probs.numel()) * self.world
        loss, dice, bce = b.criterion_losses(sums, count, self.priority)
        if self.fuse_criterion_grad and hasattr(b, "backward_criterion"):
            b.backward_criterion(self.flat, target_shard, sums, count, self.bg_weight, self.priority, self.grads)
        else:
            dprobs = b.criterion_grad(probs, target_shard, sums, count, self.bg_weight, self.priority)
            b.backward(self.flat, dprobs, self.grads)
        if self.distributed:
            segs = getattr(b, "reduce_runs", None) or getattr(b, "live_segments", None)
            if segs and sum(e - a for a, e in segs) < 0.9 * self.grads.numel():
                self._all_reduce_many([self.grads[a:e] for a, e in segs])
            else:
                self._all_reduce(self.grads)
        self.last_probs = probs
        return loss, dice, bce

    def _probed(self, what, fn):
        if self.comm_probe is None:
            return fn()
        e0, e1 = torch.cuda.Event(enable_timing=True), torch.cuda.Event(enable_timing=True)
        e0.record()
        fn()
        e1.record()
        self.comm_probe.append((what, e0, e1))

    def _all_reduce(self, t):
        if self.comm is not None:
            self._probed("criterion_sums" if t.numel() < 64 else "gradients", lambda: self.comm.all_reduce(t))
        else:
            self._probed("criterion_sums" if t.numel() < 64 else "gradients", lambda: dist.all_reduce(t, op=dist.ReduceOp.SUM, group=self.group))

    def _all_reduce_many(self, tensors):
        if self.comm is not None:
            self._probed("gradients", lambda: self.comm.all_reduce_many(tensors))
        else:
            self._probed("gradients", lambda: all_reduce_coalesced(tensors, self.group))

    def step(self, x_shard, target_shard):
        loss, dice, bce = self.loss_and_grads(x_shard, target_shard)
        self.global_step += 1
        lr = self.base_lr * self.gamma ** ((self.global_step - 1) // self.step_size)
        self.backend.adam(self.flat, self.grads, self.m, self.v, self.vmax, self.global_step, lr, self.betas, self.eps, self.weight_decay)
        return loss, dice, bce

    def state_dict(self):
        return dict(m=self.m, v=self.v, vmax=self.vmax, global_step=self.global_step)

    def load_state_dict(self, sd):
        self.m.copy_(sd["m"]); self.v.copy_(sd["v"]); self.vmax.copy_(sd["vmax"])
        self.global_step = int(sd["global_step"])


def all_reduce_coalesced(tensors, group=None):
    if len(tensors) == 1 or (tensors[0].is_cuda and dist.get_backend(group) == "gloo"):
        for t in tensors:
# ... 119 lines not shown
```

include/resunet_hip.h:

```cpp
#ifndef RESUNET_HIP_H_
#define RESUNET_HIP_H_

#include <stddef.h>
#include <stdint.h>

#ifdef __cplusplus
extern "C" {
#endif

#define RU_OK 0
#define RU_EINVAL (-1)
#define RU_ENOMEM (-2)
#define RU_EHIP (-3)
#define RU_ESTATE (-4)

#define RU_PREC_F32 0
#define RU_PREC_BF16X3 1
#define RU_PREC_BF16 2

typedef void* ru_stream_t;
typedef struct ru_unet* ru_unet_t;

const char* ru_last_error(void);
int ru_version(void);
int ru_device_ok(void);

size_t ru_conv3d_workspace_bytes(int N, int Cin, int Cout, int D, int H, int W, int k);
int ru_conv3d_fwd(const float* x, const float* w, const float* bias, float* y,
                  int N, int Cin, int Cout, int D, int H, int W, int k,
                  void* ws, size_t ws_bytes, ru_stream_t stream);
int ru_conv3d_fwd_p(const float* x, const float* w, const float* bias, float* y,
                    int N, int Cin, int Cout, int D, int H, int W, int k, int precision,
                    void* ws, size_t ws_bytes, ru_stream_t stream);
int ru_conv3d_bwd_data_p(const float* dy, const float* w, float* dx,
                         int N, int Cin, int Cout, int D, int H, int W, int k, int precision,
                         void* ws, size_t ws_bytes, ru_stream_t stream);
int ru_conv3d_bwd_weight_p(const float* x, const float* dy, float* dw, float* db,
                           int N, int Cin, int Cout, int D, int H, int W, int k, int precision,
                           void* ws, size_t ws_bytes, ru_stream_t stream);
int ru_conv3d_bwd_data(const float* dy, const float* w, float* dx,
                       int N, int Cin, int Cout, int D, int H, int W, int k,
                       void* ws, size_t ws_bytes, ru_stream_t stream);
int ru_conv3d_bwd_weight(const float* x, const float* dy, float* dw, float* db,
                         int N, int Cin, int Cout, int D, int H, int W, int k,
                         void* ws, size_t ws_bytes, ru_stream_t stream);

size_t ru_groupnorm_workspace_bytes(int N, int C, size_t V);
int ru_groupnorm_fwd(const float* x, const float* gamma, const float* beta, const float* residual, float* y,
                     float* mean, float* rstd, int N, int C, size_t V, int G, float eps, float slope,
                     void* ws, size_t ws_bytes, ru_stream_t stream);
int ru_groupnorm_bwd(const float* x, const float* gamma, const float* beta, const float* mean, const float* rstd,
                     const float* dy, float* dx, float* dgamma, float* dbeta,
                     int N, int C, size_t V, int G, float slope,
                     void* ws, size_t ws_bytes, ru_stream_t stream);

int ru_leaky_relu_fwd(const float* x, float* y, size_t n, float slope, ru_stream_t stream);
int ru_leaky_relu_bwd(const float* y, const float* dy, float* dx, size_t n, float slope, ru_stream_t stream);

int ru_upsample2x_trilinear_fwd(const float* x, float* y, int N, int C, int D, int H, int W, ru_stream_t stream);
int ru_upsample2x_trilinear_bwd(const float* dy, float* dx, int N, int C, int D, int H, int W, ru_stream_t stream);

int ru_sigmoid_fwd(const float* x, float* y, size_t n, ru_stream_t stream);

size_t ru_criterion_workspace_bytes(int N, int C, size_t V);
int ru_criterion_sums(const float* p, const float* g, double* sums, int N, int C, size_t V, float bg_weight,
                      void* ws, size_t ws_bytes, ru_stream_t stream);
int ru_criterion_grad(const float* p, const float* g, const double* sums, double count,
                      float w_dice, float w_bce, float bg_weight, float priority,
                      float* dp, int N, int C, size_t V, ru_stream_t stream);
int ru_criterion_value(const double* sums_host, int C, double count, double priority, double* dice, double* bce);
int ru_criterion_value_device(const double* sums, int C, double count, double priority, double w_dice, double w_bce,
                              double* out3, ru_stream_t stream);

#define RU_CRIT_DICE_JOINT 0
#define RU_CRIT_BCE 1
#define RU_CRIT_MSE 2
#define RU_CRIT_CE 3
#define RU_CRIT_DICE1D 4
#define RU_CRIT_GDL_JOINT 5
#define RU_CRIT_SENS_JOINT 6
#define RU_CRIT_DICE_SEPARATE 7
#define RU_CRIT_NUM_KINDS 8
#define RU_CRIT_MAX_TERMS 8
#define RU_CRIT_M_PG 0
#define RU_CRIT_M_PP 1
#define RU_CRIT_M_P 2
#define RU_CRIT_M_G 3
#define RU_CRIT_M_GLOGP 4
#define RU_CRIT_M_QLOGQ 5
#define RU_CRIT_M_D2 6
#define RU_CRIT_MOMENTS 7
#define RU_CRIT_MASK_ALL 0x7fu
typedef struct {
    int kind;
    double weight;
    double priority;
    double bg_weight;
} ru_crit_term_t;
size_t ru_crit_moments_workspace_bytes(int N, int C, size_t V);
int ru_crit_moments(const float* p, const float* g, int N, int C, size_t V, unsigned mask, double* moments,
                    void* ws, size_t ws_bytes, ru_stream_t stream);
int ru_crit_reduce(const double* moments, int N, int C, double* out, ru_stream_t stream);
int ru_crit_eval(const double* totals, const double* moments, int N, int C, double count, double n_global,
                 const ru_crit_term_t* terms, int nterms, double* values, float* coef, ru_stream_t stream);
int ru_crit_grad(const float* p, const float* g, const float* coef, const float* scale, int N, int C, size_t V, int with_logs,
                 float* dp, ru_stream_t stream);

int ru_adam_amsgrad_step(float* w, const float* g, float* m, float* v, float* vmax, size_t n,
                         float lr, float beta1, float beta2, float eps, float weight_decay, int step,
                         ru_stream_t stream);
int ru_adam_step(float* w, const float* g, float* m, float* v, float* vmax_or_null, size_t n,
                 float lr, float beta1, float beta2, float eps, float weight_decay, int step,
                 ru_stream_t stream);

ru_unet_t ru_unet_create(int depth, const int* encoder_layers, const int* decoder_layers,
                         const int* number_of_channels, int number_of_outputs);
void ru_unet_destroy(ru_unet_t h);
int ru_unet_set_precision(ru_unet_t h, int precision);
int ru_unet_freeze_params(ru_unet_t h, int frozen);
int ru_unet_get_precision(ru_unet_t h);
int ru_unet_set_grad_precision(ru_unet_t h, int precision);
int ru_unet_get_grad_precision(ru_unet_t h);
#define RU_FUSE_GN_BWD_STATS 1
#define RU_FUSE_GN_BWD_APPLY 2
#define RU_FUSE_SIDE_STREAM 4
#define RU_FUSE_BATCH_WREDUCE 8
#define RU_FUSE_TAIL_FINALIZE 16
#define RU_FUSE_PW_DGRAD 32
int ru_unet_set_fusion(ru_unet_t h, unsigned mask);
int ru_unet_probe(ru_unet_t h, int enable);
int ru_unet_probe_read(ru_unet_t h, double* total_ms, int* launches);
#define RU_PROBE_FAMILIES 7
#define RU_PROBE_INSTANCES 7
int ru_unet_probe_read_families(ru_unet_t h, double* ms, int* launches, int nfam);
int ru_unet_param_count(ru_unet_t h);
const char* ru_unet_param_name(ru_unet_t h, int i);
int ru_unet_param_ndim(ru_unet_t h, int i);
int ru_unet_param_dim(ru_unet_t h, int i, int d);
size_t ru_unet_param_offset(ru_unet_t h, int i);
size_t ru_unet_param_total(ru_unet_t h);
int ru_unet_param_is_dead(ru_unet_t h, int i);
size_t ru_unet_workspace_bytes(ru_unet_t h, int N, int D, int H, int W, int training);
int ru_unet_forward(ru_unet_t h, const float* params, const float* x, float* probs,
                    int N, int D, int H, int W, int training,
                    void* ws, size_t ws_bytes, ru_stream_t stream);
int ru_unet_backward(ru_unet_t h, const float* params, const float* dprobs, float* grads, float* dx,
                     ru_stream_t stream);
int ru_unet_backward_criterion(ru_unet_t h, const float* params, const float* target, const double* sums, double count,
                               float w_dice, float w_bce, float bg_weight, float priority, float* grads, float* dx,
                               ru_stream_t stream);
int ru_unet_gn_stats(ru_unet_t h, int idx, float* mean, float* rstd, ru_stream_t stream);

typedef struct ru_comm* ru_comm_t;
#define RU_COMM_ID_BYTES 128
#define RU_DT_F32 0
#define RU_DT_F64 1
int ru_comm_unique_id(void* id_out );
int ru_comm_init(ru_comm_t* out, const void* id, int rank, int world);
int ru_comm_destroy(ru_comm_t c);
int ru_comm_rank(ru_comm_t c);
int ru_comm_world(ru_comm_t c);
int ru_allreduce(ru_comm_t c, void* buf, size_t count, int dtype, ru_stream_t stream);
int ru_comm_group_begin(void);
int ru_comm_group_end(void);

int ru_tta_merge(const float* probs, int K, unsigned flips, float* mean_out, unsigned char* mask, unsigned long long* counts,
// ... 143 lines not shown
```

Baseline: 269.1.

## Batch weight packs, fuse criterion sums+losses, multi-run Adam, overlap packing on side stream

Folds the down16 and transpose weight packs into the existing batched pack kernel, which cuts the per-step launch count. It adds an opt-in path (RU_PACK_ASIDE) that runs packing, the grad zero-fill and the head weight pack on a side stream, overlapping them with the stem or head work. Criterion sums and loss evaluation are fused into one call, and Adam updates over multiple parameter runs go out as one launch per eight runs. Together these target launch and host overhead, at the cost of extra stream fork/join bookkeeping.

```diff
diff --git a/brats2019_amd/_lib.py b/brats2019_amd/_lib.py
--- a/brats2019_amd/_lib.py
+++ b/brats2019_amd/_lib.py
@@ -46,6 +46,9 @@
     "ru_crit_grad": (_i, [_vp, _vp, _vp, _vp, _i, _i, _sz, _i, _vp, _vp]),
     "ru_adam_amsgrad_step": (_i, [_vp] * 5 + [_sz] + [_f] * 5 + [_i, _vp]),
     "ru_adam_step": (_i, [_vp] * 5 + [_sz] + [_f] * 5 + [_i, _vp]),
+    "ru_adam_step_runs": (_i, [_vp] * 6 + [_i] + [_f] * 5 + [_i, _vp]),
+    "ru_weight_packs": (_i, [_vp] * 5 + [_i, _i, _vp]),
+    "ru_criterion_sums_losses": (_i, [_vp, _vp, _vp, _i, _i, _sz, _f, _d, _d, _d, _d, _vp, _vp, _sz, _vp]),
     "ru_unet_create": (_vp, [_i, C.POINTER(_i), C.POINTER(_i), C.POINTER(_i), _i]),
     "ru_unet_destroy": (None, [_vp]),
     "ru_unet_set_precision": (_i, [_vp, _i]),
@@ -160,6 +163,10 @@
     _fields_ = [("kind", _i), ("weight", _d), ("priority", _d), ("bg_weight", _d)]
 
 
+def has(name):
+    return hasattr(load(), name)
+
+
 def load():
     global _lib
     if _lib is not None:
diff --git a/brats2019_amd/csrc/conv3_sb.hip b/brats2019_amd/csrc/conv3_sb.hip
--- a/brats2019_amd/csrc/conv3_sb.hip
+++ b/brats2019_amd/csrc/conv3_sb.hip
@@ -602,14 +602,21 @@
 }
 __global__ void conv3_sb_pack_batch_kernel(const SbPackBatch b) {
     const SbPackEntry& e = b.e[blockIdx.y];
-    sb_pack_both(e.w, reinterpret_cast<u32x4*>(e.wfrag), e.Cin_f, e.Cout_f, e.mode, e.nchunk, e.ncog, e.forms, blockIdx.x * blockDim.x + threadIdx.x);
+    const int i = blockIdx.x * blockDim.x + threadIdx.x;
+    if (e.mode == SB_PACK_DOWN16) { pack_down16_one(e.w, (float*)e.wfrag, (float*)e.wfrag + (size_t)8 * e.Cin_f * e.Cout_f, e.Cout_f, e.Cin_f, i); return; }
+    if (e.mode == SB_PACK_TRANSPOSE) { transpose_one(e.w, (float*)e.wfrag, e.Cout_f, e.Cin_f, i); return; }
+    sb_pack_both(e.w, reinterpret_cast<u32x4*>(e.wfrag), e.Cin_f, e.Cout_f, e.mode, e.nchunk, e.ncog, e.forms, i);
+}
+static inline int sb_entry_threads(const SbPackEntry& e) {
+    if (e.mode == SB_PACK_DOWN16) return e.Cout_f * e.Cin_f * 8;
+    if (e.mode == SB_PACK_TRANSPOSE) return e.Cout_f * e.Cin_f;
+    return sb_pack_threads(e.mode == 0 ? e.Cin_f : e.Cout_f, e.mode == 0 ? e.Cout_f : e.Cin_f, e.forms);
 }
 int conv3_sb_pack_batch(SbPackBatch& b, hipStream_t s) {
     if (b.n == 0) return RU_OK;
     int maxtotal = 0;
     for (int i = 0; i < b.n; ++i) {
-        const SbPackEntry& e = b.e[i];
-        const int t = sb_pack_threads(e.mode == 0 ? e.Cin_f : e.Cout_f, e.mode == 0 ? e.Cout_f : e.Cin_f, e.forms);
+        const int t = sb_entry_threads(b.e[i]);
         if (t > maxtotal) maxtotal = t;
     }
     hipLaunchKernelGGL(conv3_sb_pack_batch_kernel, dim3(cdiv(maxtotal, 256), b.n), dim3(256), 0, s, b);
@@ -633,6 +640,15 @@
     e.forms = all_forms ? SB_FORMS_ALL : (sb_pack_forms(mode) | ((skip_direct && mode == 0) ? 16 : 0));
     return RU_OK;
 }
+
+static int sb_pack_add_plain(SbPackBatch& b, const float* src, float* dst, int rows, int cols, int mode, hipStream_t s) {
+    if (b.n == RU_PACK_BATCH) { const int rc = conv3_sb_pack_batch(b, s); if (rc) return rc; }
+    SbPackEntry& e = b.e[b.n++];
+    e.w = src; e.wfrag = dst; e.Cin_f = cols; e.Cout_f = rows; e.mode = mode; e.nchunk = 0; e.ncog = 0; e.forms = 0;
+    return RU_OK;
+}
+int conv3_sb_pack_add_down16(SbPackBatch& b, const float* w, float* wd, int Cout, int Cin, hipStream_t s) { return sb_pack_add_plain(b, w, wd, Cout, Cin, SB_PACK_DOWN16, s); }
+int conv3_sb_pack_add_transpose(SbPackBatch& b, const float* src, float* dst, int rows, int cols, hipStream_t s) { return sb_pack_add_plain(b, src, dst, rows, cols, SB_PACK_TRANSPOSE, s); }
 
 size_t conv3_sb_frag_bytes_direct(int Cin_conv, int Cout_conv) {
     return (size_t)cdiv(Cout_conv, 16) * cdiv(Cin_conv, 16) * SB_KSTEPS * 2 * 64 * 16;
diff --git a/brats2019_amd/csrc/engine.hip b/brats2019_amd/csrc/engine.hip
--- a/brats2019_amd/csrc/engine.hip
+++ b/brats2019_amd/csrc/engine.hip
@@ -106,17 +106,18 @@
     k.used += 2;
 }
 
-#define RU_RUN(call)                      \
+#define RU_RUN_ON(call, st)               \
     do {                                  \
         if (!A.dry) {                     \
             if (A.failed) { set_error("workspace too small"); return RU_ENOMEM; } \
-            if (t_sink) sink_begin(#call, s); \
+            if (t_sink) sink_begin(#call, st); \
             const int rc__ = (call);      \
-            if (t_sink) sink_end(s);      \
+            if (t_sink) sink_end(st);     \
             if (rc__ != RU_OK) return rc__; \
-            if (trace_on()) { const int rt__ = trace_sync(#call, s); if (rt__ != RU_OK) return rt__; } \
+            if (trace_on()) { const int rt__ = trace_sync(#call, st); if (rt__ != RU_OK) return rt__; } \
         }                                 \
     } while (0)
+#define RU_RUN(call) RU_RUN_ON(call, s)
 
 __global__ void gn_scale_shift_kernel(const float* __restrict__ gamma, const float* __restrict__ beta, const float* __restrict__ mean,
                                       const float* __restrict__ rstd, float* __restrict__ scale, float* __restrict__ shift, int N, int C, int G) {
@@ -220,6 +221,7 @@
     std::vector<hipEvent_t> probe_ev;
     size_t probe_used = 0;
     hipStream_t side = nullptr;
+    bool pack_aside = false;
     std::vector<hipEvent_t> fork_ev;
     ru::RedQueues red;
     unsigned* tickets = nullptr;
@@ -303,6 +305,7 @@
     }
     ru_unet* h = new ru_unet();
     if (const char* e = getenv("RU_SIDE_STREAM")) { if (*e == '0') h->fusion &= ~(unsigned)RU_FUSE_SIDE_STREAM; }
+    if (const char* e = getenv("RU_PACK_ASIDE")) { if (*e) h->pack_aside = *e != '0'; }
     if (const char* e = getenv("RU_FUSION_OFF")) h->fusion &= ~(unsigned)strtoul(e, nullptr, 0);
     if (const char* e = getenv("RU_FUSION_ON")) h->fusion |= (unsigned)strtoul(e, nullptr, 0) & 63u;
     h->depth = depth;
@@ -432,6 +435,12 @@
 static inline const float* P(const ru_unet* h, const float* params, int idx) { return params ? params + h->params[idx].offset : nullptr; }
 static inline float* G(const ru_unet* h, float* grads, int idx) { return grads ? grads + h->params[idx].offset : nullptr; }
 
+static int side_fork(ru_unet* h, hipStream_t main);
+static int side_join(ru_unet* h, hipStream_t main, bool last = true);
+static bool weights_aside(const ru_unet* h, const Arena& A) {
+    return !A.dry && h->pack_aside && (h->fusion & RU_FUSE_SIDE_STREAM) && h->c16 && h->precision == RU_PREC_BF16X3 && !trace_on();
+}
+
 static int pack_all(ru_unet* h, const float* params, Arena& A, hipStream_t s) {
     float* pk = h->pack;
     SbPackBatch batch;
@@ -452,8 +461,8 @@
             rc = pack3(b.conv2, b.pk_d2, b.fk_d2, b.c, b.c, 1); if (rc) return rc;
         }
         if (b.down >= 0) {
-            if (h->c16) RU_RUN(pack_down16_launch(P(h, params, b.down), pk + b.pk_down16, pk + b.pk_down16 + (size_t)8 * b.cin_down * b.c, b.c, b.cin_down, s));
-            else RU_RUN(transpose_launch(P(h, params, b.down), pk + b.pk_downT, b.c, 8 * b.cin_down, s));
+            if (h->c16) RU_RUN(conv3_sb_pack_add_down16(batch, P(h, params, b.down), pk + b.pk_down16, b.c, b.cin_down, s));
+            else RU_RUN(conv3_sb_pack_add_transpose(batch, P(h, params, b.down), pk + b.pk_downT, b.c, 8 * b.cin_down, s));
         }
         return RU_OK;
     };
@@ -465,8 +474,8 @@
     for (int i = 0; i < h->depth - 1; ++i) for (auto& b : h->dec_blocks[i]) { int rc = blk(b, i); if (rc) return rc; }
     for (int i = 0; i < h->depth - 1; ++i) {
         if (h->c16 && !h->training) continue;
-        RU_RUN(transpose_launch(P(h, params, h->up_w[i]), pk + h->pk_upT[i], h->ch[i], h->ch[i + 1], s));
-        RU_RUN(transpose_launch(P(h, params, h->dec1_w[i]), pk + h->pk_decT[i], h->ch[i], 2 * h->ch[i], s));
+        RU_RUN(conv3_sb_pack_add_transpose(batch, P(h, params, h->up_w[i]), pk + h->pk_upT[i], h->ch[i], h->ch[i + 1], s));
+        RU_RUN(conv3_sb_pack_add_transpose(batch, P(h, params, h->dec1_w[i]), pk + h->pk_decT[i], h->ch[i], 2 * h->ch[i], s));
     }
     RU_RUN(conv3_sb_pack_batch(batch, s));
     return RU_OK;
@@ -604,8 +613,11 @@
     const bool reuse_packs = h->params_frozen && !h->training && !A.dry && h->packed_params == params && h->packed_base == (const void*)h->pack &&
                              h->packed_prec == h->precision && h->packed_c16 == h->c16;
     int rc = RU_OK;
+    const bool stem4 = h->c16 && h->precision == RU_PREC_BF16X3 && conv3_sb4_usable(N, kInCh, h->ch[0], Dl[0], Hl[0], Wl[0]);
+    const bool packs_aside = !reuse_packs && stem4 && weights_aside(h, A);
     if (!reuse_packs) {
-        rc = pack_all(h, params, A, s);
+        if (packs_aside) { rc = side_fork(h, s); if (rc) return rc; }
+        rc = pack_all(h, params, A, packs_aside ? h->side : s);
         if (rc) return rc;
     }
 
@@ -616,7 +628,7 @@
     h->x_in4_planned = false;
     h->y0 = A.alloc((size_t)N * C0 * Vl(0));
     const size_t stem_mark = A.off;
-    if (h->c16 && h->precision == RU_PREC_BF16X3 && conv3_sb4_usable(N, kInCh, C0, Dl[0], Hl[0], Wl[0])) {
+    if (stem4) {
         float* x4 = A.alloc((size_t)N * 4 * Vl(0));
         float* wf4 = wf4_in;
         h->x_in4 = x4;
@@ -629,6 +641,7 @@
         rc = conv3_gn(h, A, s, x, h->pack + h->pk_in, h->fpack + h->fk_in, h->y0, nullptr, P(h, params, h->nin_w), P(h, params, h->nin_b), h->g0, N, kInCh, C0, Dl[0], Hl[0], Wl[0], false);
     }
     if (rc) return rc;
+    if (packs_aside) { rc = side_join(h, s, false); if (rc) return rc; }
     if (!h->training) A.rewind(stem_mark);
     h->g0.act_slope = 1.0f;
     const bool stem_fused = h->c16 && !h->first_blocks.empty() && h->first_blocks[0].down < 0;
@@ -839,14 +852,14 @@
     if (er == hipSuccess) er = hipStreamWaitEvent(h->side, e, 0);
     return er == hipSuccess ? RU_OK : hip_fail(er, "side_fork");
 }
-static int side_join(ru_unet* h, hipStream_t main) {
+static int side_join(ru_unet* h, hipStream_t main, bool last) {
     if (!h->side || h->fork_used == 0) return RU_OK;
     hipEvent_t e;
     int rc = side_event(h, &e);
     if (rc) return rc;
     hipError_t er = hipEventRecord(e, h->side);
     if (er == hipSuccess) er = hipStreamWaitEvent(main, e, 0);
-    h->fork_used = 0;
+    if (last) h->fork_used = 0;
     return er == hipSuccess ? RU_OK : hip_fail(er, "side_join");
 }
 
@@ -966,9 +979,14 @@
     auto Vl = [&](int i) { return (size_t)Dl[i] * Hl[i] * Wl[i]; };
     const int C0 = h->ch[0];
     t_hint_c = C0;
-    RU_RUN(fill_launch(grads, 0.f, h->total, s));
     const bool c16 = h->c16;
     const bool head4 = c16 && conv3_sb4_usable(N, h->nout, C0, Dl[0], Hl[0], Wl[0]);
+    float* wf4 = head4 ? A.alloc(conv3_sb4_frag_bytes(C0) / sizeof(float) + 64) : nullptr;
+    const bool aside0 = weights_aside(h, A) && h->params[h->conv_out_b].offset + h->params[h->conv_out_b].numel == h->total;
+    hipStream_t s0 = s;
+    if (aside0) { const int rf = side_fork(h, s); if (rf) return rf; s0 = h->side; }
+    RU_RUN_ON(fill_launch(grads, 0.f, aside0 ? h->params[h->conv_out_b].offset : h->total, s0), s0);
+    if (head4) RU_RUN_ON(conv3_sb4_pack_weights(P(h, params, h->conv_out_w), wf4, C0, h->nout, 1, s0), s0);
     float* d4 = head4 ? A.alloc((size_t)N * 4 * Vl(0)) : nullptr;
     const bool need_dlog = !head4 || C0 > 16;
     float* dlog = need_dlog ? A.alloc((size_t)N * h->nout * Vl(0)) : nullptr;
@@ -989,6 +1007,7 @@
         RU_RUN(sigmoid_bwd_launch(h->probs, dprobs, dlog, (size_t)N * h->nout * Vl(0), s));
         RU_RUN(bias_grad_launch(dlog, G(h, grads, h->conv_out_b), N, h->nout, Vl(0), wsp, wsb, s));
     }
+    if (aside0) { const int rj = side_join(h, s, false); if (rj) return rj; }
     int rc = wgrad3_run(A, s, h->wgrad_mode(), h->head_in, nullptr, dlog, G(h, grads, h->conv_out_w), N, C0, h->nout, Dl[0], Hl[0], Wl[0], c16, false,
                         C0 <= 16 ? d4 : nullptr);
     if (rc) return rc;
@@ -996,8 +1015,6 @@
     Conv3Args dh{};
     dh.x = dlog; dh.wp = h->pack + h->pk_out_d; dh.y = dcur_buf; dh.mode = h->precision; dh.wfrag = h->fpack + h->fk_out_d; dh.out_c16 = c16; dh.N = N; dh.Cin = h->nout; dh.Cout = C0; dh.D = Dl[0]; dh.H = Hl[0]; dh.W = Wl[0];
     if (head4) {
-        float* wf4 = A.alloc(conv3_sb4_frag_bytes(C0) / sizeof(float) + 64);
-        RU_RUN(conv3_sb4_pack_weights(P(h, params, h->conv_out_w), wf4, C0, h->nout, 1, s));
         dh.x = d4; dh.wfrag = wf4; dh.in_c4 = 1;
     }
     const bool no_bst = !(h->fusion & RU_FUSE_GN_BWD_STATS);
@@ -1221,9 +1238,14 @@
         if (e != hipSuccess) return hip_fail(e, "ru_unet_forward: ticket words");
     }
     h->ticket_next = 0;
+    h->fork_used = 0;
     ru::t_sink = h->probe_families ? h->sink : nullptr;
     rc = unet_forward_impl(h, params, x, probs, A, (hipStream_t)stream);
     ru::t_sink = nullptr;
+    if (rc && h->side) {
+        (void)side_join(h, (hipStream_t)stream);
+        h->fork_used = 0;
+    }
     if (rc) return rc;
     if (A.failed) { set_error("ru_unet_forward: workspace too small (%zu bytes given)", ws_bytes); return RU_ENOMEM; }
     h->fwd_end = A.off;
@@ -1536,6 +1558,37 @@
     RU_REQUIRE(sums && out3 && C > 0 && C <= 64 && count > 0, "ru_criterion_value_device: bad argument");
     return crit_value_launch(sums, C, count, priority, w_dice, w_bce, out3, (hipStream_t)stream);
 }
+extern "C" int ru_criterion_sums_losses(const float* p, const float* g, double* sums, int N, int C, size_t V, float bg_weight, double count, double priority,
+                                        double w_dice, double w_bce, double* out3, void* ws, size_t ws_bytes, ru_stream_t stream) {
+    RU_REQUIRE(p && g && sums && out3 && C > 0 && C <= 64 && count > 0, "ru_criterion_sums_losses: bad argument");
+    return crit_sums_value_launch(p, g, sums, N, C, V, bg_weight, ws, ws_bytes, count, priority, w_dice, w_bce, out3, (hipStream_t)stream);
+}
+extern "C" int ru_adam_step_runs(float* const* w, const float* const* g, float* const* m, float* const* v, float* const* vmax_or_null, const size_t* n, int nruns,
+                                 float lr, float beta1, float beta2, float eps, float weight_decay, int step, ru_stream_t stream) {
+    RU_REQUIRE(w && g && m && v && n && nruns >= 1 && nruns <= RU_ADAM_RUNS, "ru_adam_step_runs: null argument or not 1..%d runs", (int)RU_ADAM_RUNS);
+    AdamRuns r{};
+    r.nruns = nruns;
+    for (int k = 0; k < nruns; ++k) {
+        RU_REQUIRE(w[k] && g[k] && m[k] && v[k] && (!vmax_or_null || vmax_or_null[k]), "ru_adam_step_runs: null run %d", k);
+        r.w[k] = w[k]; r.g[k] = g[k]; r.m[k] = m[k]; r.v[k] = v[k]; r.vmax[k] = vmax_or_null ? vmax_or_null[k] : nullptr; r.n[k] = n[k];
+    }
+    return adam_runs_launch(r, vmax_or_null != nullptr, lr, beta1, beta2, eps, weight_decay, step, (hipStream_t)stream);
+}
+extern "C" int ru_weight_packs(const float* const* src, float* const* dst, const int* rows, const int* cols, const int* kind, int n, int batched, ru_stream_t stream) {
+    RU_REQUIRE(src && dst && rows && cols && kind && n >= 0, "ru_weight_packs: null argument");
+    hipStream_t s = (hipStream_t)stream;
+    SbPackBatch batch;
+    batch.n = 0;
+    for (int i = 0; i < n; ++i) {
+        RU_REQUIRE(src[i] && dst[i] && rows[i] > 0 && cols[i] > 0 && (kind[i] == SB_PACK_DOWN16 || kind[i] == SB_PACK_TRANSPOSE), "ru_weight_packs: bad entry %d", i);
+        int rc;
+        if (kind[i] == SB_PACK_DOWN16) rc = batched ? conv3_sb_pack_add_down16(batch, src[i], dst[i], rows[i], cols[i], s)
+                                                    : pack_down16_launch(src[i], dst[i], dst[i] + (size_t)8 * rows[i] * cols[i], rows[i], cols[i], s);
+        else rc = batched ? conv3_sb_pack_add_transpose(batch, src[i], dst[i], rows[i], cols[i], s) : transpose_launch(src[i], dst[i], rows[i], cols[i], s);
+        if (rc) return rc;
+    }
+    return conv3_sb_pack_batch(batch, s);
+}
 extern "C" int ru_adam_amsgrad_step(float* w, const float* g, float* m, float* v, float* vmax, size_t n, float lr, float beta1, float beta2,
                                     float eps, float weight_decay, int step, ru_stream_t stream) {
     RU_REQUIRE(w && g && m && v && vmax, "ru_adam_amsgrad_step: null argument");
diff --git a/brats2019_amd/csrc/pointwise.hip b/brats2019_amd/csrc/pointwise.hip
--- a/brats2019_amd/csrc/pointwise.hip
+++ b/brats2019_amd/csrc/pointwise.hip
@@ -143,10 +143,7 @@
 }
 
 __global__ void transpose_kernel(const float* __restrict__ src, float* __restrict__ dst, int rows, int cols) {
-    const int i = blockIdx.x * blockDim.x + threadIdx.x;
-    if (i >= rows * cols) return;
-    const int c = i / rows, r = i % rows;
-    dst[i] = src[(size_t)r * cols + c];
+    transpose_one(src, dst, rows, cols, blockIdx.x * blockDim.x + threadIdx.x);
 }
 int transpose_launch(const float* src, float* dst, int rows, int cols, hipStream_t s) {
     hipLaunchKernelGGL(transpose_kernel, dim3(cdiv(rows * cols, 256)), dim3(256), 0, s, src, dst, rows, cols);
@@ -862,6 +859,50 @@
     }
     if (threadIdx.x == 0) sums[2 * C] = bce;
 }
+__device__ __forceinline__ void crit_value_eval(double si, double su, bool live, double bce_sum, int C, double count, double priority, double w_dice, double w_bce,
+                                                double* __restrict__ out) {
+    double q = live ? 2.0 * (si + 1e-6) / (su + 2e-6) : 0.0;
+    for (int o = 32; o > 0; o >>= 1) q += __shfl_xor(q, o);
+    if (threadIdx.x == 0) {
+        const double dice = priority * (1.0 - q / C), bce = -bce_sum / count;
+        out[0] = w_dice * dice + w_bce * bce; out[1] = dice; out[2] = bce;
+    }
+}
+__global__ __launch_bounds__(256) void crit_final_value_kernel(const float* __restrict__ part, double* __restrict__ sums, int N, int C, int nblk, double count,
+                                                               double priority, double w_dice, double w_bce, double* __restrict__ out) {
+    __shared__ double buf[4];
+    __shared__ double fin[2 * 64 + 1];
+    double bce = 0.0;
+    for (int c = 0; c < C; ++c) {
+        double si = 0.0, su = 0.0, sb = 0.0;
+        for (int i = threadIdx.x; i < N * nblk; i += 256) {
+            const int n = i / nblk, b = i % nblk;
+            const float* q = part + (((size_t)n * C + c) * nblk + b) * 3;
+            si += (double)q[0]; su += (double)q[1]; sb += (double)q[2];
+        }
+        si = block_sum_d(si, buf);
+        su = block_sum_d(su, buf);
+        sb = block_sum_d(sb, buf);
+        if (threadIdx.x == 0) { sums[c] = si; sums[C + c] = su; fin[c] = si; fin[64 + c] = su; }
+        bce += sb;
+    }
+    if (threadIdx.x == 0) { sums[2 * C] = bce; fin[128] = bce; }
+    __syncthreads();
+    if (threadIdx.x < 64) {
+        const bool live = threadIdx.x < (unsigned)C;
+        crit_value_eval(live ? fin[threadIdx.x] : 0.0, live ? fin[64 + threadIdx.x] : 0.0, live, fin[128], C, count, priority, w_dice, w_bce, out);
+    }
+}
+int crit_sums_value_launch(const float* p, const float* g, double* sums, int N, int C, size_t V, float bgw, void* ws, size_t ws_bytes,
+                           double count, double priority, double w_dice, double w_bce, double* out3, hipStream_t s) {
+    const int nblk = crit_tiles(V);
+    if (!ws || ws_bytes < (size_t)N * C * nblk * 3 * sizeof(float)) { set_error("criterion: workspace too small"); return RU_ENOMEM; }
+    hipLaunchKernelGGL(crit_partial_kernel, dim3(nblk, N * C), dim3(256), 0, s, p, g, (float*)ws, V, nblk, bgw);
+    RU_CHECK_LAUNCH("crit_partial_kernel");
+    hipLaunchKernelGGL(crit_final_value_kernel, dim3(1), dim3(256), 0, s, (const float*)ws, sums, N, C, nblk, count, priority, w_dice, w_bce, out3);
+    RU_CHECK_LAUNCH("crit_final_value_kernel");
+    return RU_OK;
+}
 int crit_sums_launch(const float* p, const float* g, double* sums, int N, int C, size_t V, float bgw, void* ws, size_t ws_bytes, hipStream_t s) {
     const int nblk = crit_tiles(V);
     if (!ws || ws_bytes < (size_t)N * C * nblk * 3 * sizeof(float)) { set_error("criterion: workspace too small"); return RU_ENOMEM; }
@@ -873,12 +914,8 @@
 }
 __global__ void crit_value_kernel(const double* __restrict__ sums, int C, double count, double priority, double w_dice, double w_bce,
                                   double* __restrict__ out) {
-    double q = threadIdx.x < (unsigned)C ? 2.0 * (sums[threadIdx.x] + 1e-6) / (sums[C + threadIdx.x] + 2e-6) : 0.0;
-    for (int o = 32; o > 0; o >>= 1) q += __shfl_xor(q, o);
-    if (threadIdx.x == 0) {
-        const double dice = priority * (1.0 - q / C), bce = -sums[2 * C] / count;
-        out[0] = w_dice * dice + w_bce * bce; out[1] = dice; out[2] = bce;
-    }
+    const bool live = threadIdx.x < (unsigned)C;
+    crit_value_eval(live ? sums[threadIdx.x] : 0.0, live ? sums[C + threadIdx.x] : 0.0, live, sums[2 * C], C, count, priority, w_dice, w_bce, out);
 }
 int crit_value_launch(const double* sums, int C, double count, double priority, double w_dice, double w_bce, double* out3, hipStream_t s) {
     hipLaunchKernelGGL(crit_value_kernel, dim3(1), dim3(64), 0, s, sums, C, count, priority, w_dice, w_bce, out3);
@@ -1218,9 +1255,8 @@
 }
 
 template <bool AMS>
-__global__ __launch_bounds__(256) void adam_kernel(float* __restrict__ w, const float* __restrict__ g, float* __restrict__ m, float* __restrict__ v,
-                                                   float* __restrict__ vmax, size_t n, float step_size, float b1, float b2, float eps, float wd,
-                                                   float bc2_sqrt) {
+__device__ __forceinline__ void adam_span(float* __restrict__ w, const float* __restrict__ g, float* __restrict__ m, float* __restrict__ v, float* __restrict__ vmax,
+                                          size_t n, float step_size, float b1, float b2, float eps, float wd, float bc2_sqrt) {
     for (size_t i = (size_t)blockIdx.x * 256 + threadIdx.x; i < n; i += (size_t)gridDim.x * 256) {
         const float wi = w[i];
         const float gi = g[i] + wd * wi;
@@ -1233,6 +1269,30 @@
         w[i] = wi - step_size * (mi / denom);
     }
 }
+template <bool AMS>
+__global__ __launch_bounds__(256) void adam_kernel(float* __restrict__ w, const float* __restrict__ g, float* __restrict__ m, float* __restrict__ v,
+                                                   float* __restrict__ vmax, size_t n, float step_size, float b1, float b2, float eps, float wd,
+                                                   float bc2_sqrt) {
+    adam_span<AMS>(w, g, m, v, vmax, n, step_size, b1, b2, eps, wd, bc2_sqrt);
+}
+template <bool AMS>
+__global__ __launch_bounds__(256) void adam_runs_kernel(const AdamRuns r, float step_size, float b1, float b2, float eps, float wd, float bc2_sqrt) {
+    const int k = blockIdx.y;
+    adam_span<AMS>(r.w[k], r.g[k], r.m[k], r.v[k], r.vmax[k], r.n[k], step_size, b1, b2, eps, wd, bc2_sqrt);
+}
+int adam_runs_launch(const AdamRuns& r, bool amsgrad, float lr, float b1, float b2, float eps, float wd, int step, hipStream_t s) {
+    RU_REQUIRE(r.nruns >= 1 && r.nruns <= RU_ADAM_RUNS, "adam: 1..%d runs per launch", RU_ADAM_RUNS);
+    RU_REQUIRE(step >= 1, "adam: step is 1-based");
+    size_t nmax = 0;
+    for (int k = 0; k < r.nruns; ++k) nmax = r.n[k] > nmax ? r.n[k] : nmax;
+    if (nmax == 0) return RU_OK;
+    const double bc1 = 1.0 - pow((double)b1, (double)step), bc2 = 1.0 - pow((double)b2, (double)step);
+    const dim3 grid(grid1d(nmax, 256 * 4, 4096), r.nruns);
+    if (amsgrad) hipLaunchKernelGGL(adam_runs_kernel<true>, grid, dim3(256), 0, s, r, (float)((double)lr / bc1), b1, b2, eps, wd, (float)sqrt(bc2));
+    else hipLaunchKernelGGL(adam_runs_kernel<false>, grid, dim3(256), 0, s, r, (float)((double)lr / bc1), b1, b2, eps, wd, (float)sqrt(bc2));
+    RU_CHECK_LAUNCH("adam_runs_kernel");
+    return RU_OK;
+}
 int adam_launch(float* w, const float* g, float* m, float* v, float* vmax, size_t n, float lr, float b1, float b2,
                 float eps, float wd, int step, hipStream_t s) {
     if (n == 0) return RU_OK;
diff --git a/brats2019_amd/csrc/pointwise_c16.hip b/brats2019_amd/csrc/pointwise_c16.hip
--- a/brats2019_amd/csrc/pointwise_c16.hip
+++ b/brats2019_amd/csrc/pointwise_c16.hip
@@ -333,12 +333,7 @@
 }
 
 __global__ void pack_down16_kernel(const float* __restrict__ w, float* __restrict__ wd, float* __restrict__ wdT, int Cout, int Cin) {
-    const int i = blockIdx.x * blockDim.x + threadIdx.x;
-    if (i >= Cout * Cin * 8) return;
-    const int tap = i & 7, c = (i >> 3) % Cin, o = i / (8 * Cin);
-    const float v = w[i];
-    wd[(size_t)o * 8 * Cin + tap * Cin + c] = v;
-    wdT[(size_t)(tap * Cin + c) * Cout + o] = v;
+    pack_down16_one(w, wd, wdT, Cout, Cin, blockIdx.x * blockDim.x + threadIdx.x);
 }
 int pack_down16_launch(const float* w, float* wd, float* wdT, int Cout, int Cin, hipStream_t s) {
     const int total = Cout * Cin * 8;
diff --git a/brats2019_amd/csrc/ru_common.h b/brats2019_amd/csrc/ru_common.h
--- a/brats2019_amd/csrc/ru_common.h
+++ b/brats2019_amd/csrc/ru_common.h
@@ -68,6 +68,19 @@
         hi[i] = hb;
         lo[i] = lb;
     }
+}
+
+__device__ __forceinline__ void pack_down16_one(const float* __restrict__ w, float* __restrict__ wd, float* __restrict__ wdT, int Cout, int Cin, int i) {
+    if (i >= Cout * Cin * 8) return;
+    const int tap = i & 7, c = (i >> 3) % Cin, o = i / (8 * Cin);
+    const float v = w[i];
+    wd[(size_t)o * 8 * Cin + tap * Cin + c] = v;
+    wdT[(size_t)(tap * Cin + c) * Cout + o] = v;
+}
+__device__ __forceinline__ void transpose_one(const float* __restrict__ src, float* __restrict__ dst, int rows, int cols, int i) {
+    if (i >= rows * cols) return;
+    const int c = i / rows, r = i % rows;
+    dst[i] = src[(size_t)r * cols + c];
 }
 
 void set_error(const char* fmt, ...);
@@ -189,6 +202,9 @@
 int conv3_mxg_split_launch(const float* x, void* g16, size_t nvox, hipStream_t s);
 bool conv3_sb_forward_skips_direct(int N, int Cin, int Cout, int D, int H, int W);
 int conv3_sb_pack_batch(SbPackBatch& b, hipStream_t s);
+constexpr int SB_PACK_DOWN16 = 2, SB_PACK_TRANSPOSE = 3;
+int conv3_sb_pack_add_down16(SbPackBatch& b, const float* w, float* wd, int Cout, int Cin, hipStream_t s);
+int conv3_sb_pack_add_transpose(SbPackBatch& b, const float* src, float* dst, int rows, int cols, hipStream_t s);
 int conv3_pack_weights(const float* w, float* wp, int Cin_f, int Cout_f, int mode, hipStream_t s);
 size_t conv3_packed_floats(int Cin_conv, int Cout_conv);
 
@@ -332,6 +348,8 @@
 int crit_grad_launch(const float* p, const float* g, const double* sums, double count, float w_dice, float w_bce,
                      float bgw, float priority, float* dp, int N, int C, size_t V, hipStream_t s);
 int crit_value_launch(const double* sums, int C, double count, double priority, double w_dice, double w_bce, double* out3, hipStream_t s);
+int crit_sums_value_launch(const float* p, const float* g, double* sums, int N, int C, size_t V, float bgw, void* ws, size_t ws_bytes,
+                           double count, double priority, double w_dice, double w_bce, double* out3, hipStream_t s);
 int tta_merge_launch(const float* p, int K, unsigned flips, float* mean_out, unsigned char* mask, unsigned long long* counts, int C, int D, int H, int W, hipStream_t s);
 int compose_labels_launch(const unsigned char* mask, const unsigned long long* counts, unsigned long long et_min, unsigned char* labels, size_t V, hipStream_t s);
 int dice_counts_launch(const float* p, const float* g, unsigned long long* counts, int rows, size_t V, hipStream_t s);
@@ -354,5 +372,8 @@
 int augment_patch_launch(const AugmentArgs& a, hipStream_t s);
 int adam_launch(float* w, const float* g, float* m, float* v, float* vmax, size_t n, float lr, float b1, float b2,
                 float eps, float wd, int step, hipStream_t s);
-
-}
+constexpr int RU_ADAM_RUNS = 8;
+struct AdamRuns { float* w[RU_ADAM_RUNS]; const float* g[RU_ADAM_RUNS]; float* m[RU_ADAM_RUNS]; float* v[RU_ADAM_RUNS]; float* vmax[RU_ADAM_RUNS]; size_t n[RU_ADAM_RUNS]; int nruns; };
+int adam_runs_launch(const AdamRuns& r, bool amsgrad, float lr, float b1, float b2, float eps, float wd, int step, hipStream_t s);
+
+}
diff --git a/brats2019_amd/loss.py b/brats2019_amd/loss.py
--- a/brats2019_amd/loss.py
+++ b/brats2019_amd/loss.py
@@ -14,6 +14,17 @@
     return 1
 
 
+def _sums_and_losses(pred, gt, bg_weight, priority, w_dice, w_bce, group):
+    import torch.distributed as dist
+    if group is False or not (dist.is_available() and dist.is_initialized()):
+        count = float(pred.numel())
+        sums, out = ops.criterion_sums_losses(pred, gt, count, bg_weight, priority, w_dice, w_bce)
+        return sums, count, out
+    sums = ops.criterion_sums(pred, gt, bg_weight)
+    count = float(pred.numel()) * _all_reduce_sums(sums, group)
+    return sums, count, ops.criterion_losses(sums, count, priority, w_dice, w_bce)
+
+
 _HAND_OVER_DEPTH = 0
 
 
@@ -56,10 +67,7 @@
 class _CriterionFn(torch.autograd.Function):
     @staticmethod
     def forward(ctx, pred, gt, w_dice, w_bce, bg_weight, priority, group):
-        sums = ops.criterion_sums(pred, gt, bg_weight)
-        world = _all_reduce_sums(sums, group)
-        count = float(pred.numel()) * world
-        out = ops.criterion_losses(sums, count, priority, w_dice, w_bce)
+        sums, count, out = _sums_and_losses(pred, gt, bg_weight, priority, w_dice, w_bce, group)
         ctx.save_for_backward(pred, gt, sums)
         ctx.cfg = (count, w_dice, w_bce, bg_weight, priority)
         return out[0].to(torch.float32)
@@ -79,10 +87,8 @@
 
     @staticmethod
     def forward(ctx, pred, gt, bg_weight, priority, group):
-        sums = ops.criterion_sums(pred, gt, bg_weight)
-        world = _all_reduce_sums(sums, group)
-        count = float(pred.numel()) * world
-        out = ops.criterion_losses(sums, count, priority, 0.5, 0.5).to(torch.float32)
+        sums, count, out = _sums_and_losses(pred, gt, bg_weight, priority, 0.5, 0.5, group)
+        out = out.to(torch.float32)
         ctx.save_for_backward(pred, gt, sums)
         ctx.cfg = (count, bg_weight, priority)
         loss, dice, bce = out[0], out[1], out[2]
diff --git a/brats2019_amd/ops.py b/brats2019_amd/ops.py
--- a/brats2019_amd/ops.py
+++ b/brats2019_amd/ops.py
@@ -159,6 +159,40 @@
     L.check(L.load().ru_criterion_value_device(L.ptr(sums), c, float(count), float(priority), float(w_dice), float(w_bce), L.ptr(out), L.stream()),
             "ru_criterion_value_device")
     return out
+
+
+def criterion_sums_losses(p, g, count, bg_weight=1e-2, priority=1.0, w_dice=0.5, w_bce=0.5):
+    p, g = _prep(p), _prep(g)
+    if p.shape != g.shape:
+        raise AssertionError("prediction/target shape mismatch")
+    lib = L.load()
+    n, c = int(p.shape[0]), int(p.shape[1])
+    if c > 64 or not L.has("ru_criterion_sums_losses"):
+        sums = criterion_sums(p, g, bg_weight)
+        return sums, criterion_losses(sums, count, priority, w_dice, w_bce)
+    v = p.numel() // (n * c)
+    sums = torch.empty(2 * c + 1, dtype=torch.float64, device=p.device)
+    out = torch.empty(3, dtype=torch.float64, device=p.device)
+    ws = L.workspace(lib.ru_criterion_workspace_bytes(n, c, v), p.device)
+    L.check(lib.ru_criterion_sums_losses(L.f32(p), L.f32(g), L.ptr(sums), n, c, v, bg_weight, float(count), float(priority), float(w_dice), float(w_bce),
+                                         L.ptr(out), L.ptr(ws), ws.numel(), L.stream()), "ru_criterion_sums_losses")
+    return sums, out
+
+
+def adam_step_runs(runs, lr, betas, eps, weight_decay, step, amsgrad=True):
+    import ctypes as C
+    lib = L.load()
+    if len(runs) == 1 or not L.has("ru_adam_step_runs"):
+        for w, g, m, v, vm, n in runs:
+            L.check(lib.ru_adam_step(w, g, m, v, vm if amsgrad else None, n, lr, float(betas[0]), float(betas[1]), float(eps), float(weight_decay), int(step), L.stream()),
+                    "ru_adam_step")
+        return
+    for i in range(0, len(runs), 8):
+        part = runs[i:i + 8]
+        cols = [(C.c_void_p * len(part))(*[r[j] for r in part]) for j in range(5)]
+        nn = (C.c_size_t * len(part))(*[r[5] for r in part])
+        L.check(lib.ru_adam_step_runs(cols[0], cols[1], cols[2], cols[3], cols[4] if amsgrad else None, nn, len(part), lr, float(betas[0]), float(betas[1]),
+                                      float(eps), float(weight_decay), int(step), L.stream()), "ru_adam_step_runs")
 
 
 def criterion_value(sums, count, priority=1.0):
diff --git a/brats2019_amd/optim.py b/brats2019_amd/optim.py
--- a/brats2019_amd/optim.py
+++ b/brats2019_amd/optim.py
@@ -2,7 +2,7 @@
 
 import torch
 
-from . import _lib as L
+from . import _lib as L, ops
 
 
 class Adam(torch.optim.Optimizer):
@@ -83,8 +83,6 @@
         if closure is not None:
             with torch.enable_grad():
                 loss = closure()
-        lib = L.load()
-        stream = L.stream()
         for gi, group in enumerate(self.param_groups):
             params = group["params"]
             if not params:
@@ -123,8 +121,11 @@
                         r[5] += n
                         continue
                 runs.append([ptrs[0], ptrs[1], ptrs[2], ptrs[3], ptrs[4], n, k])
-            for w, g, m, v, vm, n, k in runs:
-                L.check(lib.ru_adam_step(w, g, m, v, vm if ams else None, n, lr, float(b1), float(b2), float(group["eps"]),
-                                         float(group["weight_decay"]), k, stream), "ru_adam_step")
+            launches = 0
+            for k in sorted(set(r[6] for r in runs)):
+                same = [tuple(r[:6]) for r in runs if r[6] == k]
+                ops.adam_step_runs(same, lr, (b1, b2), group["eps"], group["weight_decay"], k, amsgrad=ams)
+                launches += (len(same) + 7) // 8 if L.has("ru_adam_step_runs") else len(same)
             self.__dict__["last_launches"] = len(runs)
+            self.__dict__["last_kernel_launches"] = launches
         return loss
diff --git a/brats2019_amd/parallel.py b/brats2019_amd/parallel.py
--- a/brats2019_amd/parallel.py
+++ b/brats2019_amd/parallel.py
@@ -48,6 +48,11 @@
         out = ops.criterion_losses(sums, count, priority, 0.5, 0.5)
         return out[0], out[1], out[2]
 
+    def criterion_sums_losses(self, probs, target, count, bg_weight, priority):
+        from . import ops
+        sums, out = ops.criterion_sums_losses(probs, target, count, bg_weight, priority, 0.5, 0.5)
+        return sums, out[0], out[1], out[2]
+
     def criterion_grad(self, probs, target, sums, count, bg_weight, priority):
         from . import ops
         return ops.criterion_grad(probs, target, sums, count, 0.5, 0.5, bg_weight, priority)
@@ -60,8 +65,11 @@
 
     def adam(self, flat, grads, m, v, vmax, step, lr, betas, eps, weight_decay):
         from . import ops
-        for a, b in self.live_segments:
-            ops.adam_amsgrad_step(flat[a:b], grads[a:b], m[a:b], v[a:b], vmax[a:b], step, lr, betas, eps, weight_decay)
+        for t in (flat, grads, m, v, vmax):
+            if not (t.is_cuda and t.dtype == torch.float32 and t.is_contiguous()):
+                raise TypeError("HipBackend.adam: contiguous float32 device buffers")
+        ops.adam_step_runs([tuple(t.data_ptr() + 4 * a for t in (flat, grads, m, v, vmax)) + (b - a,) for a, b in self.live_segments],
+                           float(lr), betas, eps, weight_decay, step, amsgrad=True)
 
 
 def merge_runs(runs, max_gap=1 << 16):
@@ -172,11 +180,14 @@
     def loss_and_grads(self, x_shard, target_shard):
         b = self.backend
         probs = b.forward(self.flat, x_shard, training=True)
-        sums = b.criterion_sums(probs, target_shard, self.bg_weight)
-        if self.distributed:
-            self._all_reduce(sums)
         count = float(probs.numel()) * self.world
-        loss, dice, bce = b.criterion_losses(sums, count, self.priority)
+        if not self.distributed and hasattr(b, "criterion_sums_losses"):
+            sums, loss, dice, bce = b.criterion_sums_losses(probs, target_shard, count, self.bg_weight, self.priority)
+        else:
+            sums = b.criterion_sums(probs, target_shard, self.bg_weight)
+            if self.distributed:
+                self._all_reduce(sums)
+            loss, dice, bce = b.criterion_losses(sums, count, self.priority)
         if self.fuse_criterion_grad and hasattr(b, "backward_criterion"):
             b.backward_criterion(self.flat, target_shard, sums, count, self.bg_weight, self.priority, self.grads)
         else:
diff --git a/include/resunet_hip.h b/include/resunet_hip.h
--- a/include/resunet_hip.h
+++ b/include/resunet_hip.h
@@ -71,6 +71,8 @@
 int ru_criterion_value(const double* sums_host, int C, double count, double priority, double* dice, double* bce);
 int ru_criterion_value_device(const double* sums, int C, double count, double priority, double w_dice, double w_bce,
                               double* out3, ru_stream_t stream);
+int ru_criterion_sums_losses(const float* p, const float* g, double* sums, int N, int C, size_t V, float bg_weight, double count,
+                             double priority, double w_dice, double w_bce, double* out3, void* ws, size_t ws_bytes, ru_stream_t stream);
 
 #define RU_CRIT_DICE_JOINT 0
 #define RU_CRIT_BCE 1
@@ -112,6 +114,11 @@
 int ru_adam_step(float* w, const float* g, float* m, float* v, float* vmax_or_null, size_t n,
                  float lr, float beta1, float beta2, float eps, float weight_decay, int step,
                  ru_stream_t stream);
+int ru_adam_step_runs(float* const* w, const float* const* g, float* const* m, float* const* v, float* const* vmax_or_null,
+                      const size_t* n, int nruns, float lr, float beta1, float beta2, float eps, float weight_decay, int step,
+                      ru_stream_t stream);
+int ru_weight_packs(const float* const* src, float* const* dst, const int* rows, const int* cols, const int* kind, int n, int batched,
+                    ru_stream_t stream);
 
 ru_unet_t ru_unet_create(int depth, const int* encoder_layers, const int* decoder_layers,
                          const int* number_of_channels, int number_of_outputs);
```

Result: no change. 270.1, median of 6 (+0.4%).
